# graphic-goose/ferreus_rbf_rs

Measured on AMD Instinct MI355X. Metric: BBFMM matvecs/s, higher is better.
Workload: dtype f64; 1 GPU; 10000000 uniform 3D points, LinearRbf, order 7, 1 rhs, adaptive sparse tree, ACA eps=1e-7, set_weights + evaluate at the sources; points=10000000, kernel=LinearRbf, order=7, nrhs=1, parallelism=single GPU

## Files before the change

### ferreus_rbf_rs_amd/_lib.py

```python
from __future__ import annotations

import ctypes
import os

HERE = os.path.dirname(os.path.abspath(__file__))
LIB_PATH = os.environ.get("FERREUS_BBFMM_HIP_LIB") or os.path.join(HERE, "libferreus_bbfmm_hip.so")

OK, POINT_OUTSIDE_TREE, KERNEL_NO_GRADIENTS, BAD_ARGUMENT, DEVICE_ERROR, UNSUPPORTED, CALLBACK_FAILED = range(7)
FLAG_HOST_ONLY = 1
FLAG_M2L_SHARED_BASIS = 2
FLAG_DIRECT_SMALL_W_LEAVES = 4
FLAG_DETERMINISTIC = 8
N_PHASES = 11
PHASE_NAMES = ["gather", "P2M", "M2M", "M2L_stage1", "M2L_stage2", "P2L", "L2L", "P2P", "M2P",
               "L2P", "scatter"]

c_i32, c_i64, c_f64, c_u32 = ctypes.c_int32, ctypes.c_int64, ctypes.c_double, ctypes.c_uint32
c_p = ctypes.c_void_p


class Params(ctypes.Structure):
    _fields_ = [("max_points_per_cell", c_i64), ("compression_type", c_i32),
                ("epsilon", c_f64), ("eval_chunk_size", c_i64)]

# ... 36 lines not shown
    "bbfmm_isosurface_tables": (ctypes.c_int, [c_p, c_p, c_p, c_p, c_p]),
    "bbfmm_isosurface_lattice": (ctypes.c_int, [c_p, c_p, c_f64, c_p]),
    "bbfmm_build_isosurfaces": (ctypes.c_int, [c_p, c_p, c_f64, c_p, c_i32, c_p, c_p, c_i64, c_p]),
    "bbfmm_isosurfaces_from_values": (ctypes.c_int, [c_p, c_p, c_p, c_f64, c_p, c_i32, c_i64, c_p]),
    "bbfmm_build_isosurfaces_ex": (ctypes.c_int, [c_p, c_p, c_f64, c_p, c_i32, c_p, c_p, c_i64, c_i32, c_p]),
    "bbfmm_isosurfaces_from_values_ex": (ctypes.c_int, [c_p, c_p, c_p, c_f64, c_p, c_i32, c_i64, c_i32, c_p]),
    "bbfmm_isosurface_stats": (ctypes.c_int, [c_p, c_i32, c_p]),
    "bbfmm_build_isosurfaces_opts": (ctypes.c_int, [c_p, c_p, c_f64, c_p, c_i32, c_p, c_p, c_p, c_p]),
    "bbfmm_isosurfaces_from_values_opts": (ctypes.c_int, [c_p, c_p, c_p, c_f64, c_p, c_i32, c_p, c_p]),
    "bbfmm_isosurfaces_from_fields_opts": (ctypes.c_int, [c_p, c_i32, c_p, c_i32, c_p, c_f64, c_p, c_i32, c_p, c_p, c_p]),
    "bbfmm_isosurfaces_from_function_opts": (ctypes.c_int, [c_p, c_p, c_p, c_p, c_f64, c_p, c_i32, c_p, c_p]),
    "bbfmm_debug_evaluate_fields": (ctypes.c_int, [c_p, c_i32, c_p, c_i32, c_p, c_i64, c_i64, c_p, c_p, c_i64]),
    "bbfmm_debug_field_program": (ctypes.c_int, [c_i32, c_i32, c_p, c_p, c_p, c_i32, c_p, c_p, c_i64, c_p, c_p]),
    "bbfmm_isosurface_finish_mesh": (ctypes.c_int, [c_p, c_p, c_i64, c_p, c_i64, c_p, c_p]),
    "bbfmm_isosurface_finish_stats": (ctypes.c_int, [c_p, c_i32, c_p]),
    "bbfmm_isosurface_close_mesh": (ctypes.c_int, [c_p, c_p, c_i64, c_p, c_i64, c_p, ctypes.c_double, c_i32, c_p]),
    "bbfmm_isosurface_closure_stats": (ctypes.c_int, [c_p, c_i32, c_p]),
    "bbfmm_debug_closure_triangulate": (ctypes.c_int, [c_i32, c_i32, c_p, c_p, c_p, c_i64, c_p, c_i64, c_p, c_i64, ctypes.c_double,
                                                       ctypes.c_double, c_i64, c_p, c_p, c_i64, c_p, c_p, c_p, c_i64]),
    "bbfmm_debug_orient2d": (ctypes.c_int, [c_p, c_i64, c_p]),
    "bbfmm_isosurface_follow_stats": (ctypes.c_int, [c_p, c_i32, c_p]),
    "bbfmm_isosurface_follow_times": (ctypes.c_int, [c_p, c_i32, c_p]),
    "bbfmm_isosurface_follow_bricks": (ctypes.c_int, [c_p, c_i32, c_p, c_p]),
    "bbfmm_isosurface_intersection_stats": (ctypes.c_int, [c_p, c_i32, c_p]),
    "bbfmm_isosurface_self_intersections": (ctypes.c_int, [c_p, c_p, c_i64, c_p, c_i64, c_p, c_p]),
    "bbfmm_isosurface_intersection_ids": (ctypes.c_int, [c_p, c_i32, c_p, c_p]),
    "bbfmm_isosurface_triangle_pair": (ctypes.c_int, [c_p, c_p, c_p, c_p, c_p, c_p]),
    "bbfmm_isosurface_clip_triangle": (ctypes.c_int, [c_p, c_p, c_p, c_p, c_p]),
    "bbfmm_isosurface_topology": (ctypes.c_int, [ctypes.c_uint32, c_p, c_p, c_p]),
    "bbfmm_isosurface_cluster_tables": (ctypes.c_int, [c_p, c_p, c_p]),
    "bbfmm_isosurface_curvature_tables": (ctypes.c_int, [c_p, c_p, c_p]),
    "bbfmm_isosurface_curvature_weight": (ctypes.c_int, [c_p, c_p, c_i32, c_p, c_p, c_p, c_p]),
    "bbfmm_isosurface_curvature_stats": (ctypes.c_int, [c_p, c_i32, c_p]),
    "bbfmm_isosurface_count": (c_i32, [c_p]),
    "bbfmm_isosurface_size": (ctypes.c_int, [c_p, c_i32, c_p, c_p]),
    "bbfmm_isosurface_copy": (ctypes.c_int, [c_p, c_i32, c_p, c_p]),
    "bbfmm_isosurface_error": (ctypes.c_char_p, [c_p]),
    "bbfmm_isosurface_destroy": (None, [c_p]),
    "bbfmm_prepare_target_subset": (ctypes.c_int, [c_p, c_p, c_i64]),
    "bbfmm_fast_matrix_vector_product": (ctypes.c_int, [c_p, c_p, c_i64, c_i64, c_p, c_i64, c_p,
                                                        c_i64, c_f64, c_p]),
    "bbfmm_matvec_device": (ctypes.c_int, [c_p, c_p, c_i64, c_i32, c_p, c_i64, c_i32]),
    "bbfmm_target_subset_create": (ctypes.c_int, [c_p, c_p, c_i64, c_p]),
    "bbfmm_matvec_subset_device": (ctypes.c_int, [c_p, c_i32, c_p, c_p, c_i32]),
    "bbfmm_stream": (c_p, [c_p]),
    "bbfmm_set_partition": (ctypes.c_int, [c_p, c_i32, c_i32]),
    "bbfmm_partition_row_count": (c_i64, [c_p]),
    "bbfmm_partition_rows": (ctypes.c_int, [c_p, c_p]),
    "bbfmm_partition_coarse_count": (c_i64, [c_p]),
    "bbfmm_matvec_partition_upward": (ctypes.c_int, [c_p, c_p, c_i64, c_i32, c_p, c_p]),
    "bbfmm_matvec_partition_finish": (ctypes.c_int, [c_p, c_p, c_p, c_i64, c_i32, c_p]),
    "bbfmm_partition_world": (c_i32, [c_p]),
    "bbfmm_partition_rank": (c_i32, [c_p]),
    "bbfmm_partition_bounds": (ctypes.c_int, [c_p, c_i32, c_p]),
    "bbfmm_matvec_partition_finish_sorted": (ctypes.c_int, [c_p, c_p, c_p, c_i64, c_p]),
    "bbfmm_partition_scatter": (ctypes.c_int, [c_p, c_p, c_i32, c_i32, c_i64, c_i32, c_p, c_i64]),
    "bbfmm_debug_partition_upward_counts": (ctypes.c_int, [c_p, c_p, c_p, c_p]),
    "bbfmm_debug_host_copy_rates": (ctypes.c_int, [c_i64, c_p]),
    "bbfmm_get_tree_stats": (ctypes.c_int, [c_p, c_p]),
    "bbfmm_tree_built_on_device": (ctypes.c_int, [c_p]),
    "bbfmm_last_evaluate_at_sources": (ctypes.c_int, [c_p]),
    "bbfmm_debug_targets_are_sources": (ctypes.c_int, [c_p, c_p, c_i64, c_i64]),
    "bbfmm_debug_rows_of_sources": (ctypes.c_int, [c_p, c_p, c_i64, c_i64, c_p]),
    "bbfmm_get_cells": (ctypes.c_int, [c_p, c_p, c_p]),
    "bbfmm_get_leaf_sources": (ctypes.c_int, [c_p, c_p, c_p]),
    "bbfmm_get_list": (ctypes.c_int, [c_p, ctypes.c_char, c_p, c_p, c_p]),
    "bbfmm_get_m2l_ranks": (ctypes.c_int, [c_p, c_p, c_p]),
    "bbfmm_get_m2l_operator": (ctypes.c_int, [c_p, c_i32, c_i32, c_p]),
    "bbfmm_get_m2l_factors": (ctypes.c_int, [c_p, c_i32, c_i32, c_p, c_p]),
    "bbfmm_get_permutation_tables": (ctypes.c_int, [c_p, c_p, c_p, c_p, c_p, c_p]),
    "bbfmm_points_to_leaves": (ctypes.c_int, [c_p, c_p, c_i64, c_i64, c_p, c_p]),
    "bbfmm_set_profiling": (ctypes.c_int, [c_p, c_i32]),
    "bbfmm_get_phase_ms": (ctypes.c_int, [c_p, c_p, c_p]),
    "bbfmm_reset_phase_ms": (ctypes.c_int, [c_p]),
    "bbfmm_mfma_f64_selftest": (ctypes.c_int, [c_p, c_p, c_p]),
    "bbfmm_fp64_valu_selftest": (ctypes.c_int, [c_p, c_p]),
    "bbfmm_debug_kernel_values": (ctypes.c_int, [c_i32, c_i32, ctypes.c_double, ctypes.c_double, c_p, c_i64, c_p, c_p, c_p]),
    "bbfmm_debug_math": (ctypes.c_int, [c_i32, c_i32, c_p, c_i64, c_p, c_p]),
    "bbfmm_debug_dense_m2m": (ctypes.c_int, [c_p, c_i32, c_p]),
    "bbfmm_debug_apply_m2l_tables_host": (ctypes.c_int, [c_p, c_p, c_p]),
    "bbfmm_debug_m2l_variants": (ctypes.c_int, [c_p, c_p, c_p]),
    "bbfmm_debug_m2l_pairs": (ctypes.c_int, [c_p, c_p, c_i64, c_p, c_p]),
    "bbfmm_debug_m2l_pairs_axes": (ctypes.c_int, [c_p, c_p, c_i64, c_p]),
    "bbfmm_debug_m2l_pairs_stage2": (ctypes.c_int, [c_p, c_p, c_i64, c_p, c_p]),
    "bbfmm_debug_m2l_pairs_axes_stage2": (ctypes.c_int, [c_p, c_p, c_i64, c_p]),
    "bbfmm_debug_m2l_table_digests": (ctypes.c_int, [c_p, c_p, c_i32, c_p, c_p, c_i32, c_p]),
    "bbfmm_debug_m2l_s2_last_ksplit": (ctypes.c_int, [c_p, c_p]),
    "bbfmm_debug_leaf_runs": (ctypes.c_int, [c_p, c_p]),
    "bbfmm_debug_group_state": (ctypes.c_int, [c_p, c_p, c_i64]),
    "bbfmm_debug_m2l_parity_len": (ctypes.c_int, [c_p, c_p]),
    "bbfmm_debug_get_coefficients": (ctypes.c_int, [c_p, ctypes.c_char, c_i32, c_p]),
    "bbfmm_debug_morton_encode": (ctypes.c_uint64, [c_i32, c_p, ctypes.c_uint64]),
    "bbfmm_debug_morton_decode": (None, [c_i32, ctypes.c_uint64, c_p, c_p]),
    "bbfmm_debug_morton_neighbours": (c_i32, [c_i32, ctypes.c_uint64, c_p]),
    "bbfmm_debug_direction_vectors": (c_i32, [c_i32, c_p]),
    "bbfmm_debug_reference_vectors": (ctypes.c_int, [c_p, c_p, c_p]),
    "bbfmm_givens_rotation": (None, [c_f64, c_f64, c_p, c_p, c_p]),
    "bbfmm_fgmres": (ctypes.c_int, [c_i64, c_p, c_p, c_p, c_p, c_p, c_p, c_i32, c_i32, c_i32, c_f64,
                                    c_p, c_p, c_p, c_p, c_p]),
    "bbfmm_schwarz_ddm_solver": (ctypes.c_int, [c_i64, c_p, c_p, c_p, c_p, c_p, c_i32, c_i32, c_f64,
                                                c_p, c_p, c_p, c_p, c_p]),
    "bbfmm_rbf_system_apply": (ctypes.c_int, [c_p, c_p, c_p, c_i64]),
    "bbfmm_rbf_system_device_create": (ctypes.c_int, [c_p, c_i64, c_p, c_i64, c_f64, c_p]),
    "bbfmm_rbf_system_device_destroy": (None, [c_p]),
    "bbfmm_rbf_system_apply_device": (ctypes.c_int, [c_p, c_p, c_p, c_i64, c_p]),
    "bbfmm_fgmres_device": (ctypes.c_int, [c_i64, c_p, c_p, c_p, c_p, c_p, c_p, c_i32, c_i32, c_i32, c_f64,
                                           c_p, c_p, c_p, c_p, c_p, c_p]),
    "bbfmm_schwarz_ddm_solver_device": (ctypes.c_int, [c_i64, c_p, c_p, c_p, c_p, c_p, c_i32, c_i32, c_f64,
                                                       c_p, c_p, c_p, c_p, c_p, c_p]),
    "bbfmm_debug_solver_vector_op": (ctypes.c_int, [c_i32, c_i32, c_i64, c_p, c_p, c_p, c_f64, c_i32, c_p, c_i32, c_p, c_p]),
    "bbfmm_ddm_params_defaults": (None, [c_p]),
    "bbfmm_ddm_params_for_points": (None, [c_i64, c_p]),
    "bbfmm_ddm_build": (ctypes.c_int, [c_p, c_i64, c_i32, c_i64, c_p, c_p]),
    "bbfmm_ddm_destroy": (None, [c_p]),
    "bbfmm_ddm_num_levels": (c_i32, [c_p]),
    "bbfmm_ddm_level_size": (c_i64, [c_p, c_i32]),
    "bbfmm_ddm_level_points": (ctypes.c_int, [c_p, c_i32, c_p]),
    "bbfmm_ddm_num_domains": (c_i64, [c_p, c_i32]),
    "bbfmm_ddm_domain_size": (c_i64, [c_p, c_i32, c_i64]),
    "bbfmm_ddm_domain": (ctypes.c_int, [c_p, c_i32, c_i64, c_p, c_p, c_p]),
    "bbfmm_schwarz_create": (ctypes.c_int, [c_p, c_p, c_i64, c_i32, c_i64, c_p, c_p, c_p]),
    "bbfmm_schwarz_create_sharded": (ctypes.c_int, [c_p, c_p, c_i64, c_i32, c_i64, c_p, c_p, c_i32, c_i32, c_p, c_i64, c_p, c_p, c_p]),
    "bbfmm_schwarz_factor_bytes": (c_i64, [c_p]),
    "bbfmm_schwarz_domains_owned": (c_i64, [c_p, c_i32, ctypes.POINTER(c_i64), ctypes.POINTER(c_i64)]),
    "bbfmm_schwarz_destroy": (None, [c_p]),
    "bbfmm_schwarz_basis_size": (c_i64, [c_p]),
    "bbfmm_schwarz_num_levels": (c_i32, [c_p]),
    "bbfmm_schwarz_monomial_matrix": (c_p, [c_p]),
    "bbfmm_debug_evaluate_monomials": (ctypes.c_int, [c_p, c_i64, c_i32, c_i64, c_i32, c_p, c_p, c_p]),
    "bbfmm_schwarz_apply": (ctypes.c_int, [c_p, c_p, c_p, c_i64]),
    "bbfmm_schwarz_apply_device": (ctypes.c_int, [c_p, c_p, c_p, c_i64, c_p]),
    "bbfmm_schwarz_debug_trace_steps": (c_i32, [c_p]),
    "bbfmm_schwarz_debug_apply_trace": (ctypes.c_int, [c_p, c_p, c_p, c_i64, c_i32, c_p, c_p, c_p, c_p, c_p]),
    "bbfmm_schwarz_debug_ortho_matrix": (c_p, [c_p]),
    "bbfmm_schwarz_level_size": (c_i64, [c_p, c_i32]),
    "bbfmm_schwarz_level_points": (ctypes.c_int, [c_p, c_i32, c_p]),
    "bbfmm_schwarz_debug_level_solve": (ctypes.c_int, [c_p, c_i32, c_p, c_p, c_i64, c_i32]),
    "bbfmm_ddm_debug_level_create": (ctypes.c_int, [c_p, c_i64, c_i32, c_i64, c_i64, c_p, c_p, c_p, c_p, c_i32, c_i32, c_p]),
    "bbfmm_ddm_debug_level_destroy": (None, [c_p]),
    "bbfmm_ddm_debug_level_info": (ctypes.c_int, [c_p, c_p]),
    "bbfmm_ddm_debug_level_layout": (ctypes.c_int, [c_p, c_p, c_p, c_p, c_p, c_p]),
    "bbfmm_ddm_debug_level_assembled": (ctypes.c_int, [c_p, c_p]),
    "bbfmm_ddm_debug_level_factor": (ctypes.c_int, [c_p, c_p]),
    "bbfmm_ddm_debug_level_solve": (ctypes.c_int, [c_p, c_p, c_p, c_i64, c_i32]),
    "bbfmm_schwarz_create_ex": (ctypes.c_int, [c_p, c_p, c_i64, c_i32, c_i64, c_p, c_i64, c_p, c_p, c_p]),
    "bbfmm_schwarz_create_sharded_ex": (ctypes.c_int, [c_p, c_p, c_i64, c_i32, c_i64, c_p, c_i64, c_p, c_p, c_i32, c_i32, c_p, c_i64,
                                                       c_p, c_p, c_p]),
    "bbfmm_ddm_debug_level_create_ex": (ctypes.c_int, [c_p, c_i64, c_i32, c_i64, c_p, c_i64, c_i64, c_p, c_p, c_p, c_p, c_i32, c_i32,
                                                       c_p]),
    "bbfmm_global_trend_transform": (ctypes.c_int, [c_i32, c_p, c_p, c_p, c_p]),
    "bbfmm_duplicate_cutoff_distance": (ctypes.c_int, [c_p, c_f64, c_p]),
    "bbfmm_remove_duplicates": (ctypes.c_int, [c_p, c_i64, c_i32, c_i64, c_f64, c_i32, c_p, c_p, c_p]),
    "bbfmm_debug_interpolant_terms": (ctypes.c_int, [c_i32, c_i32, c_p, c_p, c_i64, c_i64, c_p, c_i64, c_p, c_i64, c_p, c_i64]),
    "bbfmm_evaluate_interpolant": (ctypes.c_int, [c_p, c_i32, c_i32, c_p, c_i64, c_i32, c_i64, c_p, c_i64, c_i64, c_p, c_f64,
                                                  c_p, c_i64, c_p, c_i64, c_p]),
    "bbfmm_evaluate_device": (ctypes.c_int, [c_p, c_i32, c_p, c_i64, c_i64, c_p, c_p, c_i64, c_p, c_i64, c_p, c_p]),
    "bbfmm_evaluate_grid": (ctypes.c_int, [c_p, c_i32, c_p, c_p, c_p, c_i64, c_p, c_i64, c_p, c_p]),
    "bbfmm_evaluate_grid_stats": (ctypes.c_int, [c_p, c_p]),
    "bbfmm_debug_grid_coords": (ctypes.c_int, [c_i32, c_p, c_i64, c_i64, c_p, c_i64]),
    "bbfmm_debug_split_runs": (ctypes.c_int, [c_i32, c_p, c_p, c_p, c_i64, c_i32, c_p, c_p, c_p, c_i64, c_p]),
}


class Interpolant(ctypes.Structure):
    _fields_ = [("kernel_type", c_i32), ("polynomial_degree", c_i32), ("nugget", c_f64), ("base_range", c_f64),
                ("total_sill", c_f64), ("flags", c_u32)]
# ... 83 lines not shown
```

### ferreus_rbf_rs_amd/csrc/capi_debug.cpp

```cpp
#include <algorithm>
#include <chrono>
#include <cstring>
#include <vector>

#include "capi_handle.hpp"
#include "morton.hpp"

namespace {
template <int ID>
void debug_kernel_values_host(const bbfmm::KernelSpec &ks, const double *r2, int64_t n, double *value, double *value_g, double *factor) {
    for (int64_t i = 0; i < n; ++i) {
        value[i] = bbfmm::kernel_value_r2<ID>(ks, r2[i]);
        value_g[i] = bbfmm::kernel_value_grad_r2<ID>(ks, r2[i], &factor[i]);
    }
}
}

extern "C" {

int bbfmm_debug_targets_are_sources(const bbfmm_handle *h, const double *x, int64_t m, int64_t ldx) {
    return (h && h->tree.targets_are_sources(x, m, ldx)) ? 1 : 0;
}
int bbfmm_debug_rows_of_sources(bbfmm_handle *h, const double *x, int64_t m, int64_t ldx, int64_t *rows_out) {
    if (!h || !rows_out) return 0;
// ... 95 lines not shown
            case 1: bbfmm::bb_sqrt_rsqrt(x[i], &a, &b); break;
            case 2: a = bbfmm::bb_rcp(x[i]); break;
            default: a = bbfmm::bb_log(x[i]); break;
            }
            out[i] = a;
            if (out2) out2[i] = b;
        }
        return BBFMM_OK;
    }
    int ndev = 0;
    if (hipGetDeviceCount(&ndev) != hipSuccess || ndev == 0) return BBFMM_DEVICE_ERROR;
    return bbfmm::debug_math_device(which, x, n, out, out2) == 0 ? BBFMM_OK : BBFMM_DEVICE_ERROR;
}

int bbfmm_debug_dense_m2m(const bbfmm_handle *h, int32_t child_index, double *out) {
    if (!h || !out) return BBFMM_BAD_ARGUMENT;
    std::vector<double> m;
    bbfmm::dense_m2m_matrix(h->tree.ops(), child_index, &m);
    std::memcpy(out, m.data(), m.size() * sizeof(double));
    return BBFMM_OK;
}

int bbfmm_debug_apply_m2l_tables_host(const bbfmm_handle *h, const double *M, double *L) {
    if (!h || !M || !L) return BBFMM_BAD_ARGUMENT;
    return h->tree.debug_apply_m2l_tables_host(M, L);
}

uint64_t bbfmm_debug_morton_encode(int32_t d, const uint64_t *anchor, uint64_t level) {
    if (d < 1 || d > 3 || !anchor) return 0;
    return bbfmm::encode_morton_point(anchor, level, d);
}
void bbfmm_debug_morton_decode(int32_t d, uint64_t key, uint64_t *anchor_out, uint64_t *level_out) {
    if (d < 1 || d > 3 || !anchor_out || !level_out) return;
    bbfmm::decode_key(key, d, anchor_out, level_out);
}
int32_t bbfmm_debug_morton_neighbours(int32_t d, uint64_t key, uint64_t *keys_out) {
    if (d < 1 || d > 3 || !keys_out) return -1;
    return bbfmm::get_neighbours(key, d, keys_out);
}
int32_t bbfmm_debug_direction_vectors(int32_t d, int32_t *out) {
    if (d < 1 || d > 3 || !out) return -1;
    const int(*dirs)[3];
    const int n = bbfmm::direction_vectors(d, &dirs);
    for (int i = 0; i < n; ++i)
        for (int a = 0; a < d; ++a) out[i * d + a] = dirs[i][a];
    return n;
}
int bbfmm_debug_reference_vectors(const bbfmm_handle *h, int32_t *out, int32_t *n_ref_out) {
    if (!h) return BBFMM_BAD_ARGUMENT;
    const bbfmm::Operators &ops = h->tree.ops();
    if (n_ref_out) *n_ref_out = ops.n_ref;
    if (out) std::copy(ops.ref_vecs.begin(), ops.ref_vecs.end(), out);
    return BBFMM_OK;
}

int bbfmm_debug_m2l_variants(const bbfmm_handle *h, int64_t *n_variants, int64_t *n_cells) {
    if (!h) return BBFMM_BAD_ARGUMENT;
    int64_t nv = 0, nc = 0;
    h->tree.m2l_variant_stats(&nv, &nc);
    if (n_variants) *n_variants = nv;
    if (n_cells) *n_cells = nc;
    return BBFMM_OK;
}

int bbfmm_debug_m2l_pairs(const bbfmm_handle *h, int32_t *out, int64_t cap, int64_t *n_out, int32_t *pairs_on) {
    if (!h || !n_out) return BBFMM_BAD_ARGUMENT;
    std::vector<int32_t> v;
    h->tree.debug_m2l_pairs(&v);
    *n_out = static_cast<int64_t>(v.size());
    if (pairs_on) *pairs_on = h->tree.m2l_pairs() ? 1 : 0;
    if (out) std::copy(v.begin(), v.begin() + std::min<int64_t>(cap, *n_out), out);
    return BBFMM_OK;
}

int bbfmm_debug_m2l_pairs_axes(const bbfmm_handle *h, int32_t *out, int64_t cap, int64_t *n_out) {
    if (!h || !n_out) return BBFMM_BAD_ARGUMENT;
    std::vector<int32_t> v;
    h->tree.debug_m2l_pairs_axes(&v);
    *n_out = static_cast<int64_t>(v.size());
    if (out) std::copy(v.begin(), v.begin() + std::min<int64_t>(cap, *n_out), out);
    return BBFMM_OK;
}

int bbfmm_debug_m2l_pairs_stage2(const bbfmm_handle *h, int32_t *out, int64_t cap, int64_t *n_out, int32_t *pairs_on) {
    if (!h || !n_out) return BBFMM_BAD_ARGUMENT;
    std::vector<int32_t> v;
    h->tree.debug_m2l_pairs_stage2(&v);
    *n_out = static_cast<int64_t>(v.size());
    if (pairs_on) *pairs_on = h->tree.m2l_pairs_stage2() ? 1 : 0;
    if (out) std::copy(v.begin(), v.begin() + std::min<int64_t>(cap, *n_out), out);
    return BBFMM_OK;
}

int bbfmm_debug_m2l_pairs_axes_stage2(const bbfmm_handle *h, int32_t *out, int64_t cap, int64_t *n_out) {
    if (!h || !n_out) return BBFMM_BAD_ARGUMENT;
    std::vector<int32_t> v;
    h->tree.debug_m2l_pairs_axes_stage2(&v);
    *n_out = static_cast<int64_t>(v.size());
    if (out) std::copy(v.begin(), v.begin() + std::min<int64_t>(cap, *n_out), out);
    return BBFMM_OK;
}

int bbfmm_debug_m2l_table_digests(const bbfmm_handle *h, uint64_t *digests, int32_t cap, int32_t *n_out, double *flops_level,
                                  int32_t flops_cap, int32_t *n_levels_out) {
    if (!h || !n_out) return BBFMM_BAD_ARGUMENT;
    std::vector<uint64_t> v;
    h->tree.debug_m2l_table_digests(&v);
    *n_out = static_cast<int32_t>(v.size());
    if (digests) std::copy(v.begin(), v.begin() + std::min<int32_t>(cap, *n_out), digests);
    const std::vector<double> &fl = h->tree.m2l_flops_level();
    if (n_levels_out) *n_levels_out = static_cast<int32_t>(fl.size());
    if (flops_level) std::copy(fl.begin(), fl.begin() + std::min<int32_t>(flops_cap, static_cast<int32_t>(fl.size())), flops_level);
    return BBFMM_OK;
}

int bbfmm_debug_m2l_s2_last_ksplit(const bbfmm_handle *h, int32_t *ksplit) {
    if (!h || !ksplit) return BBFMM_BAD_ARGUMENT;
    *ksplit = h->tree.debug_m2l_s2_last_ksplit();
    return BBFMM_OK;
}

int bbfmm_debug_leaf_runs(const bbfmm_handle *h, int32_t *counts) {
    if (!h || !counts) return BBFMM_BAD_ARGUMENT;
    h->tree.debug_leaf_runs(counts);
    return BBFMM_OK;
}

int bbfmm_debug_group_state(const bbfmm_handle *h, int64_t *out, int64_t cap) {
    if (!h || !out) return BBFMM_BAD_ARGUMENT;
    const int64_t need = bbfmm::DeviceGroup::kStateHeader + (h->group ? h->group->n_parts() : 1);
    if (cap < need) return BBFMM_BAD_ARGUMENT;
    std::fill(out, out + need, int64_t(0));
    if (h->group)
        h->group->debug_state(out);
    else
        out[0] = 1;
    return BBFMM_OK;
}

int bbfmm_debug_m2l_parity_len(const bbfmm_handle *h, int32_t *len) {
    if (!h || !len) return BBFMM_BAD_ARGUMENT;
    *len = h->tree.debug_m2l_parity_len();
    return BBFMM_OK;
}

int bbfmm_debug_get_coefficients(bbfmm_handle *h, char which, int32_t k, double *out) {
    GUARD(h) return h->tree.debug_get_coefficients(which, k, out);
    END_GUARD(h)
}

}
```

### ferreus_rbf_rs_amd/csrc/device.hpp

```cpp
#pragma once
#include <hip/hip_runtime.h>

#include <cstdint>

#include "kernels.hpp"

namespace bbfmm {

constexpr int kMaxOrder = 16;
constexpr int kM2lTile = 128;
constexpr int kM2lS1Block = 176;
constexpr int kM2lS1BlockPairs = 160;
constexpr int kM2lSlotWindow = 128;
constexpr int kM2lBlkTwoDst = 1 << 30;

struct DevCheb {
    int p, d, n, n_pad;
    double polyn[kMaxOrder * kMaxOrder];
    double q[kMaxOrder * kMaxOrder];
    double nodes[kMaxOrder];
    double xfer[2 * kMaxOrder * kMaxOrder];
};

struct ChebRef {
    const DevCheb *dev;
    int p, d, n, n_pad;
};

struct M2lClass {
    const double *vt_all;
    const int32_t *row_dst;
    const int32_t *row_dst2;
    const int32_t *blk_t0;
    int32_t yb0;
    int32_t n_rows;
    int32_t r_pad16;
    int32_t n_t;
    const double *u_all;
    int32_t k_pad;
    int32_t kp;
    int32_t kpy;
    const int32_t *cells;
    int32_t n_cells;
    const int32_t *cslot;
    const int64_t *cbase;
};

struct M2lTileDesc {
    int32_t level_class;
    int32_t first;
    int32_t count;
    int32_t q_first;
    int32_t q_count;
    int32_t pad;
};

void launch_gather_weights(const double *w, int64_t ldw, int K, const int32_t *order, int64_t N,
                           double *w_sorted, hipStream_t s);
void launch_gather_weights_subset(const double *w, int64_t ldw, int K, const int32_t *order, const int32_t *pos, int64_t n_pos,
                                  int64_t N, double *w_sorted, hipStream_t s);
constexpr int kMaxScatterParts = 64;
struct ScatterParts {
    int n;
    int64_t bound[kMaxScatterParts + 1];
};
void launch_scatter_parts(const double *all, const ScatterParts &parts, int64_t m_max, int K, const int32_t *order, double *out,
                          int64_t ldo, hipStream_t s);
void launch_sum_slots(const double *slots, int n_slots, int64_t len, double *out, hipStream_t s);
void launch_scatter_output(const double *out_sorted, int64_t n, int K, const int32_t *perm,
                           double *out, int64_t ldo, int accumulate, hipStream_t s);
void launch_gather_rows(const double *src, int64_t ld_src, int ncols, const int32_t *idx, int64_t n,
                        double *dst, int64_t ld_dst, hipStream_t s);

void launch_p2m(const ChebRef &ch, const double *const *src_xyz, const double *w_sorted, int64_t N,
                int K, int64_t C, const int32_t *leaf_cells, int n_leaves, const int32_t *pt_begin,
                const int32_t *pt_end, const double *centers, const double *lengths, double *M,
                hipStream_t s);
struct M2lParityRowArgs;
struct M2lUnparityRowArgs;
int launch_m2m(const ChebRef &ch, int K, int64_t C, const int32_t *parents, int n_parents,
               const int64_t *child_ptr, const int32_t *child_idx, const int32_t *octant, double *M,
               hipStream_t s, const M2lParityRowArgs *par = nullptr, double *Mp = nullptr);
bool m2m_writes_parity(const ChebRef &ch);
int launch_l2l(const ChebRef &ch, int K, int64_t C, const int32_t *cells, int n_cells,
               const int32_t *parent, const int32_t *octant, const uint8_t *active, double *L,
               hipStream_t s, const M2lUnparityRowArgs *unp = nullptr, const double *Lp = nullptr,
               const uint8_t *has_m2l = nullptr, const uint8_t *has_x = nullptr);
bool l2l_reads_parity(const ChebRef &ch);
void launch_zero_rows(const int32_t *cells, int n_cells, int n_pad, int K, int64_t C, double *L, hipStream_t s);

void launch_m2l_stage1(const M2lClass *classes, const M2lTileDesc *tiles, const int32_t *tile_idx, int n_tiles,
                       int n_pad, int max_slot_t, int K, int64_t C, const double *M, double *cbuf,
                       int64_t cbuf_len, hipStream_t s, bool own_blocks = false, int max_blocks = 8, int ne16 = 0, int s_ee = 0,
                       int s_eo = 0);
void launch_m2l_parity(const double *M, int n_pad, double *Mp, int n_par, int ne16, int n_e, int n_o, int p, int64_t rows,
                       hipStream_t s);
struct M2lParityOffsets {
    int32_t v[4];
};
void launch_m2l_parity2(const double *M, int n_pad, double *Mp, int n_par, M2lParityOffsets off, int p, int p2, int64_t rows,
                        hipStream_t s);
void launch_m2l_stage2(const M2lClass *classes, const M2lTileDesc *tiles, const int32_t *tile_idx, int n_tiles,
                       int n_pad, int K, int64_t C, const double *cbuf, int64_t cbuf_len,
                       const uint16_t *qlist, double *L, hipStream_t s, bool allow_ksplit = true);
struct M2lS2PairsPlan {
    int ga, gb, ce, co;
    int ya = 0, yb = 0;
    int ne16() const { return 16 * ga * ce; }
    __host__ __device__ int n_par() const { return 16 * (ga * ce + gb * co); }
    __host__ __device__ int col(int part, int j) const {
        const int g = part < 2 ? ga : gb, y = part < 2 ? ya : yb, w = 16 * ((part & 1) ? g - y : y);
        const int jj = j % w, gl = ((part & 1) ? y : 0) + jj / 16, pp = jj % 16, paired = g / 2 * 2;
        const int local = gl < paired ? 32 * (gl / 2) + 2 * pp + (gl & 1) : 16 * paired + pp;
        return (part < 2 ? 0 : 16 * ga * ce) + (j / w) * 16 * g + local;
    }
};
M2lS2PairsPlan m2l_s2_pairs_plan(int groups_even, int groups_odd);
M2lS2PairsPlan m2l_s2_pairs_plan2(const int groups[4]);
struct M2lParityRowArgs {
    int axes = 0;
    int n_par = 0;
    int p = 0;
    int ne16 = 0, n_e = 0, n_o = 0, p1 = 0;
    M2lParityOffsets off{{0, 0, 0, 0}};
    int p2 = 0;
};

struct M2lUnparityRowArgs {
    int axes = 0;
    int n_par = 0;
    int p = 0;
    int ne16 = 0, n_e = 0, n_o = 0, p1 = 0;
    M2lS2PairsPlan plan{1, 1, 1, 1};
    int p2 = 0;
};
void launch_m2l_parity_cells(const double *M, int n_pad, double *Mp, const M2lParityRowArgs &par, const int32_t *cells, int n_cells,
                             int K, int64_t C, hipStream_t s);
int m2l_s2_pairs_ksplit(int n_tiles, const M2lS2PairsPlan &plan, int K, bool allow_ksplit);
bool launch_m2l_stage2_pairs(const M2lClass *classes, const M2lTileDesc *tiles, const int32_t *tile_idx, int n_tiles,
                             const M2lS2PairsPlan &plan, int K, int64_t C, const double *cbuf, int64_t cbuf_len,
                             const uint16_t *qlist, double *Lp, hipStream_t s, bool allow_ksplit = true, int *ksplit_out = nullptr);
void launch_m2l_unparity(const double *Lp, int n_par, int ne16, double *L, int n, int n_pad, int n_e, int n_o, int p, int64_t rows,
                         hipStream_t s);
void launch_m2l_unparity2(const double *Lp, const M2lS2PairsPlan &plan, double *L, int n, int n_pad, int p, int p2, int64_t rows,
                          hipStream_t s);
void launch_m2l_zero_segments(const int32_t *segs, int64_t n_segs, int K, double *cbuf, int64_t cbuf_len, hipStream_t s);
void launch_m2l_basis(const M2lClass *classes, const M2lTileDesc *tiles, int n_tiles, int in_ld, int out_ld, int K,
                      int64_t C, const double *in, double *out, hipStream_t s);
void launch_small_gemm(bool trans_a, int M, int N, int Kd, const double *A, int64_t lda, const double *B, int64_t ldb,
                       double *Cm, int64_t ldc, hipStream_t s);

struct M2lAssembleTv {
    int32_t perm;
    int32_t rank;
    int32_t row;
    int64_t vt_off;
    int64_t u_off;
};
struct M2lAssembleClass {
    const M2lAssembleTv *src, *tgt;
    int32_t n_src, n_tgt, r_pad16, k_pad, max_rank;
    int32_t n_e, n_o, ne16, n_par, p;
    int32_t u_npar, u_ne16, u_rows, u_ne, u_no;
    int32_t s1_axes;
    M2lParityOffsets s1_off;
    M2lS2PairsPlan u_plan;
};
void launch_m2l_assemble(const M2lAssembleClass &c, int n, int n_pad, bool compressed, const double *ops,
                         const int32_t *invperm, double *vt_all, double *u_all, hipStream_t s);

struct DirectJobs {
    int n_jobs;
    const int32_t *job_cell;
    const int32_t *tgt_begin, *tgt_end;
    const int64_t *run_ptr;
    const int32_t *runs;
};
// ... 53 lines not shown
```

### ferreus_rbf_rs_amd/csrc/device_m2l.hip

```cpp
#include "device_common.hpp"
#include "m2l_basis_rows.hpp"

#include <cmath>

namespace bbfmm {

typedef __attribute__((address_space(3))) void *lptr_t;

__device__ inline unsigned lds_offset(const double *p) {
    return static_cast<unsigned>(reinterpret_cast<uintptr_t>((lptr_t)p));
}
__device__ inline unsigned uniform_u32(unsigned v) { return __builtin_amdgcn_readfirstlane(v); }
__device__ inline const double *uniform_ptr(const double *p) {
    const uintptr_t v = reinterpret_cast<uintptr_t>(p);
    const unsigned lo = __builtin_amdgcn_readfirstlane(static_cast<unsigned>(v));
    const unsigned hi = __builtin_amdgcn_readfirstlane(static_cast<unsigned>(v >> 32));
    return reinterpret_cast<const double *>((static_cast<uintptr_t>(hi) << 32) | lo);
}
__device__ inline void dma16(const double *g, unsigned lds_wave_byte_offset) {
    asm volatile("s_mov_b32 m0, %1\n\ts_nop 0\n\tglobal_load_lds_dwordx4 %0, off" ::"v"(g),
                 "s"(uniform_u32(lds_wave_byte_offset))
                 : "memory");
}
__device__ inline void dma4(const int32_t *g, unsigned lds_wave_byte_offset) {
    asm volatile("s_mov_b32 m0, %1\n\ts_nop 0\n\tglobal_load_lds_dword %0, off" ::"v"(g),
                 "s"(uniform_u32(lds_wave_byte_offset))
                 : "memory");
}
__device__ inline void wait_dma_and_barrier() {
    asm volatile("s_waitcnt vmcnt(0)" ::: "memory");
    __syncthreads();
}
template <int N> __device__ inline void wait_dma_keep_stores_and_barrier() {
    asm volatile("s_waitcnt vmcnt(%0)" ::"n"(N < 63 ? N : 63) : "memory");
    __syncthreads();
}
template <int N> __device__ inline double add_row_ror(double v) {
    const int lo = __double2loint(v), hi = __double2hiint(v);
    const int rlo = __builtin_amdgcn_update_dpp(0, lo, 0x120 + N, 0xf, 0xf, false);
    const int rhi = __builtin_amdgcn_update_dpp(0, hi, 0x120 + N, 0xf, 0xf, false);
    return v + __hiloint2double(rhi, rlo);
}

__device__ inline void dma16s(const double *sbase, unsigned voff_bytes, unsigned lds_wave_byte_offset) {
    asm volatile("s_mov_b32 m0, %2\n\ts_nop 0\n\tglobal_load_lds_dwordx4 %0, %1" ::"v"(voff_bytes),
                 "s"(uniform_ptr(sbase)), "s"(uniform_u32(lds_wave_byte_offset))
                 : "memory");
}

template <int NG16, int STAGE, int MINW, bool PAIRS = false>
__global__ __launch_bounds__(512, MINW) void m2l_gemm_k4(const M2lClass *__restrict__ classes,
                                                  const M2lTileDesc *__restrict__ tiles, int n_pad, int g16_0,
                                                  int64_t C, const double *__restrict__ in, int64_t in_len,
                                                  double *__restrict__ out, int64_t out_len,
                                                  const uint16_t *__restrict__ qlist, int slot_t,
                                                  const int32_t *__restrict__ tile_idx) {
    extern __shared__ double lds[];
    const M2lTileDesc tile = tiles[blockIdx.x];
    const M2lClass cls = classes[tile.level_class];
    const int kr = blockIdx.y;
    const int tid = threadIdx.x, wave = tid >> 6, lane = tid & 63;
    constexpr int BLK = PAIRS ? kM2lS1BlockPairs : kM2lS1Block;
    const int n_zb = STAGE == 1 ? cls.r_pad16 / BLK : 1;
    const bool own_blocks = STAGE == 1 && tile.pad == 2;
    const int zb0 = STAGE == 1 ? (own_blocks ? tile.q_first : (int)((int64_t)n_zb * blockIdx.z / gridDim.z)) : 0;
    const int zb1 = STAGE == 1 ? (own_blocks ? tile.q_first + tile.q_count : (int)((int64_t)n_zb * (blockIdx.z + 1) / gridDim.z)) : 1;
    const int ld = STAGE == 1 ? cls.r_pad16 : n_pad;
    const int ksplit = STAGE == 2 && slot_t > 1 ? slot_t : 1;
    const int zcols = STAGE == 2 ? (int)gridDim.z / ksplit : 1;
    const int zk = STAGE == 2 ? (int)blockIdx.z / zcols : 0, zc = STAGE == 2 ? (int)blockIdx.z - zk * zcols : (int)blockIdx.z;
    const int q_lo = STAGE == 2 ? tile.q_count * zk / ksplit : 0;
    const int nq = STAGE == 1 ? n_pad / 16 : STAGE == 2 ? tile.q_count * (zk + 1) / ksplit - q_lo : (int)(in_len / 16);
    const uint16_t *ql = qlist + tile.q_first + q_lo;
    const int nq_e = PAIRS ? (int)(in_len & 0xffffffff) / 16 : 0;
    const int s_ee = PAIRS ? (int)(in_len >> 32) & 0xffff : 0, s_eo = PAIRS ? (int)(in_len >> 48) : 0;
    if (zb0 >= zb1) return;
    const int g16 = g16_0 + (STAGE >= 2 ? zc * NG16 : 0);
    const double *opbase = (STAGE == 1 ? cls.vt_all : cls.u_all) + 16 * g16;

    constexpr int OP_CHUNKS = 2 * NG16;
    constexpr int NCH = (OP_CHUNKS + 7) / 8;
    constexpr int OP_DOUBLES = OP_CHUNKS * 128;
    constexpr int BUF = OP_DOUBLES + 2048;

    constexpr int NP = NG16 / 2, NS = NG16 & 1;
    unsigned voff[NCH];
#pragma unroll
    for (int i = 0; i < NCH; ++i) {
        const int c = wave + 8 * i;
        if (c < 4 * NP) {
            const int e = c / NP, pr = c - e * NP, k = lane >> 4, p = lane & 15;
            voff[i] = (unsigned)(((4 * k + e) * ld + 32 * pr + 2 * p) * 8);
        } else {
            const int e = 2 * (c - 4 * NP) + (lane >> 5), r = lane & 31, k = r >> 3, pair = r & 7;
            voff[i] = (unsigned)(((4 * k + e) * ld + 32 * NP + 2 * pair) * 8);
        }
    }
    auto cell_p = [&](int pos) {
        const int q = pos < tile.count ? pos : 0;
        return tile.pad ? tile_idx[tile.first + q] : tile.first + q;
    };
    const double *cptr[2];
#pragma unroll
    for (int h = 0; h < 2; ++h) {
        const int tg = 2 * h + (lane >> 5), eh = (lane >> 4) & 1, k = (lane >> 2) & 3, j = lane & 3;
        const int pos = wave * 16 + 4 * tg + j;
        const int p = cell_p(pos);
        const int64_t base = STAGE == 2 ? (int64_t)kr * in_len + cls.cbase[p]
                                        : ((int64_t)kr * C + cls.cells[p]) * (STAGE == 1 ? (int64_t)n_pad : in_len);
        cptr[h] = in + base + 4 * k + 2 * eh;
    }
    const unsigned lds0 = lds_offset(lds);
    const int64_t qstride = (int64_t)16 * ld;
    auto stage = [&](int sidx, int buf) {
        const int zb = zb0 + sidx / nq, qi = sidx - (sidx / nq) * nq;
        int q = STAGE == 2 ? (int)ql[qi] : qi;
        if constexpr (PAIRS) {
            if (zb >= cls.yb0) {
                if (qi >= s_ee && qi < s_ee + s_eo) q = qi + s_eo;
                else if (qi >= s_ee + s_eo && qi < s_ee + 2 * s_eo) q = qi - s_eo;
            }
        }
#pragma unroll
        for (int i = 0; i < NCH; ++i)
            if (wave + 8 * i < OP_CHUNKS)
                dma16s(opbase + (int64_t)zb * BLK + q * qstride, voff[i],
                       lds0 + (unsigned)(buf * BUF + (wave + 8 * i) * 128) * 8u);
#pragma unroll
        for (int h = 0; h < 2; ++h)
            dma16(cptr[h] + 16 * q, lds0 + (unsigned)(buf * BUF + OP_DOUBLES + (2 * wave + h) * 128) * 8u);
    };

    double acc[4][NG16];
    double acc_e[4][PAIRS ? NG16 : 1];
#pragma unroll
    for (int tg = 0; tg < 4; ++tg)
#pragma unroll
        for (int g = 0; g < NG16; ++g) {
            acc[tg][g] = 0.0;
            if constexpr (PAIRS) acc_e[tg][g] = 0.0;
        }

    const int bk = lane >> 4, bj = lane & 3;
    const bool wave_live = wave * 16 < tile.count;
    const int n_steps = (zb1 - zb0) * nq;
    const int di = lane >> 4, db = (lane >> 2) & 3, dj = lane & 3;
    constexpr int AUX = PAIRS ? 384 : 192;
    const int32_t *aux = reinterpret_cast<const int32_t *>(lds + 2 * BUF);
    int32_t *ptab = reinterpret_cast<int32_t *>(lds + 2 * BUF) + 2 * AUX;
    const int32_t *slds = aux + 2 * AUX + 128 + wave * 16 * slot_t;
    if (STAGE == 1 && lane < 16) ptab[wave * 16 + lane] = cell_p(wave * 16 + lane);
    const unsigned aux0 = lds0 + (unsigned)(2 * BUF) * 8u;
    auto stage_cols = [&](int zb_, int par) {
        if (STAGE == 1 && 64 * wave <= 16 * NG16) {
            const int e = 64 * wave + lane;
            const int32_t *src = e < 16 * NG16 ? cls.row_dst + zb_ * BLK + 16 * g16 + e : cls.blk_t0 + zb_;
            dma4(src, aux0 + (unsigned)(par * AUX + 64 * wave) * 4u);
        } else if (PAIRS && 64 * wave < 192 + 16 * NG16) {
            const int e = 64 * wave + lane - 192;
            const int32_t *src = e < 16 * NG16 ? cls.row_dst2 + zb_ * BLK + 16 * g16 + e : cls.blk_t0 + zb_;
            dma4(src, aux0 + (unsigned)(par * AUX + 64 * wave) * 4u);
        }
    };
    const int slot_sh = 31 - __builtin_clz(slot_t | 1);
    auto stage_slots = [&](int par) {
        const int t0 = __builtin_amdgcn_readfirstlane(aux[par * AUX + 16 * NG16]) & (kM2lBlkTwoDst - 1);
        const unsigned dst0 = aux0 + (unsigned)(2 * AUX + 128 + wave * 16 * slot_t) * 4u;
        for (int i = 0; i < slot_t / 4; ++i) {
            const int e = i * 64 + lane, cl = e >> slot_sh, tl = e & (slot_t - 1);
            const int32_t *src = cls.cslot + (int64_t)ptab[wave * 16 + cl] * cls.n_t + min(t0 + tl, cls.n_t - 1);
            dma4(src, dst0 + (unsigned)i * 256u);
        }
    };
    if (n_steps > 0) {
        stage(0, 0);
        stage_cols(zb0, 0);
    }
    wait_dma_and_barrier();
    int qcnt = 0, zb = zb0;
    for (int sidx = 0; sidx < n_steps; ++sidx) {
        const double *op = lds + (sidx & 1) * BUF + lane;
        const double2 *op2 = reinterpret_cast<const double2 *>(lds + (sidx & 1) * BUF) + lane;
        const double *ct = lds + (sidx & 1) * BUF + OP_DOUBLES + wave * 256 + (bk * 4 + bj) * 2;
        if (sidx + 1 < n_steps) stage(sidx + 1, (sidx + 1) & 1);
        if (STAGE == 1) {
            if (qcnt == 0 && zb + 1 < zb1) stage_cols(zb + 1, (zb + 1 - zb0) & 1);
            if (qcnt == nq - 2) stage_slots((zb - zb0) & 1);
        }
        if (wave_live) {
            if constexpr (PAIRS) {
                if (qcnt == nq_e) {
#pragma unroll
                    for (int tg = 0; tg < 4; ++tg)
#pragma unroll
                        for (int g = 0; g < NG16; ++g) {
                            acc_e[tg][g] = acc[tg][g];
                            acc[tg][g] = 0.0;
                        }
                }
            }
            constexpr int EH = PAIRS ? 1 : 2;
#pragma unroll
            for (int eh0 = 0; eh0 < 2; eh0 += EH) {
                double bq[4][2 * EH];
#pragma unroll
                for (int tg = 0; tg < 4; ++tg)
#pragma unroll
                    for (int eh = 0; eh < EH; ++eh) {
                        const double2 v = *reinterpret_cast<const double2 *>(ct + ((tg * 2 + eh0 + eh) * 16) * 2);
                        bq[tg][2 * eh] = v.x;
                        bq[tg][2 * eh + 1] = v.y;
                    }
#pragma unroll
                for (int el = 0; el < 2 * EH; ++el) {
                    const int e = 2 * eh0 + el;
#pragma unroll
                    for (int pr = 0; pr < NP; ++pr) {
                        const double2 a = op2[(e * NP + pr) * 64];
#pragma unroll
                        for (int tg = 0; tg < 4; ++tg) {
                            acc[tg][2 * pr] = __builtin_amdgcn_mfma_f64_4x4x4f64(a.x, bq[tg][el], acc[tg][2 * pr], 0, 0, 0);
                            acc[tg][2 * pr + 1] =
                                __builtin_amdgcn_mfma_f64_4x4x4f64(a.y, bq[tg][el], acc[tg][2 * pr + 1], 0, 0, 0);
                        }
                    }
                    if (NS) {
                        const double a = op[4 * NP * 128 + e * 64];
#pragma unroll
                        for (int tg = 0; tg < 4; ++tg)
                            acc[tg][NG16 - 1] = __builtin_amdgcn_mfma_f64_4x4x4f64(a, bq[tg][el], acc[tg][NG16 - 1], 0, 0, 0);
                    }
                }
            }
        }
        if (++qcnt == nq) {
            qcnt = 0;
            const int col0 = zb * BLK + 16 * g16;
            ++zb;
            bool two_dst = false;
            if constexpr (PAIRS) {
              if (wave_live) {
                double *cb = out + (int64_t)kr * out_len;
                double *dump = cb + (out_len - 128) + 2 * lane;
                const int32_t *auxb = aux + ((zb - 1 - zb0) & 1) * AUX;
                two_dst = (__builtin_amdgcn_readfirstlane(auxb[16 * NG16]) & kM2lBlkTwoDst) != 0;
                int pk[NP + NS], pk2[NP + NS];
#pragma unroll
                for (int pr = 0; pr < NP + NS; ++pr) {
                    pk[pr] = auxb[pr < NP ? 32 * pr + 2 * (4 * db + di) : 32 * NP + 4 * db + di];
                    pk2[pr] = two_dst ? auxb[192 + (pr < NP ? 32 * pr + 2 * (4 * db + di) : 32 * NP + 4 * db + di)] : -1;
                }
#pragma unroll
                for (int tg = 0; tg < 4; ++tg) {
                    const bool spv = wave * 16 + 4 * tg + dj < tile.count;
                    const int32_t *srow = slds + (4 * tg + dj) * slot_t;
#pragma unroll
                    for (int pr = 0; pr < NP + NS; ++pr) {
                        const bool single = NS && pr == NP;
                        const int g0 = single ? NG16 - 1 : 2 * pr, g1 = single ? NG16 - 1 : 2 * pr + 1;
                        const int sl = srow[max(pk[pr] >> 24, 0)];
                        const int okm = (spv ? -1 : 0) & ~(pk[pr] | sl);
                        double *dst = okm < 0 ? cb + (int64_t)sl * 2 + (pk[pr] & 0xffffff) : dump;
                        if (single) *dst = acc_e[tg][g0] + acc[tg][g0];
                        else *reinterpret_cast<double2 *>(dst) = make_double2(acc_e[tg][g0] + acc[tg][g0], acc_e[tg][g1] + acc[tg][g1]);
                        if (two_dst) {
                            const int sl2 = srow[max(pk2[pr] >> 24, 0)];
                            const int okm2 = (spv ? -1 : 0) & ~(pk2[pr] | sl2);
                            double *dst2 = okm2 < 0 ? cb + (int64_t)sl2 * 2 + (pk2[pr] & 0xffffff) : dump;
                            if (single) *dst2 = acc_e[tg][g0] - acc[tg][g0];
                            else *reinterpret_cast<double2 *>(dst2) = make_double2(acc_e[tg][g0] - acc[tg][g0], acc_e[tg][g1] - acc[tg][g1]);
                        }
                    }
                    __builtin_amdgcn_sched_barrier(0);
                }
              }
            } else if (STAGE == 1 && wave_live) {
                double *cb = out + (int64_t)kr * out_len;
                double *dump = cb + (out_len - 128) + 2 * lane;
                const int32_t *auxb = aux + ((zb - 1 - zb0) & 1) * AUX;
                int pk[NP + NS];
#pragma unroll
                for (int pr = 0; pr < NP; ++pr) pk[pr] = auxb[32 * pr + 2 * (4 * db + di)];
                if (NS) pk[NP] = auxb[32 * NP + 4 * db + di];
#pragma unroll
                for (int tg = 0; tg < 4; ++tg) {
                    const bool spv = wave * 16 + 4 * tg + dj < tile.count;
                    const int32_t *srow = slds + (4 * tg + dj) * slot_t;
#pragma unroll
                    for (int pr = 0; pr < NP; ++pr) {
                        const int sl = srow[max(pk[pr] >> 24, 0)];
                        const int okm = (spv ? -1 : 0) & ~(pk[pr] | sl);
                        double *dst = okm < 0 ? cb + (int64_t)sl * 2 + (pk[pr] & 0xffffff) : dump;
                        *reinterpret_cast<double2 *>(dst) = make_double2(acc[tg][2 * pr], acc[tg][2 * pr + 1]);
                    }
                    if (NS) {
                        const int sl = srow[max(pk[NP] >> 24, 0)];
                        const int okm = (spv ? -1 : 0) & ~(pk[NP] | sl);
                        double *dst = okm < 0 ? cb + (int64_t)sl * 2 + (pk[NP] & 0xffffff) : dump;
                        *dst = acc[tg][NG16 - 1];
                    }
                }
            } else if (STAGE >= 2) {
#pragma unroll
                for (int tg = 0; tg < 4; ++tg) {
                    const int tp = wave * 16 + 4 * tg + dj;
                    if (tp < tile.count) {
                        const int cell = cls.cells[cell_p(tp)];
                        double *Lc = out + ((int64_t)kr * C + cell) * n_pad + col0;
                        if (ksplit > 1) {
#pragma unroll
                            for (int pr = 0; pr < NP; ++pr) {
                                unsafeAtomicAdd(Lc + 32 * pr + 2 * (4 * db + di), acc[tg][2 * pr]);
                                unsafeAtomicAdd(Lc + 32 * pr + 2 * (4 * db + di) + 1, acc[tg][2 * pr + 1]);
                            }
                            if (NS) unsafeAtomicAdd(Lc + 32 * NP + 4 * db + di, acc[tg][NG16 - 1]);
                        } else {
#pragma unroll
                            for (int pr = 0; pr < NP; ++pr)
                                *reinterpret_cast<double2 *>(Lc + 32 * pr + 2 * (4 * db + di)) =
                                    make_double2(acc[tg][2 * pr], acc[tg][2 * pr + 1]);
                            if (NS) Lc[32 * NP + 4 * db + di] = acc[tg][NG16 - 1];
                        }
                    }
                }
            }
#pragma unroll
            for (int tg = 0; tg < 4; ++tg)
#pragma unroll
                for (int g = 0; g < NG16; ++g) acc[tg][g] = 0.0;
            if (STAGE == 1) {
                if (wave_live && two_dst) asm volatile("s_waitcnt vmcnt(%0)" ::"n"(8 * (NP + NS) < 63 ? 8 * (NP + NS) : 63) : "memory");
                else if (wave_live) asm volatile("s_waitcnt vmcnt(%0)" ::"n"(4 * (NP + NS) < 63 ? 4 * (NP + NS) : 63) : "memory");
                else asm volatile("s_waitcnt vmcnt(0)" ::: "memory");
                __syncthreads();
                continue;
            }
        }
        wait_dma_and_barrier();
    }
}

template <int NG16, int STAGE, int MINW, bool PAIRS = false>
static void m2l_gemm_launch(const M2lClass *classes, const M2lTileDesc *tiles, int n_tiles, int n_pad, int g16_0,
                            int n_colblocks, int K, int64_t C, const double *in, int64_t in_len, double *out,
                            int64_t out_len, const uint16_t *qlist, int slot_t, const int32_t *tile_idx, hipStream_t s) {
    const size_t lds = 2 * sizeof(double) * (size_t)(2 * NG16 * 128 + 2048) + (STAGE == 1 ? (size_t)(2 * (PAIRS ? 384 : 192) + 128 + 8 * 16 * (slot_t & 0xffff)) * 4 : 0);
    static std::atomic<uint64_t> attr_set[4] = {{0}, {0}, {0}, {0}};
    (void)allow_large_dynamic_lds(reinterpret_cast<const void *>(&m2l_gemm_k4<NG16, STAGE, MINW, PAIRS>), lds, attr_set);
    const int zdim = STAGE == 2 && slot_t > 1 ? n_colblocks * slot_t : n_colblocks;
    hipLaunchKernelGGL((m2l_gemm_k4<NG16, STAGE, MINW, PAIRS>), dim3(n_tiles, K, zdim), dim3(512), lds, s, classes,
                       tiles, n_pad, g16_0, C, in, in_len, out, out_len, qlist, slot_t, tile_idx);
}


template <int STAGE> constexpr int m2l_chunk_pref() { return STAGE == 1 ? kM2lS1Block / 16 : 22; }
constexpr int kM2lS2KsplitFill = 4;

template <int STAGE>
static void m2l_dispatch_chunks(int total_groups, const M2lClass *classes, const M2lTileDesc *tiles, int n_tiles,
                                int n_pad, int n_colblocks, int K, int64_t C, const double *in, int64_t in_len,
                                double *out, int64_t out_len, const uint16_t *qlist, int slot_t,
                                const int32_t *tile_idx, hipStream_t s) {
    int done = 0;
    const int pref = m2l_chunk_pref<STAGE>();
    while (done < total_groups) {
        const int left = total_groups - done;
        int take;
#define M2L_GO(NG, MW)                                                                                              \
    {                                                                                                               \
        take = NG;                                                                                                  \
        m2l_gemm_launch<NG, STAGE, MW>(classes, tiles, n_tiles, n_pad, done,                                        \
                                       STAGE >= 2 ? 1 : n_colblocks, K, C, in, in_len,                            \
                                       out, out_len, qlist, slot_t, tile_idx, s);                                   \
    }
        if (STAGE >= 2 && !(n_colblocks == 1 && left >= 16)) {
            int best_ng = 2, best_z = 1;
            for (int ng : {11, 8, 7, 6, 4, 2})
                for (int zc = 1; zc <= (n_colblocks == 1 ? 1 : ng == 11 ? 2 : 3); ++zc)
                    if (ng * zc <= left && ((left - ng * zc) % 2 == 0 || left - ng * zc == 7) &&
                        (ng * zc > best_ng * best_z || (ng * zc == best_ng * best_z && ng > best_ng))) {
                        best_ng = ng;
                        best_z = zc;
                    }
            take = best_ng * best_z;
#define M2L_ZGO(NG, MW)                                                                                             \
    m2l_gemm_launch<NG, STAGE, MW>(classes, tiles, n_tiles, n_pad, done, best_z, K, C, in, in_len, out, out_len,    \
                                   qlist, slot_t, tile_idx, s);
            if constexpr (STAGE >= 2) {
                switch (best_ng) {
                case 11: M2L_ZGO(11, 1) break;
                case 8: M2L_ZGO(8, 4) break;
                case 7: M2L_ZGO(7, 2) break;
                case 6: M2L_ZGO(6, 4) break;
                case 4: M2L_ZGO(4, 4) break;
                default: M2L_ZGO(2, 4) break;
                }
            }
#undef M2L_ZGO
        } else if (pref == 22 && left >= 22) M2L_GO(22, 1)
        else if (pref == 22 && left >= 16) M2L_GO(16, 1)
        else if (pref == 11 && left >= 11) M2L_GO(11, 1)
        else if (left >= 8) M2L_GO(8, 4)
        else if (left >= 6) M2L_GO(6, 4)
        else if (left >= 4) M2L_GO(4, 4)
        else M2L_GO(2, 4)
#undef M2L_GO
        done += take;
    }
}

void launch_m2l_stage1(const M2lClass *classes, const M2lTileDesc *tiles, const int32_t *tile_idx, int n_tiles,
                       int n_pad, int max_slot_t, int K, int64_t C, const double *M, double *cbuf, int64_t cbuf_len,
                       hipStream_t s, bool own_blocks, int max_blocks, int ne16, int s_ee, int s_eo) {
    if (n_tiles == 0) return;
    int slot_t = 16;
    while (slot_t < max_slot_t) slot_t *= 2;
    const int n_cu = device_cu_count();
    const int zmax = n_tiles * 8 < n_cu ? std::max(8, std::min(max_blocks, 32)) : 8;
    int zsplit = 1;
    double best = 1e300;
    for (int z = 1; z <= zmax; ++z) {
        const double rounds = std::ceil(static_cast<double>(n_tiles) * z / n_cu);
        const double cost = rounds / z * (1.0 + 0.005 * z);
        if (cost < best - 1e-12) {
            best = cost;
            zsplit = z;
        }
    }
    const int n_colblocks = own_blocks ? 1 : zsplit;
    if (ne16 > 0) {
        const int64_t packed = static_cast<int64_t>(ne16) | (static_cast<int64_t>(s_ee & 0xffff) << 32) | (static_cast<int64_t>(s_eo & 0x7fff) << 48);
        m2l_gemm_launch<kM2lS1BlockPairs / 16, 1, 1, true>(classes, tiles, n_tiles, n_pad, 0, n_colblocks, K, C, M, packed, cbuf, cbuf_len,
                                                      nullptr, slot_t, tile_idx, s);
        return;
    }
    m2l_dispatch_chunks<1>(kM2lS1Block / 16, classes, tiles, n_tiles, n_pad, n_colblocks, K, C, M, 0, cbuf, cbuf_len, nullptr,
                           slot_t, tile_idx, s);
}

static int m2l_s2_ksplit(int64_t wgs, bool allow_ksplit) {
    static const int ks_env = [] {
        const int v = env_int("BBFMM_M2L_S2_KSPLIT", 0);
        return v >= 1 && v <= 32 ? v : 0;
    }();
    if (!allow_ksplit) return 1;
    if (ks_env > 0) return ks_env;
    const int n_cu = device_cu_count();
    int ksplit = 1;
    if (wgs * 2 <= static_cast<int64_t>(kM2lS2KsplitFill) * n_cu) {
        double best = 1e300;
        for (int ks = 1; ks <= 16; ++ks) {
            const double cost = std::ceil(static_cast<double>(wgs * ks) / n_cu) * (0.05 + 1.0 / ks);
            if (cost < best - 1e-12) {
                best = cost;
                ksplit = ks;
            }
        }
    }
    return ksplit;
}

void launch_m2l_stage2(const M2lClass *classes, const M2lTileDesc *tiles, const int32_t *tile_idx, int n_tiles,
                       int n_pad, int K, int64_t C, const double *cbuf, int64_t cbuf_len, const uint16_t *qlist,
                       double *L, hipStream_t s, bool allow_ksplit) {
    if (n_tiles == 0) return;
    static const int z = env_int("BBFMM_M2L_S2_ZSPLIT", 2) == 1 ? 1 : 2;
    const int ksplit = m2l_s2_ksplit(static_cast<int64_t>(n_tiles) * z * K, allow_ksplit);
    m2l_dispatch_chunks<2>(n_pad / 16, classes, tiles, n_tiles, n_pad, z, K, C, cbuf, cbuf_len, L, 0, qlist, ksplit > 1 ? ksplit : 0, tile_idx, s);
}

template <int NG16, int Y = NG16>
__device__ __forceinline__ void m2l_s2_pairs_body(const M2lClass &cls, const M2lTileDesc &tile, int n_par, int g16, bool odd,
                                                  int zk, int ksplit, int64_t C, const double *__restrict__ in, int64_t in_len,
                                                  double *__restrict__ out, const uint16_t *__restrict__ qlist,
                                                  const int32_t *__restrict__ tile_idx, double *lds) {
    const int kr = blockIdx.y;
    const int tid = threadIdx.x, wave = tid >> 6, lane = tid & 63;
    const int ld = n_par;
    const int q_lo = tile.q_count * zk / ksplit;
    const int nq = tile.q_count * (zk + 1) / ksplit - q_lo;
    const uint16_t *ql = qlist + tile.q_first + q_lo;
    const int kp = cls.kp, kp16 = kp >> 4;
    const int kpy16 = Y < NG16 ? cls.kpy >> 4 : kp16;
    const double *opbase = cls.u_all + 16 * g16;

    constexpr int OP_CHUNKS = 2 * NG16;
    constexpr int NCH = (OP_CHUNKS + 7) / 8;
    constexpr int OP_DOUBLES = OP_CHUNKS * 128;
    constexpr int BUF = OP_DOUBLES + 4096;
    constexpr int NP = NG16 / 2, NS = NG16 & 1;
    unsigned voff[NCH];
#pragma unroll
    for (int i = 0; i < NCH; ++i) {
        const int c = wave + 8 * i;
        if (c < 4 * NP) {
            const int e = c / (NP > 0 ? NP : 1), pr = c - e * NP, k = lane >> 4, p = lane & 15;
            voff[i] = (unsigned)(((4 * k + e) * ld + 32 * pr + 2 * p) * 8);
        } else {
            const int e = 2 * (c - 4 * NP) + (lane >> 5), r = lane & 31, k = r >> 3, pair = r & 7;
            voff[i] = (unsigned)(((4 * k + e) * ld + 32 * NP + 2 * pair) * 8);
        }
    }
    auto cell_p = [&](int pos) {
        const int q = pos < tile.count ? pos : 0;
        return tile.pad ? tile_idx[tile.first + q] : tile.first + q;
    };
    const double *cptr[2];
#pragma unroll
    for (int h = 0; h < 2; ++h) {
        const int tg = 2 * h + (lane >> 5), eh = (lane >> 4) & 1, k = (lane >> 2) & 3, j = lane & 3;
        const int p = cell_p(wave * 16 + 4 * tg + j);
        cptr[h] = in + (int64_t)kr * in_len + cls.cbase[p] + 4 * k + 2 * eh;
    }
    const unsigned lds0 = lds_offset(lds);
    const int64_t qstride = (int64_t)16 * ld;
    auto stage = [&](int qi, int buf) {
// ... 558 lines not shown
```

### ferreus_rbf_rs_amd/csrc/fmm_m2l_debug.cpp

```cpp
#include "fmm_tree_impl.hpp"

#include <type_traits>

namespace bbfmm {

namespace {
struct Fnv {
    uint64_t h = 1469598103934665603ull;
    template <class T> void put(T v) {
        static_assert(std::is_integral<T>::value, "integer tables only");
        unsigned char b[sizeof(T)];
        std::memcpy(b, &v, sizeof(T));
        for (unsigned char c : b) h = (h ^ c) * 1099511628211ull;
    }
    template <class V> void vec(const V &v) {
        put(static_cast<uint64_t>(v.size()));
        for (auto x : v) put(x);
    }
    void tiles(const std::vector<M2lTileDesc> &v) {
        put(static_cast<uint64_t>(v.size()));
        for (const M2lTileDesc &t : v) {
            put(t.level_class);
            put(t.first);
            put(t.count);
// ... 40 lines not shown
        f[2].vec(h.tgt_pair);
        f[2].vec(h.tgt_kind);
        for (int v : {h.level, h.octant, h.n_rows, h.r_pad16, h.n_t, h.k_pad, h.yb0, h.pad_cols, h.kp, h.kpy, h.tgt_pad}) f[2].put<int32_t>(v);
        f[3].vec(h.row_dst);
        f[3].vec(h.row_dst2);
        f[3].vec(h.blk_t0);
        f[3].vec(h.row_tpos);
        f[3].vec(h.row_off);
        f[3].vec(h.row_tpos2);
        f[3].vec(h.row_off2);
        f[4].vec(h.cells);
        f[4].vec(h.cbase);
        f[4].vec(h.cslot);
    }
    f[5].tiles(m2l_tiles1_h_);
    f[5].vec(m2l_tile_idx1_h_);
    f[6].tiles(m2l_tiles_h_);
    f[6].tiles(m2l_tiles2_h_);
    f[6].vec(m2l_qlist_h_);
    f[7].put(static_cast<uint64_t>(m2l_batches_.size()));
    for (const M2lBatch &b : m2l_batches_) {
        for (int v : {b.level_lo, b.level_hi, b.groups, b.group}) f[7].put<int32_t>(v);
        f[7].put(b.len);
        for (int32_t v : {b.t1_first, b.t1_count, b.t2_first, b.t2_count}) f[7].put(v);
    }
    f[7].vec(m2l_batch_of_class_);
    f[7].put(static_cast<uint64_t>(m2l_group_ops_.size()));
    for (const std::vector<int32_t> &g : m2l_group_ops_) f[7].vec(g);
    f[7].vec(m2l_zero_h_);
    f[7].vec(m2l_zero_ptr_);
    out->clear();
    for (const Fnv &x : f) out->push_back(x.h);
}

int FmmTree::debug_apply_m2l_tables_host(const double *M, double *L) const {
    const int n = ops_.n, n_pad = round_up(n, 32);
    std::vector<double> Mp;
    if (m2l_pairs_) {
        Mp.assign(static_cast<size_t>(tree_.n_cells()) * m2l_npar_, 0.0);
        for (int64_t c = 0; c < tree_.n_cells(); ++c) {
            const double *Mv = M + static_cast<size_t>(c) * n;
            double *mp = &Mp[static_cast<size_t>(c) * m2l_npar_];
            for (int k = 0; m2l_axes_ == 2 && k < m2l_npar_; ++k)
                for (int g = 0; g < 4; ++g)
                    if (m2l_par_node_[static_cast<size_t>(4 * k + g)] >= 0)
                        mp[k] += m2l_par_sign_[static_cast<size_t>(4 * k + g)] * Mv[m2l_par_node_[static_cast<size_t>(4 * k + g)]];
            for (int j = 0; m2l_axes_ == 1 && j < m2l_ne_; ++j) {
                if (j < m2l_no_) {
                    mp[j] = Mv[j] + Mv[m2l_rho(j)];
                    mp[m2l_ne16_ + j] = Mv[j] - Mv[m2l_rho(j)];
                } else {
                    mp[j] = Mv[j];
                }
            }
        }
    }
    std::vector<double> cbuf(static_cast<size_t>(std::max<int64_t>(cbuf_batch_len_, 1)), 0.0);
    std::vector<int32_t> seen(static_cast<size_t>(tree_.n_cells()), 0);
    const bool have_zero_lists = m2l_batches_.size() > 1 && !m2l_zero_h_.empty();
    for (size_t b = 0; b < m2l_batches_.size(); ++b) {
        const M2lBatch &mb = m2l_batches_[b];
        if (have_zero_lists)
            for (int64_t z = m2l_zero_ptr_[b]; z < m2l_zero_ptr_[b + 1]; ++z)
                std::fill(cbuf.begin() + 2 * static_cast<int64_t>(m2l_zero_h_[static_cast<size_t>(2 * z)]),
                          cbuf.begin() + 2 * (static_cast<int64_t>(m2l_zero_h_[static_cast<size_t>(2 * z)]) + m2l_zero_h_[static_cast<size_t>(2 * z + 1)]), 0.0);
        for (int32_t ti = mb.t1_first; ti < mb.t1_first + mb.t1_count; ++ti) {
            const M2lTileDesc &td = m2l_tiles1_h_[static_cast<size_t>(ti)];
            const bool variant = static_cast<size_t>(td.level_class) >= m2l_host_.size();
            const HostM2lClass &hc = variant ? m2l_variants_[static_cast<size_t>(td.level_class) - m2l_host_.size()]
                                             : m2l_host_[static_cast<size_t>(td.level_class)];
            if (hc.vt_all.empty()) return BBFMM_UNSUPPORTED;
            if (m2l_batch_of_class_[static_cast<size_t>(td.level_class)] != static_cast<int32_t>(b)) return BBFMM_BAD_ARGUMENT;
            for (int32_t q = 0; q < td.count; ++q) {
                const size_t pos = static_cast<size_t>(td.pad ? m2l_tile_idx1_h_[static_cast<size_t>(td.first + q)] : td.first + q);
                ++seen[hc.cells[pos]];
                const double *Mv = M + static_cast<size_t>(hc.cells[pos]) * n;
                for (int row = 0; row < hc.n_rows; ++row) {
                    if (hc.row_tpos[row] < 0) continue;
                    const int32_t slot = hc.cslot[pos * hc.n_t + hc.row_tpos[row]];
                    if (m2l_pairs_) {
                        const int32_t slot2 = hc.row_tpos2[row] >= 0 ? hc.cslot[pos * hc.n_t + hc.row_tpos2[row]] : -1;
                        if (slot < 0 && slot2 < 0) continue;
                        const double *mp = &Mp[static_cast<size_t>(hc.cells[pos]) * m2l_npar_];
                        double a = 0.0, bsum = 0.0;
                        if (row / m2l_s1_block_ >= hc.yb0) {
                            for (int j = 0; j < m2l_npar_; ++j) {
                                const bool y_odd = (j >= m2l_s1_off_.v[1] && j < m2l_s1_off_.v[2]) || j >= m2l_s1_off_.v[3];
                                (y_odd ? bsum : a) += hc.vt_all[static_cast<size_t>(j) * hc.r_pad16 + row] * mp[j];
                            }
                        } else {
                            for (int j = 0; j < m2l_ne16_; ++j) a += hc.vt_all[static_cast<size_t>(j) * hc.r_pad16 + row] * mp[j];
                            for (int j = m2l_ne16_; j < m2l_npar_; ++j) bsum += hc.vt_all[static_cast<size_t>(j) * hc.r_pad16 + row] * mp[j];
                        }
                        if (slot >= 0) cbuf[static_cast<size_t>(slot) * 2 + hc.row_off[row]] = a + bsum;
                        if (slot2 >= 0) cbuf[static_cast<size_t>(slot2) * 2 + hc.row_off2[row]] = a - bsum;
                        continue;
                    }
                    if (slot < 0) continue;
                    double s = 0.0;
                    for (int m = 0; m < n; ++m) s += hc.vt_all[static_cast<size_t>(m) * hc.r_pad16 + row] * Mv[m];
                    cbuf[static_cast<size_t>(slot) * 2 + hc.row_off[row]] = s;
                }
            }
        }
        for (size_t lc = 0; lc < m2l_host_.size(); ++lc) {
            if (m2l_batch_of_class_[lc] != static_cast<int32_t>(b)) continue;
            const HostM2lClass &hc = m2l_host_[lc];
            for (size_t pos = 0; pos < hc.cells.size(); ++pos) {
                double *Lb = L + static_cast<size_t>(hc.cells[pos]) * n;
                const double *cc = &cbuf[static_cast<size_t>(hc.cbase[pos])];
                if (m2l_pairs2_) {
                    const int n_par = m2l_s2_plan_.n_par(), ne16 = m2l_s2_plan_.ne16(), rows = hc.k_pad - hc.kp;
                    std::vector<double> sm(static_cast<size_t>(rows)), df(static_cast<size_t>(rows));
                    for (int r = 0; r < rows; ++r) {
                        sm[static_cast<size_t>(r)] = r < hc.kp ? cc[r] + cc[hc.kp + r] : cc[hc.kp + r];
                        df[static_cast<size_t>(r)] = r < hc.kp ? cc[r] - cc[hc.kp + r] : cc[hc.kp + r];
                    }
                    if (m2l_s2_axes_ == 2) {
                        for (int k = 0; k < n_par; ++k) {
                            const int part = m2l_s2_part_[static_cast<size_t>(k)];
                            if (part < 0) continue;
                            double acc = 0.0;
                            for (int r = 0; r < rows; ++r) {
                                const bool odd = r < hc.kpy ? part >= 2 : (part & 1);
                                acc += hc.u_all[static_cast<size_t>(r) * n_par + k] * (odd ? df : sm)[static_cast<size_t>(r)];
                            }
                            for (int g = 0; g < 4; ++g)
                                if (m2l_s2_node_[static_cast<size_t>(4 * k + g)] >= 0)
                                    Lb[m2l_s2_node_[static_cast<size_t>(4 * k + g)]] += m2l_s2_sign_[static_cast<size_t>(4 * k + g)] * acc;
                        }
                        continue;
                    }
                    for (int i = 0; i < m2l_ne_; ++i) {
                        double le = 0.0, lo = 0.0;
                        for (int r = 0; r < rows; ++r) {
                            le += hc.u_all[static_cast<size_t>(r) * n_par + i] * sm[static_cast<size_t>(r)];
                            if (i < m2l_no_) lo += hc.u_all[static_cast<size_t>(r) * n_par + ne16 + i] * df[static_cast<size_t>(r)];
                        }
                        if (i >= m2l_no_) {
                            Lb[i] += le;
                        } else {
                            Lb[i] += le + lo;
                            Lb[m2l_rho(i)] += le - lo;
                        }
                    }
                    continue;
                }
                for (int i = 0; i < n; ++i) {
                    double s = 0.0;
                    for (int k = 0; k < hc.k_pad; ++k) s += hc.u_all[static_cast<size_t>(k) * n_pad + i] * cc[k];
                    Lb[i] += s;
                }
            }
        }
    }
    for (const HostM2lClass &hc : m2l_host_)
        for (int32_t c : hc.cells) {
            const size_t lc = static_cast<size_t>(&hc - m2l_host_.data());
            const M2lBatch &mb = m2l_batches_[static_cast<size_t>(m2l_batch_of_class_[lc])];
            const int want = mb.groups == 1 || m2l_group_ops_[lc].empty() ? mb.groups : static_cast<int>(m2l_group_ops_[lc].size());
            if (seen[c] != want) return BBFMM_BAD_ARGUMENT;
        }
    return BBFMM_OK;
}

void FmmTree::debug_m2l_pairs(std::vector<int32_t> *out) const {
    out->clear();
    const int d = d_;
    for (size_t i = 0; i < m2l_host_.size() + m2l_variants_.size(); ++i) {
        const HostM2lClass &h = i < m2l_host_.size() ? m2l_host_[i] : m2l_variants_[i - m2l_host_.size()];
        if (h.cells.empty()) continue;
        out->push_back(h.level);
        out->push_back(h.octant);
        out->push_back(i < m2l_host_.size() ? 0 : 1);
        const size_t n_at = out->size();
        out->push_back(0);
        int32_t n_entries = 0;
        for (size_t pos = 0; pos < h.src_tv.size(); ++pos) {
            const bool x_pair = h.src_pair[pos] >= 0 && h.src_kind[pos] == 1;
            if (h.src_pair[pos] == -2 && h.src_kind[pos] == 1) continue;
            out->push_back(x_pair ? 1 : 0);
            for (int a = 0; a < d; ++a) out->push_back(ops_.all_vecs[static_cast<size_t>(h.src_tv[pos]) * d + a]);
            ++n_entries;
        }
        (*out)[n_at] = n_entries;
    }
}

void FmmTree::debug_m2l_pairs_axes(std::vector<int32_t> *out) const {
    out->clear();
    const int d = d_;
    out->push_back(m2l_pairs_ ? m2l_axes_ : 0);
    out->push_back(static_cast<int32_t>(m2l_work_[0]));
    out->push_back(static_cast<int32_t>(m2l_work_[1]));
    for (size_t i = 0; i < m2l_host_.size() + m2l_variants_.size(); ++i) {
        const HostM2lClass &h = i < m2l_host_.size() ? m2l_host_[i] : m2l_variants_[i - m2l_host_.size()];
        if (h.cells.empty()) continue;
        const int n_blk = h.r_pad16 / m2l_s1_block_;
        out->push_back(h.level);
        out->push_back(h.octant);
        out->push_back(i < m2l_host_.size() ? 0 : 1);
        out->push_back(h.pad_cols);
        out->push_back(h.yb0);
        out->push_back(n_blk);
        const size_t n_at = out->size();
        out->push_back(0);
        for (int b = 0; b < n_blk; ++b) out->push_back(b >= h.yb0 ? 1 : 0);
        int32_t n_entries = 0;
        for (size_t pos = 0; pos < h.src_tv.size(); ++pos) {
            if (h.src_pair[pos] == -2) continue;
            out->push_back(h.src_pair[pos] >= 0 ? h.src_kind[pos] : 0);
            const bool rows = h.src_row1[pos] > h.src_row0[pos];
            out->push_back(rows ? h.src_row0[pos] / m2l_s1_block_ : -1);
            out->push_back(rows ? (h.src_row1[pos] - 1) / m2l_s1_block_ : -1);
            for (int a = 0; a < d; ++a) out->push_back(ops_.all_vecs[static_cast<size_t>(h.src_tv[pos]) * d + a]);
            ++n_entries;
        }
        (*out)[n_at] = n_entries;
    }
}

void FmmTree::debug_m2l_pairs_stage2(std::vector<int32_t> *out) const {
    out->clear();
    const int d = d_;
    for (const HostM2lClass &h : m2l_host_) {
        if (h.cells.empty()) continue;
        out->push_back(h.level);
        out->push_back(h.octant);
        out->push_back(0);
        const size_t n_at = out->size();
        out->push_back(0);
        int32_t n_entries = 0;
        for (size_t pos = 0; pos < h.tgt_tv.size(); ++pos) {
            const bool x_member = h.tgt_kind[pos] == 1;
            if (h.tgt_pair[pos] == -2 && x_member) continue;
            out->push_back(h.tgt_pair[pos] >= 0 && x_member ? 1 : 0);
            for (int a = 0; a < d; ++a) out->push_back(ops_.all_vecs[static_cast<size_t>(h.tgt_tv[pos]) * d + a]);
            ++n_entries;
        }
        (*out)[n_at] = n_entries;
    }
}

void FmmTree::debug_m2l_pairs_axes_stage2(std::vector<int32_t> *out) const {
    out->clear();
    const int d = d_;
    out->push_back(m2l_pairs2_ ? m2l_s2_axes_ : 0);
    out->push_back(static_cast<int32_t>(m2l_s2_work_[0]));
    out->push_back(static_cast<int32_t>(m2l_s2_work_[1]));
    for (const HostM2lClass &h : m2l_host_) {
        if (h.cells.empty()) continue;
        const auto &lops = ops_.m2l[h.level];
        out->push_back(h.level);
        out->push_back(h.octant);
        out->push_back(h.kp);
        out->push_back(h.kpy);
        out->push_back(h.k_pad);
        out->push_back(h.tgt_pad);
        const size_t n_at = out->size();
        out->push_back(0);
        int32_t n_entries = 0;
        for (size_t pos = 0; pos < h.tgt_tv.size(); ++pos) {
            if (h.tgt_pair[pos] == -2) continue;
            out->push_back(h.tgt_pair[pos] >= 0 ? h.tgt_kind[pos] : 0);
            out->push_back(h.tgt_off[pos]);
            out->push_back(h.tgt_pair[pos] >= 0 ? h.tgt_off[static_cast<size_t>(h.tgt_pair[pos])] : -1);
            out->push_back(lops[ops_.ref_lookup[h.tgt_tv[pos]]].rank);
            for (int a = 0; a < d; ++a) out->push_back(ops_.all_vecs[static_cast<size_t>(h.tgt_tv[pos]) * d + a]);
            ++n_entries;
        }
        (*out)[n_at] = n_entries;
    }
}

}
```

### ferreus_rbf_rs_amd/csrc/fmm_m2l_tables.cpp

```cpp
#include "fmm_tree_impl.hpp"

namespace bbfmm {

void FmmTree::fill_m2l_operator_arrays(const HostM2lClass &hc, std::vector<double> *vt_all,
                                       std::vector<double> *u_all) const {
    const int n_pad = round_up(ops_.n, 32);
    vt_all->resize(static_cast<size_t>(m2l_pairs_ ? m2l_npar_ : n_pad) * hc.r_pad16);
    u_all->resize(m2l_pairs2_ ? static_cast<size_t>(hc.k_pad - hc.kp) * m2l_s2_plan_.n_par() : static_cast<size_t>(hc.k_pad) * n_pad);
    fill_m2l_operator_arrays(hc, vt_all->data(), u_all->data());
}

void FmmTree::fill_m2l_operator_arrays(const HostM2lClass &hc, double *vt_all, double *u_all) const {
    const int n = ops_.n, n_pad = round_up(n, 32);
    const bool compressed = ops_.compression != kCompressionNone;
    const auto &lops = ops_.m2l[hc.level];
    auto zero = [](double *p, size_t len) {
        parallel_for_chunks(static_cast<int64_t>(len), int64_t(1) << 18, [&](int64_t b, int64_t e) {
            std::memset(p + b, 0, static_cast<size_t>(e - b) * sizeof(double));
        });
    };
    zero(vt_all, static_cast<size_t>(m2l_pairs_ ? m2l_npar_ : n_pad) * hc.r_pad16);
    zero(u_all, m2l_pairs2_ ? static_cast<size_t>(hc.k_pad - hc.kp) * m2l_s2_plan_.n_par() : static_cast<size_t>(hc.k_pad) * n_pad);
    struct RowSrc {
        const M2lOperator *op;
// ... 35 lines not shown
            for (const RowSrc &rs : row_src) {
                const int r = rs.op->rank;
                const double *s0 = &rs.op->vt[static_cast<size_t>(rs.inv[j]) * r], *s1 = &rs.op->vt[static_cast<size_t>(rs.inv[rj]) * r];
                for (int kk = 0; kk < r; ++kk) {
                    if (centre) {
                        de[rs.first_row + kk] = s0[kk];
                    } else {
                        de[rs.first_row + kk] = 0.5 * (s0[kk] + s1[kk]);
                        dod[rs.first_row + kk] = 0.5 * (s0[kk] - s1[kk]);
                    }
                }
            }
        });
    } else {
        parallel_for(n, 8, [&](int64_t m) {
            double *dst = vt_all + static_cast<size_t>(m) * hc.r_pad16;
            for (const RowSrc &rs : row_src) {
                const int r = rs.op->rank;
                const int im = rs.inv[m];
                if (compressed) {
                    const double *src = &rs.op->vt[static_cast<size_t>(im) * r];
                    for (int kk = 0; kk < r; ++kk) dst[rs.first_row + kk] = src[kk];
                } else {
                    dst[rs.first_row + im] = 1.0;
                }
            }
        });
    }
    if (m2l_pairs2_) {
        const int n_par = m2l_s2_plan_.n_par(), ne16 = m2l_s2_plan_.ne16();
        parallel_for(static_cast<int64_t>(hc.tgt_tv.size()), 1, [&](int64_t pos) {
            if (hc.tgt_pair[pos] == -2) return;
            const int tv = hc.tgt_tv[pos];
            const M2lOperator &op = lops[ops_.ref_lookup[tv]];
            const int32_t *inv = &ops_.invperm[static_cast<size_t>(ops_.perm_lookup[tv]) * n];
            const int row0 = hc.tgt_off[pos] - (hc.tgt_pair[pos] >= 0 ? 0 : hc.kp);
            for (int kk = 0; kk < op.rank; ++kk) {
                double *dst = u_all + static_cast<size_t>(row0 + kk) * n_par;
                const double *ucol = &op.u[static_cast<size_t>(kk) * n];
                for (int k = 0; m2l_s2_axes_ == 2 && k < n_par; ++k) {
                    const int32_t *nd = &m2l_s2_node_[static_cast<size_t>(4 * k)];
                    const int8_t *sg = &m2l_s2_sign_[static_cast<size_t>(4 * k)];
                    if (nd[0] < 0) continue;
                    int cnt = 0;
                    double half[2] = {0.0, 0.0};
                    for (int g = 0; g < 4; ++g)
                        if (nd[g] >= 0) {
                            half[g >> 1] += sg[g] * ucol[inv[nd[g]]];
                            ++cnt;
                        }
                    dst[k] = (half[0] + half[1]) / cnt;
                }
                if (m2l_s2_axes_ == 2) continue;
                for (int i = 0; i < m2l_ne_; ++i) {
                    const double a = ucol[inv[i]], b = ucol[inv[m2l_rho(i)]];
                    if (i >= m2l_no_) {
                        dst[i] = a;
                    } else {
                        dst[i] = 0.5 * (a + b);
                        dst[ne16 + i] = 0.5 * (a - b);
                    }
                }
            }
        });
        return;
    }
    parallel_for(static_cast<int64_t>(hc.tgt_tv.size()), 1, [&](int64_t pos) {
        const int tv = hc.tgt_tv[pos];
        const M2lOperator &op = lops[ops_.ref_lookup[tv]];
        const int32_t *inv = &ops_.invperm[static_cast<size_t>(ops_.perm_lookup[tv]) * n];
        for (int kk = 0; kk < op.rank; ++kk) {
            double *dst = u_all + static_cast<size_t>(hc.tgt_off[pos] + kk) * n_pad;
            const double *ucol = &op.u[static_cast<size_t>(kk) * n];
            for (int i = 0; i < n; ++i) dst[i] = ucol[inv[i]];
        }
    });
}


struct FmmTree::M2lSwitches {
    double cbuf_mb = 0.0;
    bool s1_pairs = true, s2_pairs = true;
    int s1_axes = 0, s2_axes = 0;
    int variant_min_tiles = 4;
    bool verbose = false;
    static M2lSwitches read() {
        M2lSwitches sw;
        auto number = [](const char *name, int unset) {
            const char *e = std::getenv(name);
            return e ? std::atoi(e) : unset;
        };
        if (const char *e = std::getenv("BBFMM_M2L_CBUF_MB")) sw.cbuf_mb = std::atof(e);
        sw.s1_pairs = number("BBFMM_M2L_S1_PAIRS", 1) != 0;
        sw.s2_pairs = number("BBFMM_M2L_S2_PAIRS", 1) != 0;
        sw.s1_axes = number("BBFMM_M2L_S1_AXES", 0);
        sw.s2_axes = number("BBFMM_M2L_S2_AXES", 0);
        sw.variant_min_tiles = number("BBFMM_M2L_VARIANTS", 4);
        sw.verbose = std::getenv("BBFMM_VERBOSE") != nullptr;
        return sw;
    }
};

struct FmmTree::M2lLists {
    std::vector<std::vector<int>> src, tgt;
    std::vector<std::vector<int>> tpos_src, tpos_tgt;
    std::vector<std::vector<int32_t>> tgt_pair;
    std::vector<std::vector<int8_t>> tgt_kind;
    std::vector<int> level_groups;
    std::vector<std::vector<int>> batch_of;
    void index(int nvec) {
        for (auto *p : {&tpos_src, &tpos_tgt}) {
            const std::vector<std::vector<int>> &lists = p == &tpos_src ? src : tgt;
            p->assign(lists.size(), std::vector<int>(static_cast<size_t>(nvec), -1));
            for (size_t o = 0; o < lists.size(); ++o)
                for (size_t i = 0; i < lists[o].size(); ++i) (*p)[o][static_cast<size_t>(lists[o][i])] = static_cast<int>(i);
        }
    }
};

struct FmmTree::M2lSlotLayout {
    std::vector<std::vector<int>> off_tgt;
    std::vector<int> k_pad, kp, kpy, pad;
};

struct FmmTree::M2lPairSplit {
    std::vector<size_t> x, y, singles;
};

struct FmmTree::M2lStage1Marks {
    std::vector<int32_t> pair;
    std::vector<int8_t> kind;
    std::vector<int32_t> row0;
    int rows = 0;
    int y_blk = -1;
    int pad_rows = 0;
};

struct FmmTree::M2lTargetOrder {
    std::vector<std::vector<int>> tgt;
    std::vector<std::vector<int32_t>> pair;
    std::vector<std::vector<int8_t>> kind;
    std::vector<M2lSlotLayout> layout;
    int64_t work = 0;
};

struct FmmTree::M2lLevel {
    int level;
    size_t first_class;
    const M2lLists &lists;
    const M2lSlotLayout &lay;
};

struct FmmTree::M2lBuildState {
    std::vector<int32_t> pos_in_class;
    std::vector<std::vector<M2lTileDesc>> tiles1_of_batch;
    std::vector<int32_t> variant_batch;
    std::vector<std::vector<int32_t>> zero_of_batch;
    int64_t bad_pairs = 0;
};

namespace {
inline int tv_comp(const Operators &ops, int tv, int a) { return ops.all_vecs[static_cast<size_t>(tv) * ops.d + a]; }

int target_class(const Operators &ops, int o, int tv) {
    int oc = 0;
    for (int a = 0; a < ops.d; ++a) {
        const int v = ((o >> a) & 1) + tv_comp(ops, tv, a);
        oc |= (((v % 2) + 2) % 2) << a;
    }
    return oc;
}

M2lTileDesc m2l_tile(int32_t level_class, int32_t first, int32_t count, int32_t pad, int32_t q_first = 0, int32_t q_count = 0) {
    M2lTileDesc td;
    std::memset(&td, 0, sizeof td);
    td.level_class = level_class;
    td.first = first;
    td.count = count;
    td.pad = pad;
// ... 137 lines not shown
    mk.kind.assign(tvs.size(), 0);
    mk.row0.assign(tvs.size(), 0);
    for (size_t pos = 0; m2l_pairs_ && pos + 1 < tvs.size(); ++pos) {
        const size_t a = static_cast<size_t>(tvs[pos]), b = static_cast<size_t>(tvs[pos + 1]);
        const bool px = m2l_partner_[a] == tvs[pos + 1] && m2l_partner_[b] == tvs[pos];
        const bool py = !px && axes == 2 && m2l_partner_y_[a] == tvs[pos + 1] && m2l_partner_y_[b] == tvs[pos];
        if (px || py) {
            mk.pair[pos] = static_cast<int32_t>(pos + 1);
            mk.pair[pos + 1] = -2;
            mk.kind[pos] = mk.kind[pos + 1] = px ? 1 : 2;
            ++pos;
        }
    }
    int rows = 0, blk = -1, blk_first = 0;
    int last_x_blk = -1;
    for (size_t pos = 0; pos < tvs.size(); ++pos) {
        if (mk.pair[pos] == -2) continue;
        const int r = lops[ops_.ref_lookup[tvs[pos]]].rank;
        if (r == 0) continue;
        if (mk.kind[pos] == 2 && mk.y_blk < 0) {
            if (rows / m2l_s1_block_ <= last_x_blk) {
                mk.pad_rows = round_up(rows, m2l_s1_block_) - rows;
                rows += mk.pad_rows;
            }
            mk.y_blk = rows / m2l_s1_block_;
        }
        const int last = mk.pair[pos] >= 0 ? static_cast<int>(pos) + 1 : static_cast<int>(pos);
        if (rows / m2l_s1_block_ == blk && last - blk_first + 1 > kM2lSlotWindow) rows = round_up(rows, m2l_s1_block_);
        mk.row0[pos] = rows;
        const int b1 = (rows + r - 1) / m2l_s1_block_;
        if (rows / m2l_s1_block_ != blk || b1 != blk) {
            blk = b1;
            blk_first = static_cast<int>(pos);
        }
        if (mk.kind[pos] == 1) last_x_blk = b1;
        rows = round_up(rows + r, 2);
    }
    mk.rows = rows;
    return mk;
}

std::vector<uint8_t> FmmTree::m2l_classes_present(int level) const {
    std::vector<uint8_t> has(size_t(1) << d_, 0);
    for (int64_t c = tree_.level_ptr[level]; c < tree_.level_ptr[level + 1]; ++c) has[tree_.octant[c]] = 1;
    return has;
}

void FmmTree::choose_m2l_stage1_axes(const M2lSwitches &sw, M2lLists *lists) {
    m2l_axes_ = 1;
    m2l_s_ee_ = m2l_s_eo_ = 0;
    m2l_s1_off_ = M2lParityOffsets{{0, m2l_ne16_, m2l_ne16_, m2l_npar_}};
    m2l_work_[0] = m2l_work_[1] = 0;
    m2l_par_node_.clear();
    m2l_par_sign_.clear();
    if (!m2l_pairs_) return;
    const M2lParts q(ops_);
    M2lParityOffsets off2{{0, 0, 0, 0}};
    for (int i = 1; i < 4; ++i) off2.v[i] = off2.v[i - 1] + round_up(q.len[i - 1], 16);
    const int npar2 = off2.v[3] + round_up(q.len[3], 16);
    std::vector<std::vector<int>> src_x = lists->src, src_xy = lists->src;
    for (size_t o = 0; o < src_x.size(); ++o) {
        m2l_order_stage1(false, &src_x[o], nullptr);
        m2l_order_stage1(true, &src_xy[o], nullptr);
    }
    auto blocks = [&](int rows) { return static_cast<int64_t>(round_up(std::max(rows, 1), m2l_s1_block_) / m2l_s1_block_); };
    for (int level = 2; level <= tree_.depth; ++level) {
        const std::vector<uint8_t> has = m2l_classes_present(level);
        for (size_t o = 0; o < has.size(); ++o) {
            if (!has[o]) continue;
            m2l_work_[0] += blocks(m2l_mark_stage1(level, 1, src_x[o]).rows) * (m2l_npar_ / 16);
            m2l_work_[1] += blocks(m2l_mark_stage1(level, 2, src_xy[o]).rows) * (npar2 / 16);
        }
    }
    const bool two = sw.s1_axes == 2 || (sw.s1_axes != 1 && m2l_work_[1] < m2l_work_[0]);
    lists->src = std::move(two ? src_xy : src_x);
    if (!two) return;
    m2l_axes_ = 2;
    m2l_s1_off_ = off2;
    m2l_ne16_ = off2.v[2];
    m2l_npar_ = npar2;
    m2l_s_ee_ = off2.v[1] / 16;
    m2l_s_eo_ = (off2.v[2] - off2.v[1]) / 16;
    m2l_orbit_tables(q, npar2, [&](int part, int j) { return off2.v[part] + j; }, &m2l_par_node_, &m2l_par_sign_, nullptr);
}

FmmTree::M2lTargetOrder FmmTree::m2l_target_order(const std::vector<std::vector<int>> &tgt, int axes) const {
    M2lTargetOrder to;
    const size_t ncls = tgt.size();
    to.tgt.resize(ncls);
    to.pair.resize(ncls);
    to.kind.resize(ncls);
    for (size_t o = 0; o < ncls; ++o) {
        if (axes == 0) {
            to.tgt[o] = tgt[o];
            to.pair[o].assign(tgt[o].size(), -1);
            to.kind[o].assign(tgt[o].size(), 0);
            continue;
        }
        const M2lPairSplit ps = m2l_split_pairs(tgt[o], axes == 2);
        for (int part = 0; part < 3; ++part) {
            const std::vector<size_t> &src = part == 0 ? ps.x : part == 1 ? ps.y : ps.singles;
            for (size_t i = 0; i < src.size(); ++i) {
                const int32_t pos = static_cast<int32_t>(to.tgt[o].size());
                to.tgt[o].push_back(tgt[o][src[i]]);
                to.pair[o].push_back(part == 2 ? -1 : (i & 1) ? -2 : pos + 1);
                to.kind[o].push_back(static_cast<int8_t>(part == 2 ? 0 : part + 1));
            }
        }
    }
    to.layout.resize(static_cast<size_t>(tree_.depth) + 1);
    for (int level = 2; level <= tree_.depth; ++level) to.layout[static_cast<size_t>(level)] = m2l_slot_layout(level, to);
    return to;
}

FmmTree::M2lSlotLayout FmmTree::m2l_slot_layout(int level, const M2lTargetOrder &to) const {
    const auto &lops = ops_.m2l[level];
    const size_t ncls = to.tgt.size();
    M2lSlotLayout lay;
    lay.off_tgt.assign(ncls, {});
    for (auto *v : {&lay.k_pad, &lay.kp, &lay.kpy, &lay.pad}) v->assign(ncls, 0);
    for (size_t o = 0; o < ncls; ++o) {
        const std::vector<int> &tl = to.tgt[o];
        auto seg = [&](size_t pos) { return round_up(lops[ops_.ref_lookup[tl[pos]]].rank, 2); };
        int lead = 0, lead_y = 0;
        bool has_y = false;
        for (size_t pos = 0; pos < tl.size(); ++pos)
            if (to.pair[o][pos] >= 0) {
                (to.kind[o][pos] == 2 ? lead_y : lead) += seg(pos);
                has_y = has_y || to.kind[o][pos] == 2;
            }
        const int kp = has_y ? round_up(round_up(lead, 16) + lead_y, 16) : round_up(lead, 16);
        const int kpy = has_y ? round_up(lead, 16) : kp;
        int off = 0, off_s = 2 * kp;
        bool in_y = false;
        for (size_t pos = 0; pos < tl.size(); ++pos) {
            if (to.pair[o][pos] >= 0) {
                if (to.kind[o][pos] == 2 && !in_y) {
                    off = kpy;
                    in_y = true;
                }
                lay.off_tgt[o].push_back(off);
            } else if (to.pair[o][pos] == -2) {
                lay.off_tgt[o].push_back(kp + off);
                off += seg(pos);
            } else {
                lay.off_tgt[o].push_back(off_s);
                off_s += seg(pos);
            }
        }
        lay.k_pad[o] = round_up(std::max(off_s, 16), 16);
        lay.kp[o] = kp;
        lay.kpy[o] = kpy;
        lay.pad[o] = has_y ? kpy - lead : 0;
    }
    return lay;
}

void FmmTree::choose_m2l_stage2_axes(const M2lSwitches &sw, M2lLists *lists, std::vector<M2lSlotLayout> *layouts) {
    m2l_s2_axes_ = 1;
    m2l_s2_work_[0] = m2l_s2_work_[1] = 0;
    m2l_s2_node_.clear();
    m2l_s2_sign_.clear();
    m2l_s2_part_.clear();
    M2lTargetOrder one = m2l_target_order(lists->tgt, m2l_pairs2_ ? 1 : 0), two;
    bool pick_two = false;
    if (m2l_pairs2_) {
// ... 94 lines not shown
            if (tv >= 0 && tv < 384) bits[tv >> 6] |= 1ull << (tv & 63);
        }
        for (uint64_t b : bits) hsh = (hsh ^ b) * 1099511628211ull;
        key[static_cast<size_t>(c - c_lo)] = (static_cast<uint64_t>(1023 - std::min<int64_t>(nv, 1023)) << 54) | (hsh >> 10);
    }
    std::vector<int32_t> &pos_in_class = st->pos_in_class;
    parallel_for(int64_t(1) << d_, 1, [&](int64_t o) {
        auto &cells = m2l_host_[lv.first_class + static_cast<size_t>(o)].cells;
        std::stable_sort(cells.begin(), cells.end(), [&](int32_t a, int32_t b) {
            return key[static_cast<size_t>(a - c_lo)] < key[static_cast<size_t>(b - c_lo)];
        });
        for (size_t i = 0; i < cells.size(); ++i) pos_in_class[cells[i]] = static_cast<int32_t>(i);
    });
}

bool FmmTree::m2l_stage1_rows(const M2lLevel &lv, int o, const std::vector<int> &tvs, HostM2lClass *hcp) {
    HostM2lClass &hc = *hcp;
    const auto &lops = ops_.m2l[lv.level];
    auto rank_of = [&](int tv) { return lops[ops_.ref_lookup[tv]].rank; };
    auto slot_off = [&](int tv) {
        const int oc = target_class(ops_, o, tv);
        return lv.lay.off_tgt[oc][lv.lists.tpos_tgt[oc][tv]];
    };
    M2lStage1Marks mk = m2l_mark_stage1(lv.level, m2l_axes_, tvs);
    hc.n_t = static_cast<int>(tvs.size());
    hc.n_rows = mk.rows;
    hc.src_pair = std::move(mk.pair);
    hc.src_kind = std::move(mk.kind);
    hc.pad_cols = mk.pad_rows;
    hc.r_pad16 = round_up(std::max(hc.n_rows, 1), m2l_s1_block_);
    hc.yb0 = mk.y_blk >= 0 ? mk.y_blk : hc.r_pad16 / m2l_s1_block_;
    hc.row_tpos.assign(hc.r_pad16, -1);
    hc.row_off.assign(hc.r_pad16, 0);
    hc.row_tpos2.assign(hc.r_pad16, -1);
    hc.row_off2.assign(hc.r_pad16, 0);
    hc.src_tv = tvs;
    int row = 0;
    hc.src_row0.assign(tvs.size(), 0);
    hc.src_row1.assign(tvs.size(), 0);
    for (size_t pos = 0; pos < tvs.size(); ++pos) {
        if (hc.src_pair[pos] == -2) {
            hc.src_row0[pos] = hc.src_row0[pos - 1];
            hc.src_row1[pos] = hc.src_row1[pos - 1];
            continue;
        }
        const int tv = tvs[pos];
        const int base_off = slot_off(tv), base_off2 = hc.src_pair[pos] >= 0 ? slot_off(tvs[pos + 1]) : 0;
        if (rank_of(tv) > 0) row = mk.row0[pos];
        hc.src_row0[pos] = row;
        for (int kk = 0; kk < rank_of(tv); ++kk, ++row) {
            hc.row_tpos[row] = static_cast<int32_t>(pos);
            hc.row_off[row] = base_off + kk;
            if (hc.src_pair[pos] >= 0) {
                hc.row_tpos2[row] = static_cast<int32_t>(pos + 1);
                hc.row_off2[row] = base_off2 + kk;
            }
        }
        hc.src_row1[pos] = row;
        row = round_up(row, 2);
    }
    const int n_blk = hc.r_pad16 / m2l_s1_block_;
    m2l_max_blocks_ = std::max(m2l_max_blocks_, n_blk);
    hc.blk_t0.assign(n_blk, 0);
    hc.row_dst.assign(hc.r_pad16, -1);
    hc.row_dst2.assign(hc.r_pad16, -1);
    for (int b = 0; b < n_blk; ++b) {
        int t0 = -1, t1 = -1;
        bool two = false;
        for (int r = b * m2l_s1_block_; r < (b + 1) * m2l_s1_block_; ++r) {
            if (hc.row_tpos[r] < 0) continue;
            if (t0 < 0) t0 = hc.row_tpos[r];
            t1 = std::max(hc.row_tpos[r], hc.row_tpos2[r]);
            two = two || hc.row_tpos2[r] >= 0;
        }
        if (t0 < 0) continue;
        hc.blk_t0[b] = t0 | (two ? kM2lBlkTwoDst : 0);
        m2l_slot_t_ = std::max(m2l_slot_t_, t1 - t0 + 1);
        for (int r = b * m2l_s1_block_; r < (b + 1) * m2l_s1_block_; ++r) {
            if (hc.row_tpos[r] < 0) continue;
            if (hc.row_off[r] >= (1 << 24) || hc.row_off2[r] >= (1 << 24)) return false;
            hc.row_dst[r] = ((hc.row_tpos[r] - t0) << 24) | hc.row_off[r];
            if (hc.row_tpos2[r] >= 0) hc.row_dst2[r] = ((hc.row_tpos2[r] - t0) << 24) | hc.row_off2[r];
        }
    }
    return true;
}

int FmmTree::fill_m2l_classes(const M2lLevel &lv) {
    const M2lLists &ls = lv.lists;
    for (int o = 0; o < (1 << d_); ++o) {
        HostM2lClass &hc = m2l_host_[lv.first_class + o];
        hc.level = lv.level;
        hc.octant = o;
        hc.k_pad = lv.lay.k_pad[o];
        hc.kp = lv.lay.kp[o];
        hc.kpy = lv.lay.kpy[o];
        hc.tgt_pad = lv.lay.pad[o];
        hc.tgt_pair = ls.tgt_pair[o];
        hc.tgt_kind = ls.tgt_kind[o];
        if (!m2l_stage1_rows(lv, o, ls.src[o], &hc)) return fail(BBFMM_BAD_ARGUMENT, "M2L slot too long for the packed row table");
        if (hc.cells.empty()) continue;
        hc.tgt_tv = ls.tgt[o];
        hc.tgt_off = lv.lay.off_tgt[o];
        if (host_only_) fill_m2l_operator_arrays(hc, &hc.vt_all, &hc.u_all);
        hc.cbase.resize(hc.cells.size());
        int64_t &cursor = m2l_batches_[static_cast<size_t>(ls.batch_of[lv.level][o])].len;
        for (size_t i = 0; i < hc.cells.size(); ++i) {
            hc.cbase[i] = cursor;
            cursor += hc.k_pad;
        }
        hc.cslot.resize(hc.cells.size() * static_cast<size_t>(hc.n_t));
        int32_t *cs = hc.cslot.data();
        parallel_for_chunks(static_cast<int64_t>(hc.cslot.size()), int64_t(1) << 18, [&](int64_t b, int64_t e) {
            std::fill(cs + b, cs + e, int32_t(-1));
        });
    }
    return BBFMM_OK;
}

void FmmTree::fill_m2l_cslot(const M2lLevel &lv, M2lBuildState *st) {
    const HostTree &t = tree_;
    const int n = ops_.n, nvec = ops_.n_vec, level = lv.level;
    const bool compressed = ops_.compression != kCompressionNone;
    const auto &lops = ops_.m2l[level];
    const M2lLists &ls = lv.lists;
    const std::vector<int32_t> &pos_in_class = st->pos_in_class;
    const int64_t b0 = t.level_ptr[level], nb_cells = t.level_ptr[level + 1] - b0;
    constexpr int64_t kChunkB = 2048;
    const int64_t nch = (nb_cells + kChunkB - 1) / kChunkB;
    std::vector<double> flops_part(static_cast<size_t>(std::max<int64_t>(nch, 1)), 0.0);
    std::vector<int64_t> bad_part(static_cast<size_t>(std::max<int64_t>(nch, 1)), 0);
    parallel_for_chunks(nb_cells, kChunkB, [&](int64_t lo, int64_t hi) {
        double fl = 0.0;
        int64_t bad = 0;
        for (int64_t B = b0 + lo; B < b0 + hi; ++B) {
            const HostM2lClass &hb = m2l_host_[lv.first_class + t.octant[B]];
            const int64_t base = hb.cbase[pos_in_class[B]];
            for (int64_t q = t.v.ptr[B]; q < t.v.ptr[B + 1]; ++q) {
                const int32_t V = t.v.idx[q];
                const int tv = t.v_tidx[q];
                HostM2lClass &hv = m2l_host_[lv.first_class + t.octant[V]];
                const int ps = (tv >= 0 && tv < nvec) ? ls.tpos_src[t.octant[V]][tv] : -1;
                if (ps < 0 || t.level[V] != level || ls.tpos_tgt[t.octant[B]][tv] < 0) {
                    ++bad;
                    continue;
                }
                hv.cslot[static_cast<size_t>(pos_in_class[V]) * hv.n_t + ps] = static_cast<int32_t>(base / 2);
                fl += compressed ? 4.0 * n * lops[ops_.ref_lookup[tv]].rank : 2.0 * n * static_cast<double>(n);
            }
        }
        flops_part[static_cast<size_t>(lo / kChunkB)] = fl;
        bad_part[static_cast<size_t>(lo / kChunkB)] = bad;
    });
    double level_flops = 0.0;
    for (double f : flops_part) level_flops += f;
    m2l_flops_k1_ += level_flops;
    if (m2l_flops_level_.size() <= static_cast<size_t>(level)) m2l_flops_level_.resize(static_cast<size_t>(level) + 1, 0.0);
    m2l_flops_level_[static_cast<size_t>(level)] = level_flops;
    for (int64_t b : bad_part) st->bad_pairs += b;
}

void FmmTree::m2l_zero_segments(const M2lLevel &lv, M2lBuildState *st) const {
    const HostTree &t = tree_;
    const auto &lops = ops_.m2l[lv.level];
    for (int o = 0; o < (1 << d_); ++o) {
        const HostM2lClass &hc = m2l_host_[lv.first_class + o];
// ... 166 lines not shown
    return BBFMM_OK;
}

int FmmTree::build_m2l_level(const M2lLevel &lv, const M2lSwitches &sw, M2lBuildState *st) {
    m2l_host_.resize(lv.first_class + (size_t(1) << d_));
    m2l_group_ops_.resize(m2l_host_.size());
    sort_m2l_class_cells(lv, st);
    CHK(fill_m2l_classes(lv));
    fill_m2l_cslot(lv, st);
    if (m2l_batches_.size() > 1) m2l_zero_segments(lv, st);
    m2l_stage2_tiles(lv);
    return lv.lists.level_groups[lv.level] > 1 ? m2l_group_operators(lv, st) : m2l_boundary_variants(lv, sw, st);
}

int FmmTree::finish_m2l_launch_lists(const M2lLists &lists, const M2lBuildState &st) {
    if (st.bad_pairs > 0)
        return fail(BBFMM_UNSUPPORTED,
                    "V-list pairs outside the admissible transfer-vector set (source points outside the root box?)");
    m2l_batch_of_class_.assign(m2l_host_.size() + m2l_variants_.size(), 0);
    for (size_t lc = 0; lc < m2l_host_.size(); ++lc)
        m2l_batch_of_class_[lc] = lists.batch_of[static_cast<size_t>(m2l_host_[lc].level)][static_cast<size_t>(m2l_host_[lc].octant)];
    for (size_t v = 0; v < m2l_variants_.size(); ++v) m2l_batch_of_class_[m2l_host_.size() + v] = st.variant_batch[v];
    size_t next = 0;
    for (size_t b = 0; b < m2l_batches_.size(); ++b) {
        M2lBatch &mb = m2l_batches_[b];
        mb.t1_first = static_cast<int32_t>(m2l_tiles1_h_.size());
        for (M2lTileDesc td : st.tiles1_of_batch[b]) {
            if (td.level_class < 0) td.level_class = static_cast<int32_t>(m2l_host_.size()) + (-1 - td.level_class);
            m2l_tiles1_h_.push_back(td);
        }
        mb.t1_count = static_cast<int32_t>(m2l_tiles1_h_.size()) - mb.t1_first;
        std::vector<M2lTileDesc> part;
        while (next < m2l_tiles_h_.size() && m2l_batch_of_class_[static_cast<size_t>(m2l_tiles_h_[next].level_class)] == static_cast<int32_t>(b))
            part.push_back(m2l_tiles_h_[next++]);
        split_tile_tail(&part, n_cu_);
        mb.t2_first = static_cast<int32_t>(m2l_tiles2_h_.size());
        mb.t2_count = static_cast<int32_t>(part.size());
        m2l_tiles2_h_.insert(m2l_tiles2_h_.end(), part.begin(), part.end());
        cbuf_batch_len_ = std::max(cbuf_batch_len_, mb.len);
    }
    if (next != m2l_tiles_h_.size()) return fail(BBFMM_DEVICE_ERROR, "internal: M2L tiles out of batch order");
    m2l_zero_h_.clear();
    m2l_zero_ptr_.assign(m2l_batches_.size() + 1, 0);
    for (size_t b = 0; b < m2l_batches_.size(); ++b) {
        m2l_zero_h_.insert(m2l_zero_h_.end(), st.zero_of_batch[b].begin(), st.zero_of_batch[b].end());
        m2l_zero_ptr_[b + 1] = static_cast<int64_t>(m2l_zero_h_.size() / 2);
    }
    cbuf_batch_len_ += 128;
    if (cbuf_batch_len_ / 2 >= (int64_t(1) << 31))
        return fail(BBFMM_UNSUPPORTED, "M2L intermediate buffer of one batch too large (raise the number of groups: lower BBFMM_M2L_CBUF_MB)");
    return BBFMM_OK;
}

int FmmTree::build_m2l_tables() {
    clear_m2l_tables();
    if (tree_.depth < 2) return BBFMM_OK;
    const M2lSwitches sw = M2lSwitches::read();
    if (!host_only_) {
        size_t free_b = 0, total_b = 0;
        if (hipMemGetInfo(&free_b, &total_b) == hipSuccess && total_b > 0)
            m2l_budget_bytes_ = std::max<int64_t>(int64_t(4) << 30, static_cast<int64_t>(total_b / 16));
    }
    if (sw.cbuf_mb > 0) m2l_budget_bytes_ = static_cast<int64_t>(sw.cbuf_mb * 1048576.0);
    init_m2l_parity_basis(sw);
    const int ncls = 1 << d_;
    M2lLists lists;
    lists.src.resize(ncls);
    lists.tgt.resize(ncls);
    for (int o = 0; o < ncls; ++o)
        for (int tv = 0; tv < ops_.n_vec; ++tv) {
            int mx = 0;
            bool okt = true, oks = true;
            for (int a = 0; a < d_; ++a) {
                const int oa = (o >> a) & 1, ta = tv_comp(ops_, tv, a);
                mx = std::max(mx, std::abs(ta));
                okt = okt && ta >= oa - 3 && ta <= oa + 2;
                oks = oks && ta >= -2 - oa && ta <= 3 - oa;
            }
            if (mx >= 2 && okt) lists.tgt[o].push_back(tv);
            if (mx >= 2 && oks) lists.src[o].push_back(tv);
        }
    std::vector<M2lSlotLayout> layouts;
    choose_m2l_stage1_axes(sw, &lists);
    choose_m2l_stage2_axes(sw, &lists, &layouts);
    lists.index(ops_.n_vec);
    plan_m2l_batches(sw, layouts, &lists);
    M2lBuildState st;
    st.pos_in_class.assign(static_cast<size_t>(tree_.n_cells()), -1);
    st.tiles1_of_batch.resize(m2l_batches_.size());
    st.zero_of_batch.resize(m2l_batches_.size());
    for (int level = 2; level <= tree_.depth; ++level)
        CHK(build_m2l_level(M2lLevel{level, m2l_host_.size(), lists, layouts[static_cast<size_t>(level)]}, sw, &st));
    return finish_m2l_launch_lists(lists, st);
}

}
```

### ferreus_rbf_rs_amd/csrc/fmm_tree.cpp

```cpp
#include "fmm_tree_impl.hpp"
#include "interpolant_terms.hpp"

namespace bbfmm {

int FmmTree::fail(int code, const std::string &msg) {
    err_ = msg;
    return code;
}
int FmmTree::hip_fail(hipError_t e, const char *what) {
    err_ = std::string("HIP error: ") + hipGetErrorString(e) + " in " + what;
    return BBFMM_DEVICE_ERROR;
}

void FmmTree::arena_begin() {
    arena_active_ = true;
    arena_used_ = 0;
    arena_need_ = 0;
}
int FmmTree::arena_end() {
    arena_active_ = false;
    if (arena_need_ > arena_.n) {
        dfree(&arena_);
        CHK(dalloc(&arena_, arena_need_ + arena_need_ / 4));
    }
// ... 377 lines not shown
        std::vector<double> c3(static_cast<size_t>(C) * 3, 0.0);
        for (int64_t c = 0; c < C; ++c)
            for (int a = 0; a < d; ++a) c3[c * 3 + a] = t.centers[c * d + a];
        CHK(dupload(&d_centers_, c3));
        CHK(dupload(&d_lengths_, t.lengths));
        std::vector<int32_t> b(C), e(C);
        for (int64_t c = 0; c < C; ++c) {
            b[c] = static_cast<int32_t>(t.pt_begin[c]);
            e[c] = static_cast<int32_t>(t.pt_end[c]);
        }
        CHK(dupload(&d_pt_begin_, b));
        CHK(dupload(&d_pt_end_, e));
        CHK(dupload(&d_parent_, t.parent));
        CHK(dupload(&d_octant_, t.octant));
        CHK(dupload(&d_child_ptr_, t.children.ptr));
        CHK(dupload(&d_child_idx_, t.children.idx));
        CHK(dupload(&d_src_leaves_, src_leaves_));
    }
    d_m2m_parents_.resize(level_cells_.size());
    d_level_cells_.resize(level_cells_.size());
    for (size_t l = 0; l < level_cells_.size(); ++l) {
        CHK(dupload(&d_m2m_parents_[l], m2m_parents_[l]));
        CHK(dupload(&d_level_cells_[l], level_cells_[l]));
    }
    CHK(dupload(&d_u_run_ptr_, u_runs_.ptr));
    CHK(dupload(&d_u_runs_, u_runs_.idx));
    CHK(dupload(&d_w_ptr_, t.w.ptr));
    CHK(dupload(&d_w_idx_, t.w.idx));
    {
        std::vector<int64_t> job_ptr(x_cells_.size() + 1, 0);
        std::vector<int32_t> job_runs;
        for (size_t j = 0; j < x_cells_.size(); ++j) {
            const int32_t c = x_cells_[j];
            for (int64_t r = x_runs_.ptr[c]; r < x_runs_.ptr[c + 1]; ++r) {
                job_runs.push_back(x_runs_.idx[2 * r]);
                job_runs.push_back(x_runs_.idx[2 * r + 1]);
            }
            job_ptr[j + 1] = static_cast<int64_t>(job_runs.size() / 2);
        }
        CHK(dupload(&d_x_cells_, x_cells_));
        CHK(dupload(&d_x_job_run_ptr_, job_ptr));
        CHK(dupload(&d_x_runs_, job_runs));
    }
    StageTimer ut;
    HIPCHK(hipStreamSynchronize(stream_));
    ut.lap("  upload: tree, run lists");
    m2l_classes_h_.resize(m2l_host_.size() + m2l_variants_.size());
    const bool compressed = ops_.compression != kCompressionNone;
    DevBuf<int32_t> d_invperm;
    CHK(dupload(&d_invperm, ops_.invperm));
    std::vector<DevBuf<double>> d_level_ops(ops_.m2l.size());
    std::vector<std::vector<int64_t>> u_off(ops_.m2l.size()), vt_off(ops_.m2l.size());
    for (size_t lv = 0; lv < ops_.m2l.size(); ++lv) {
        std::vector<double> buf;
        for (const M2lOperator &op : ops_.m2l[lv]) {
            u_off[lv].push_back(static_cast<int64_t>(buf.size()));
            buf.insert(buf.end(), op.u.begin(), op.u.end());
            vt_off[lv].push_back(static_cast<int64_t>(buf.size()));
            buf.insert(buf.end(), op.vt.begin(), op.vt.end());
        }
        if (!buf.empty()) CHK(dupload(&d_level_ops[lv], buf));
    }
    if (shared_basis_) {
        if (!compressed) return fail(BBFMM_BAD_ARGUMENT, "BBFMM_FLAG_M2L_SHARED_BASIS needs compressed M2L operators (ACA or SVD)");
        CHK(build_shared_basis(&d_level_ops));
    }
    const int m2l_len = shared_basis_ ? basis_pad_ : cheb_.n_pad;
    std::vector<DevBuf<double>> natural_tmp;
    std::vector<DevBuf<M2lAssembleTv>> assemble_tmp;
    for (size_t i = 0; i < m2l_host_.size() + m2l_variants_.size(); ++i) {
        HostM2lClass &h = i < m2l_host_.size() ? m2l_host_[i] : m2l_variants_[i - m2l_host_.size()];
        M2lClass &c = m2l_classes_h_[i];
        std::memset(&c, 0, sizeof c);
        c.n_rows = h.n_rows;
        c.r_pad16 = h.r_pad16;
        c.n_t = h.n_t;
        c.k_pad = h.k_pad;
        c.kp = h.kp;
        c.kpy = h.kpy;
        c.yb0 = h.yb0;
        c.n_cells = static_cast<int32_t>(h.cells.size());
        if (h.cells.empty()) continue;
        DevBuf<double> vt, ua;
        DevBuf<int32_t> rt, rt2, ro, ce, cs;
        DevBuf<int64_t> cb;
        {
            const size_t nvt = static_cast<size_t>(m2l_pairs_ ? m2l_npar_ : cheb_.n_pad) * h.r_pad16, nu = m2l_pairs2_ ? static_cast<size_t>(h.k_pad - h.kp) * m2l_s2_plan_.n_par() : static_cast<size_t>(h.k_pad) * cheb_.n_pad;
            CHK(dalloc(&vt, nvt));
            CHK(dalloc(&ua, nu));
            const auto &lops = ops_.m2l[h.level];
            std::vector<M2lAssembleTv> src_tv, tgt_tv;
            int max_rank = 0;
            for (size_t pos = 0; pos < h.src_tv.size(); ++pos) {
                if (m2l_pairs_ && h.src_pair[pos] == -2) continue;
                const int tv = h.src_tv[pos];
                const int ref = ops_.ref_lookup[tv];
                const int rank = lops[ref].rank;
                src_tv.push_back(M2lAssembleTv{ops_.perm_lookup[tv], rank, h.src_row0[pos], vt_off[h.level][ref], u_off[h.level][ref]});
            }
            for (size_t pos = 0; pos < h.tgt_tv.size(); ++pos) {
                if (m2l_pairs2_ && h.tgt_pair[pos] == -2) continue;
                const int tv = h.tgt_tv[pos];
                const int ref = ops_.ref_lookup[tv];
                const int rank = lops[ref].rank;
                max_rank = std::max(max_rank, rank);
                const int row = m2l_pairs2_ && h.tgt_pair[pos] < 0 ? h.tgt_off[pos] - h.kp : h.tgt_off[pos];
                tgt_tv.push_back(M2lAssembleTv{ops_.perm_lookup[tv], rank, row, vt_off[h.level][ref], u_off[h.level][ref]});
            }
            DevBuf<M2lAssembleTv> d_src, d_tgt;
            CHK(dupload(&d_src, src_tv));
            CHK(dupload(&d_tgt, tgt_tv));
            const M2lAssembleClass ac{d_src.p, d_tgt.p, static_cast<int32_t>(src_tv.size()), static_cast<int32_t>(tgt_tv.size()),
                                      h.r_pad16, h.k_pad, max_rank,
                                      m2l_pairs_ ? m2l_ne_ : 0, m2l_no_, m2l_ne16_, m2l_npar_, ops_.p,
                                      m2l_pairs2_ ? m2l_s2_plan_.n_par() : 0, m2l_s2_plan_.ne16(), h.k_pad - h.kp, m2l_ne_, m2l_no_,
                                      m2l_axes_, m2l_s1_off_, m2l_pairs2_ && m2l_s2_axes_ == 2 ? m2l_s2_plan_ : M2lS2PairsPlan{1, 1, 1, 1}};
            static const bool host_fill = std::getenv("BBFMM_M2L_ASSEMBLE_HOST") != nullptr;
            if (host_fill) {
                std::vector<double> hv, hu;
                fill_m2l_operator_arrays(h, &hv, &hu);
                HIPCHK(hipMemcpy(vt.p, hv.data(), hv.size() * sizeof(double), hipMemcpyHostToDevice));
                HIPCHK(hipMemcpy(ua.p, hu.data(), hu.size() * sizeof(double), hipMemcpyHostToDevice));
            } else {
                launch_m2l_assemble(ac, ops_.n, cheb_.n_pad, compressed, d_level_ops[h.level].p, d_invperm.p, vt.p, ua.p, stream_);
            }
            assemble_tmp.push_back(d_src);
            assemble_tmp.push_back(d_tgt);
            if (shared_basis_) {
                DevBuf<double> vt2, ua2;
                CHK(dalloc(&vt2, static_cast<size_t>(m2l_len) * h.r_pad16));
                CHK(dalloc(&ua2, static_cast<size_t>(h.k_pad) * m2l_len));
                const double *W = d_basis_c_[static_cast<size_t>(h.level)].p;
                launch_small_gemm(true, m2l_len, h.r_pad16, cheb_.n_pad, W, m2l_len, vt.p, h.r_pad16, vt2.p, h.r_pad16, stream_);
                launch_small_gemm(false, h.k_pad, m2l_len, cheb_.n_pad, ua.p, cheb_.n_pad, W, m2l_len, ua2.p, m2l_len, stream_);
                natural_tmp.push_back(vt);
                natural_tmp.push_back(ua);
                vt = vt2;
                ua = ua2;
            }
        }
        CHK(dupload(&rt, h.row_dst));
        CHK(dupload(&rt2, h.row_dst2));
        CHK(dupload(&ro, h.blk_t0));
        CHK(dupload(&ce, h.cells));
        CHK(dalloc(&cs, h.cslot.size()));
        if (!h.cslot.empty()) HIPCHK(hipMemcpy(cs.p, h.cslot.data(), h.cslot.size() * sizeof(int32_t), hipMemcpyHostToDevice));
        CHK(dupload(&cb, h.cbase));
        c.vt_all = vt.p;
        c.u_all = ua.p;
        c.row_dst = rt.p;
        c.row_dst2 = rt2.p;
        c.blk_t0 = ro.p;
        c.cells = ce.p;
        c.cslot = cs.p;
        c.cbase = cb.p;
        decltype(h.cslot)().swap(h.cslot);
    }
    HIPCHK(hipStreamSynchronize(stream_));
    HIPCHK(hipGetLastError());
    for (auto &b : assemble_tmp) dfree(&b);
    for (auto &b : natural_tmp) dfree(&b);
    for (auto &b : d_level_ops) dfree(&b);
    dfree(&d_invperm);
    ut.lap("  upload: M2L operators, tables");
    CHK(dupload(&d_m2l_classes_, m2l_classes_h_));
    CHK(dupload(&d_m2l_tiles_, m2l_tiles_h_));
    CHK(dupload(&d_m2l_tiles1_, m2l_tiles1_h_));
    CHK(dupload(&d_tile_idx1_, m2l_tile_idx1_h_));
    CHK(dupload(&d_m2l_tiles2_, m2l_tiles2_h_));
    CHK(dupload(&d_m2l_zero_, m2l_zero_h_));
    decltype(m2l_zero_h_)().swap(m2l_zero_h_);
    CHK(dupload(&d_m2l_qlist_, m2l_qlist_h_));
    std::vector<uint8_t> act(static_cast<size_t>(C), 1);
    CHK(dupload(&d_active_, act));
    {
        const char *e = std::getenv("BBFMM_FUSED_PASSES");
        fused_mask_ = e ? static_cast<unsigned>(std::atoi(e)) & 15u : 15u;
        if (!(fused_mask_ & 2u)) fused_mask_ &= ~4u;
        const char *lp = std::getenv("BBFMM_LEAF_PASSES");
        leaf_mask_ = lp ? static_cast<unsigned>(std::atoi(lp)) & 1u : 1u;
        int n_cu = 256, dev = 0;
        if (hipGetDevice(&dev) != hipSuccess || hipDeviceGetAttribute(&n_cu, hipDeviceAttributeMultiprocessorCount, dev) != hipSuccess || n_cu <= 0)
            n_cu = 256;
        const char *rm = std::getenv("BBFMM_L2P_RUNS_MIN");
        l2p_runs_min_ = rm ? std::max(0, std::atoi(rm)) : 4 * n_cu;
        std::vector<uint8_t> has_m2l(static_cast<size_t>(C), 0), has_x(static_cast<size_t>(C), 0);
        fused_flags_ok_ = true;
        for (const M2lTileDesc &td : m2l_tiles2_h_) {
            const size_t lc = static_cast<size_t>(td.level_class);
            const HostM2lClass &h = lc < m2l_host_.size() ? m2l_host_[lc] : m2l_variants_[lc - m2l_host_.size()];
            if (td.pad != 0 || td.first < 0 || static_cast<size_t>(td.first) + td.count > h.cells.size()) {
                fused_flags_ok_ = false;
                break;
            }
            for (int32_t q = 0; q < td.count; ++q) has_m2l[static_cast<size_t>(h.cells[static_cast<size_t>(td.first + q)])] = 1;
        }
        for (int32_t c : x_cells_) has_x[static_cast<size_t>(c)] = 1;
        CHK(dupload(&d_has_m2l_, has_m2l));
        CHK(dupload(&d_has_x_, has_x));
        std::vector<int32_t> top;
        for (size_t l = 0; l < level_cells_.size() && l < 2; ++l) top.insert(top.end(), level_cells_[l].begin(), level_cells_[l].end());
        n_top_cells_ = static_cast<int>(top.size());
        CHK(dupload(&d_top_cells_, top));
    }
    return BBFMM_OK;
}

M2lParityRowArgs FmmTree::mp_row_args() const {
    M2lParityRowArgs a;
    a.axes = m2l_axes_;
    a.n_par = m2l_npar_;
    a.p = ops_.p;
    a.ne16 = m2l_ne16_;
    a.n_e = m2l_ne_;
    a.n_o = m2l_no_;
    a.p1 = m2l_ne_ / ((ops_.p + 1) / 2);
    a.off = m2l_s1_off_;
    a.p2 = ops_.n / (ops_.p * ops_.p);
    return a;
}

M2lUnparityRowArgs FmmTree::lp_row_args() const {
    M2lUnparityRowArgs a;
    a.axes = m2l_s2_axes_;
    a.n_par = m2l_s2_plan_.n_par();
    a.p = ops_.p;
    a.ne16 = m2l_s2_plan_.ne16();
    a.n_e = m2l_ne_;
    a.n_o = m2l_no_;
    a.p1 = m2l_ne_ / ((ops_.p + 1) / 2);
    a.plan = m2l_s2_plan_;
    a.p2 = ops_.n / (ops_.p * ops_.p);
    return a;
}

// ... 279 lines not shown
            HIPCHK(hipMemsetAsync(d_M_.p + static_cast<size_t>(j) * C * cheb_.n_pad, 0,
                                  static_cast<size_t>(dp->coarse_cells) * cheb_.n_pad * sizeof(double), stream_));
        launch_p2m(cheb_, src_ptr_, d_w_sorted_.p, t.n_points, k, C, dp->d_up_leaves.p, static_cast<int>(dp->up_leaves_h.size()),
                   d_pt_begin_.p, d_pt_end_.p, d_centers_.p, d_lengths_.p, d_M_.p, stream_);
    } else {
        launch_p2m(cheb_, src_ptr_, d_w_sorted_.p, t.n_points, k, C, d_src_leaves_.p, static_cast<int>(src_leaves_.size()),
                   d_pt_begin_.p, d_pt_end_.p, d_centers_.p, d_lengths_.p, d_M_.p, stream_);
    }
    phase_end(kPhP2M);
    phase_begin();
    for (int level = t.depth - 1; level >= 1; --level) {
        const int rc = part ? launch_m2m(cheb_, k, C, dp->d_up_parents[level].p, static_cast<int>(dp->up_parents_h[level].size()),
                                         dp->d_part_child_ptr.p, dp->d_part_child_idx.p, d_octant_.p, d_M_.p, stream_)
                            : launch_m2m(cheb_, k, C, d_m2m_parents_[level].p, static_cast<int>(m2m_parents_[level].size()),
                                         d_child_ptr_.p, d_child_idx_.p, d_octant_.p, d_M_.p, stream_, fuse_mp ? &mp_args : nullptr,
                                         fuse_mp ? d_Mp_.p : nullptr);
        if (rc != 0) return hip_fail(static_cast<hipError_t>(rc), "M2M: dynamic LDS attribute");
    }
    if (fuse_mp) {
        launch_m2l_parity_cells(d_M_.p, cheb_.n_pad, d_Mp_.p, mp_args, d_top_cells_.p, n_top_cells_, k, C, stream_);
        mp_current_k_ = k;
    }
    phase_end(kPhM2M);
    HIPCHK(hipGetLastError());
    return BBFMM_OK;
}

int FmmTree::downward(int k, const DownwardPlan *dp, const TargetSet *wx) {
    CHK(downward_m2l(k, dp));
    return downward_tail(k, dp, wx);
}

int FmmTree::downward_m2l(int k, const DownwardPlan *dp) {
    const HostTree &t = tree_;
    const int64_t C = t.n_cells();
    have_locals_ = false;
    lp_pending_ = false;
    const bool s2_pairs = m2l_pairs2_ && !m2l_batches_.empty();
    const int lp_len = m2l_s2_plan_.n_par();
    if (!s2_pairs) HIPCHK(hipMemsetAsync(d_L_.p, 0, static_cast<size_t>(k) * C * cheb_.n_pad * sizeof(double), stream_));
    const int m2l_len = shared_basis_ ? basis_pad_ : cheb_.n_pad;
    const double *m_in = shared_basis_ ? d_Mc_.p : m2l_pairs_ ? d_Mp_.p : d_M_.p;
    const int s1_len = m2l_pairs_ ? m2l_npar_ : m2l_len, s1_ne16 = m2l_pairs_ ? m2l_ne16_ : 0;
    if (m2l_pairs_ && !m2l_batches_.empty() && mp_current_k_ < k) {
        phase_begin();
        if (m2l_axes_ == 2)
            launch_m2l_parity2(d_M_.p, cheb_.n_pad, d_Mp_.p, m2l_npar_, m2l_s1_off_, ops_.p, ops_.n / (ops_.p * ops_.p), static_cast<int64_t>(k) * C, stream_);
        else
            launch_m2l_parity(d_M_.p, cheb_.n_pad, d_Mp_.p, m2l_npar_, m2l_ne16_, m2l_ne_, m2l_no_, ops_.p, static_cast<int64_t>(k) * C, stream_);
        phase_end(kPhM2L1);
    }
    double *l_out = shared_basis_ ? d_Lc_.p : s2_pairs ? d_Lp_.p : d_L_.p;
    if (shared_basis_) {
        phase_begin();
        launch_m2l_basis(d_basis_classes_.p, d_basis_tiles_c_.p, n_basis_tiles_, cheb_.n_pad, basis_pad_, k, C, d_M_.p, d_Mc_.p, stream_);
        HIPCHK(hipMemsetAsync(d_Lc_.p, 0, static_cast<size_t>(k) * C * basis_pad_ * sizeof(double), stream_));
        phase_end(kPhM2L1);
    }
    const int nb = static_cast<int>(m2l_batches_.size());
    const bool fuse_lp = s2_pairs && !dp && l2l_fusable(k);
    bool clear_lp = true;
    if (fuse_lp && (fused_mask_ & 4u)) {
        clear_lp = false;
        for (const M2lBatch &mb : m2l_batches_)
            if (mb.t2_count > 0 && m2l_s2_pairs_ksplit(mb.t2_count, m2l_s2_plan_, k, !deterministic_) > 1) clear_lp = true;
    }
    for (int k0 = 0; k0 < k; k0 += m2l_rhs_chunk_) {
        const int kb = std::min(m2l_rhs_chunk_, k - k0);
        const double *m_chunk = m_in + static_cast<size_t>(k0) * C * s1_len;
        double *l_chunk = s2_pairs ? d_Lp_.p : l_out + static_cast<size_t>(k0) * C * m2l_len;
        if (s2_pairs && clear_lp) HIPCHK(hipMemsetAsync(d_Lp_.p, 0, static_cast<size_t>(kb) * C * lp_len * sizeof(double), stream_));
        for (int b = 0; b < nb; ++b) {
            const M2lBatch &mb = m2l_batches_[static_cast<size_t>(b)];
            const int t1_first = dp ? dp->batch_t1[4 * b] : mb.t1_first, t1_count = dp ? dp->batch_t1[4 * b + 1] : mb.t1_count;
            const int t2_first = dp ? dp->batch_t2[2 * b] : mb.t2_first, t2_count = dp ? dp->batch_t2[2 * b + 1] : mb.t2_count;
            if (t2_count == 0) continue;
            phase_begin();
            if (nb > 1)
                launch_m2l_zero_segments(d_m2l_zero_.p + 2 * m2l_zero_ptr_[static_cast<size_t>(b)],
                                         m2l_zero_ptr_[static_cast<size_t>(b) + 1] - m2l_zero_ptr_[static_cast<size_t>(b)], kb, d_cbuf_.p,
                                         cbuf_batch_len_, stream_);
            if (dp) {
                launch_m2l_stage1(d_m2l_classes_.p, dp->d_tiles1.p + t1_first, dp->d_tile_idx.p, t1_count, s1_len, m2l_slot_t_, kb,
                                  C, m_chunk, d_cbuf_.p, cbuf_batch_len_, stream_, false, m2l_max_blocks_, s1_ne16, m2l_s_ee_, m2l_s_eo_);
                launch_m2l_stage1(d_m2l_classes_.p, dp->d_tiles1.p + dp->batch_t1[4 * b + 2], dp->d_tile_idx.p, dp->batch_t1[4 * b + 3],
                                  s1_len, m2l_slot_t_, kb, C, m_chunk, d_cbuf_.p, cbuf_batch_len_, stream_, true, m2l_max_blocks_, s1_ne16, m2l_s_ee_, m2l_s_eo_);
            } else
                launch_m2l_stage1(d_m2l_classes_.p, d_m2l_tiles1_.p + t1_first, d_tile_idx1_.p, t1_count, s1_len, m2l_slot_t_, kb, C,
                                  m_chunk, d_cbuf_.p, cbuf_batch_len_, stream_, false, m2l_max_blocks_, s1_ne16, m2l_s_ee_, m2l_s_eo_);
            phase_end(kPhM2L1);
            phase_begin();
            if (s2_pairs) {
                if (!launch_m2l_stage2_pairs(d_m2l_classes_.p, dp ? dp->d_tiles2.p + t2_first : d_m2l_tiles2_.p + t2_first,
                                             dp ? dp->d_tile_idx.p : nullptr, t2_count, m2l_s2_plan_, kb, C, d_cbuf_.p, cbuf_batch_len_,
                                             dp ? dp->d_qlist.p : d_m2l_qlist_.p, l_chunk, stream_, !deterministic_, &m2l_s2_last_ksplit_))
                    return fail(BBFMM_DEVICE_ERROR, "internal: no stage-2 kernel instance for the parity-basis column plan");
            } else if (dp)
                launch_m2l_stage2(d_m2l_classes_.p, dp->d_tiles2.p + t2_first, dp->d_tile_idx.p, t2_count, m2l_len, kb, C, d_cbuf_.p,
                                  cbuf_batch_len_, dp->d_qlist.p, l_chunk, stream_, !deterministic_);
            else
                launch_m2l_stage2(d_m2l_classes_.p, d_m2l_tiles2_.p + t2_first, nullptr, t2_count, m2l_len, kb, C, d_cbuf_.p,
                                  cbuf_batch_len_, d_m2l_qlist_.p, l_chunk, stream_, !deterministic_);
            phase_end(kPhM2L2);
        }
        if (fuse_lp) {
            lp_pending_ = true;
        } else if (s2_pairs) {
            phase_begin();
            if (m2l_s2_axes_ == 2)
                launch_m2l_unparity2(d_Lp_.p, m2l_s2_plan_, d_L_.p + static_cast<size_t>(k0) * C * cheb_.n_pad, ops_.n, cheb_.n_pad, ops_.p,
                                     ops_.n / (ops_.p * ops_.p), static_cast<int64_t>(kb) * C, stream_);
            else
                launch_m2l_unparity(d_Lp_.p, lp_len, m2l_s2_plan_.ne16(), d_L_.p + static_cast<size_t>(k0) * C * cheb_.n_pad, ops_.n, cheb_.n_pad,
                                    m2l_ne_, m2l_no_, ops_.p, static_cast<int64_t>(kb) * C, stream_);
            phase_end(kPhM2L2);
        }
    }
    if (shared_basis_) {
        phase_begin();
        launch_m2l_basis(d_basis_classes_.p, d_basis_tiles_e_.p, n_basis_tiles_, basis_pad_, cheb_.n_pad, k, C, d_Lc_.p, d_L_.p, stream_);
        phase_end(kPhM2L2);
    }
    HIPCHK(hipGetLastError());
    (void)t;
    return BBFMM_OK;
}

int FmmTree::downward_tail(int k, const DownwardPlan *dp, const TargetSet *wx) {
    const HostTree &t = tree_;
    const int64_t C = t.n_cells();
    const bool fuse_lp = lp_pending_ && !dp;
    lp_pending_ = false;
    const M2lUnparityRowArgs lp_args = lp_row_args();
    phase_begin();
    if (fuse_lp && t.adaptive) launch_zero_rows(d_x_cells_.p, static_cast<int>(x_cells_.size()), cheb_.n_pad, k, C, d_L_.p, stream_);
    if (t.adaptive && wx) {
        launch_wx_sym(kernel_, cheb_, wx->n_wx_jobs, wx->wx_tb.p, wx->wx_te.p, wx->wx_range.p, wx->n_wxl_jobs, wx->wxl_tb.p, wx->wxl_te.p,
                      wx->wxl_range.p, d_w_idx_.p, d_centers_.p,
                      d_lengths_.p, src_ptr_, d_w_sorted_.p, t.n_points, k, d_M_.p, d_L_.p, C * cheb_.n_pad, wx->out.p,
                      static_cast<int64_t>(wx->m), wx->sym_off, static_cast<int>(wx->m), stream_);
    } else if (t.adaptive) {
        if (dp)
            launch_p2l(kernel_, cheb_, dp->n_x_jobs, dp->d_x_cells.p, dp->d_x_ptr.p, dp->d_x_runs.p, d_centers_.p,
                       d_lengths_.p, src_ptr_, d_w_sorted_.p, t.n_points, k, C, d_L_.p, stream_);
        else
            launch_p2l(kernel_, cheb_, static_cast<int>(x_cells_.size()), d_x_cells_.p, d_x_job_run_ptr_.p,
                       d_x_runs_.p, d_centers_.p, d_lengths_.p, src_ptr_, d_w_sorted_.p, t.n_points, k, C, d_L_.p,
                       stream_);
    }
    phase_end(kPhP2L);
    phase_begin();
    for (int level = 2; level <= t.depth; ++level) {
        const int rc = launch_l2l(cheb_, k, C, d_level_cells_[level].p, static_cast<int>(level_cells_[level].size()), d_parent_.p,
                                  d_octant_.p, dp ? dp->d_active.p : d_active_.p, d_L_.p, stream_, fuse_lp ? &lp_args : nullptr,
                                  fuse_lp ? d_Lp_.p : nullptr, fuse_lp ? d_has_m2l_.p : nullptr, fuse_lp ? d_has_x_.p : nullptr);
        if (rc != 0) return hip_fail(static_cast<hipError_t>(rc), "L2L: dynamic LDS attribute");
    }
    phase_end(kPhL2L);
    HIPCHK(hipGetLastError());
    have_locals_ = dp == nullptr;
    return BBFMM_OK;
}

hipError_t FmmTree::columns_to_host(double *dst, int64_t ld, const double *d_src, int64_t m, int ncols) {
    if (m <= 0 || ncols <= 0) return hipSuccess;
    if (ld == m) return hipMemcpyAsync(dst, d_src, static_cast<size_t>(m) * ncols * sizeof(double), hipMemcpyDeviceToHost, stream_);
    for (int j = 0; j < ncols; ++j) {
        const hipError_t e = hipMemcpyAsync(dst + static_cast<size_t>(j) * ld, d_src + static_cast<size_t>(j) * m,
                                            static_cast<size_t>(m) * sizeof(double), hipMemcpyDeviceToHost, stream_);
        if (e != hipSuccess) return e;
    }
    return hipSuccess;
// ... 769 lines not shown
```

### ferreus_rbf_rs_amd/csrc/fmm_tree.hpp

```cpp
#pragma once
#include <hip/hip_runtime.h>

#include <cstdint>
#include <string>
#include <memory>
#include <vector>

#include "device.hpp"
#include "targets.hpp"
#include "ferreus_bbfmm_hip.h"
#include "kernels.hpp"
#include "operators.hpp"
#include "parallel.hpp"
#include "tree.hpp"
#include "tree_device.hpp"

namespace bbfmm {

enum Phase {
    kPhGather = 0, kPhP2M, kPhM2M, kPhM2L1, kPhM2L2, kPhP2L, kPhL2L, kPhP2P, kPhM2P, kPhL2P, kPhScatter,
    kNumPhases
};
static_assert(kNumPhases == BBFMM_N_PHASES, "phase table");

template <class T> struct DevBuf {
    T *p = nullptr;
    size_t n = 0;
    bool borrowed = false;
};

struct HostM2lClass {
    int level = 0, octant = 0;
    int n_rows = 0, r_pad16 = 16, n_t = 0, k_pad = 16;
    std::vector<double> vt_all, u_all;
    std::vector<int> src_tv, tgt_tv, tgt_off;
    std::vector<int32_t> row_tpos, row_off, row_dst, blk_t0, cells;
    std::vector<int32_t, DefaultInitAllocator<int32_t>> cslot;
    std::vector<int32_t> src_row0, src_row1;
    std::vector<int32_t> row_tpos2, row_off2, row_dst2;
    std::vector<int32_t> src_pair;
    std::vector<int8_t> src_kind;
    int yb0 = 0;
    int pad_cols = 0;
    int kp = 0;
    std::vector<int32_t> tgt_pair;
    std::vector<int8_t> tgt_kind;
    int kpy = 0;
    int tgt_pad = 0;
    std::vector<int64_t> cbase;
};

struct M2lBatch {
    int level_lo = 0, level_hi = 0;
    int groups = 1, group = 0;
    int64_t len = 0;
    int32_t t1_first = 0, t1_count = 0;
    int32_t t2_first = 0, t2_count = 0;
};

struct TargetSet {
    int64_t m = 0;
    DevBuf<double> xyz[3];
    const double *xyz_ptr[3] = {nullptr, nullptr, nullptr};
    DevBuf<int32_t> perm;
    DevBuf<int32_t> job_cell, tgt_begin, tgt_end;
    int n_jobs = 0;
    int n_l2p_runs = 0, n_l2p_rest = 0;
    DevBuf<int32_t> l2p_runs, l2p_rest_cell, l2p_rest_begin, l2p_rest_end;
    DevBuf<int32_t> w_tgt_begin, w_tgt_end;
    DevBuf<int64_t> w_begin, w_end;
    int n_w_jobs = 0;
    DevBuf<double> out, grad;
    bool sym = false;
    int32_t sym_off = 0;
    int n_sym_jobs = 0;
    DevBuf<int32_t> sym_tb, sym_te;
    DevBuf<int64_t> sym_ptr;
    DevBuf<int32_t> sym_runs;
    int n_syml_jobs = 0;
    DevBuf<int32_t> syml_tb, syml_te;
    DevBuf<int64_t> syml_ptr;
    int n_symw_jobs = 0;
    DevBuf<int32_t> symw_tb, symw_te;
    DevBuf<int64_t> symw_ptr;
    int n_wx_jobs = 0;
    DevBuf<int32_t> wx_tb, wx_te;
    DevBuf<int64_t> wx_range;
    int n_wxl_jobs = 0;
    DevBuf<int32_t> wxl_tb, wxl_te;
    DevBuf<int64_t> wxl_range;
};

struct DownwardPlan {
    std::vector<uint8_t> active;
    std::vector<M2lTileDesc> tiles2_h;
    std::vector<M2lTileDesc> tiles1_h;
    std::vector<int32_t> batch_t1, batch_t2;
    int64_t n_tiles1_blocks = 0;
    std::vector<int32_t> tile_idx_h;
    std::vector<uint16_t> qlist_h;
    int n_x_jobs = 0;
    bool restrict_upward = false;
    int coarse_level = 0;
    int64_t coarse_cells = 0;
    std::vector<int32_t> up_leaves_h;
    std::vector<std::vector<int32_t>> up_parents_h;
    std::vector<int64_t> part_child_ptr_h;
    std::vector<int32_t> part_child_idx_h;
    std::vector<uint8_t> reads_h;
    std::vector<int32_t> gather_pos_h;
    DevBuf<int32_t> d_gather_pos;
    DevBuf<int32_t> d_up_leaves;
    std::vector<DevBuf<int32_t>> d_up_parents;
    DevBuf<int64_t> d_part_child_ptr;
    DevBuf<int32_t> d_part_child_idx;
    DevBuf<uint8_t> d_active;
    DevBuf<M2lTileDesc> d_tiles2, d_tiles1;
    DevBuf<int32_t> d_tile_idx, d_x_cells, d_x_runs;
    DevBuf<int64_t> d_x_ptr;
    DevBuf<uint16_t> d_qlist;
};

struct TargetSetStats {
    int64_t runs = 0, jobs = 0, largest = 0, w_jobs = 0;
};

// ... 9 lines not shown
class DeviceGroup;
struct InterpolantTerms;

class FmmTree {
    friend class DeviceGroup;
  public:
    FmmTree() = default;
    ~FmmTree();
    FmmTree(const FmmTree &) = delete;
    FmmTree &operator=(const FmmTree &) = delete;

    int create(const double *pts, int64_t n, int d, int64_t ld, int order, int kernel_type, double base_range,
               double total_sill, bool adaptive, bool sparse, const double *extents, const bbfmm_params *params,
               uint32_t flags);
    int set_weights(const double *w, int64_t rows, int k, int64_t ldw);
    int set_local_coefficients(const double *w, int64_t rows, int k, int64_t ldw);
    int evaluate_leaves_device(const double *d_x0, const double *d_x1, const double *d_x2, int64_t m, double *d_out,
                               int64_t *bad_point_index, double *d_grad = nullptr, bool batch_independent = false);
    int evaluate_device(const double *d_x, int64_t m, int64_t ldx, const InterpolantTerms *terms, double *d_values, int64_t ldo,
                        double *d_grad, int64_t ldg, bool batch_independent, int32_t max_job_targets, int64_t *bad_point_index,
                        TargetSetStats *stats = nullptr);
    int nrhs() const { return nrhs_; }
    bool supports_gradients() const;
    int evaluate(const double *w, int64_t rows, int k, int64_t ldw, const double *x, int64_t m, int64_t ldx,
                 double *out, int64_t ldo, double *grad, int64_t ldg, bool with_grads, bool leaves_only,
                 int64_t *bad_point_index);
    int prepare_target_subset(const int64_t *target_indices, int64_t n_target_indices);
    bool is_identity_subset(const int64_t *idx, int64_t n_idx) const;
    int fast_matrix_vector_product(const double *w, int64_t rows, int64_t basis_size, const int64_t *target_indices,
                                   int64_t n_target_indices, const double *poly, int64_t ldp, double nugget,
                                   double *result);
    int matvec_device(const double *d_w, int64_t ldw, int k, double *d_out, int64_t ldo, bool sync);
    int64_t partition_coarse_count() const;
    int matvec_partition_upward(const double *d_w, int64_t ldw, int k, double *d_coarse, hipStream_t comm_stream, bool near_field = true);
    int partition_subset_finish(const double *d_coarse, const int64_t *idx, int64_t n_idx, double *h_out, hipStream_t comm_stream);
    int matvec_partition_finish(const double *d_coarse, double *d_out, int64_t ldo, bool sync, hipStream_t comm_stream);
    int matvec_partition_finish_sorted(const double *d_coarse, double *d_seg, int64_t ld, hipStream_t comm_stream);
    int partition_scatter(const double *d_all, int first_part, int n_parts, int64_t m_max, int k, double *d_out, int64_t ldo);
    int matvec_partition_finish_host(const double *d_coarse, double *h_seg, int64_t ld, hipStream_t comm_stream);
    const std::vector<int64_t> &partition_bounds() const { return part_bounds_; }
    int register_subset(const int64_t *idx, int64_t n_idx, int *id_out);
    int matvec_subset_device(int id, const double *d_w, double *d_y, bool sync);
    int set_partition(int rank, int world);

    const HostTree &tree() const { return tree_; }
    const Operators &ops() const { return ops_; }
    const PodDoubles &source_points() const { return pts_; }
    int order() const { return order_; }
    const char *last_error() const { return err_.c_str(); }
    hipStream_t stream() const { return stream_; }
    bool host_only() const { return host_only_; }
    bool deterministic() const { return deterministic_; }
    bool leaves_ready() const { return nrhs_ == 1 && have_locals_; }
    void bind_device() const {
        if (device_ >= 0) (void)hipSetDevice(device_);
    }
    int device() const { return device_; }
    bool tree_built_on_device() const { return tree_built_on_device_; }
    bool last_evaluate_at_sources() const { return last_eval_at_sources_; }
    int last_evaluate_path() const { return last_eval_at_sources_ ? 1 : (last_eval_rows_of_sources_ ? 2 : 0); }
    bool targets_are_rows_of_sources(const double *x, int64_t m, int64_t ldx, std::vector<int64_t> *rows);
    bool targets_are_sources(const double *x, int64_t m, int64_t ldx) const;
    void stats(bbfmm_tree_stats *out) const;
    void set_profiling(bool on) { profiling_ = on; }
    const double *phase_ms() { collect_phase_times(); return phase_ms_; }
    const int64_t *phase_count() { collect_phase_times(); return phase_count_; }
    void reset_phase_ms() {
        collect_phase_times();
        for (double &v : phase_ms_) v = 0.0;
        for (int64_t &v : phase_count_) v = 0;
    }
    const std::vector<int64_t> &partition_rows() const { return part_rows_; }
    bool partitioned() const { return part_world_ > 1; }
    int partition_rank() const { return part_rank_; }
    const std::vector<HostM2lClass> &m2l_host() const { return m2l_host_; }
    void m2l_variant_stats(int64_t *n_variants, int64_t *n_cells) const {
        *n_variants = static_cast<int64_t>(m2l_variants_.size());
        *n_cells = 0;
        for (const HostM2lClass &v : m2l_variants_) *n_cells += static_cast<int64_t>(v.cells.size());
    }
    void debug_m2l_pairs(std::vector<int32_t> *out) const;
    bool m2l_pairs() const { return m2l_pairs_; }
    void debug_m2l_pairs_axes(std::vector<int32_t> *out) const;
    void debug_m2l_pairs_stage2(std::vector<int32_t> *out) const;
    bool m2l_pairs_stage2() const { return m2l_pairs2_; }
    void debug_m2l_pairs_axes_stage2(std::vector<int32_t> *out) const;
    static constexpr int kM2lDigestFamilies = 8;
    void debug_m2l_table_digests(std::vector<uint64_t> *out) const;
    const std::vector<double> &m2l_flops_level() const { return m2l_flops_level_; }
    int debug_m2l_s2_last_ksplit() const { return m2l_s2_last_ksplit_; }
    void debug_leaf_runs(int32_t *counts) const {
        counts[0] = static_cast<int32_t>(leaf_mask_);
        counts[1] = src_targets_.n_l2p_runs;
        counts[2] = src_targets_.n_l2p_rest;
        counts[3] = src_targets_.n_jobs;
    }
    int debug_apply_m2l_tables_host(const double *M, double *L) const;
    int debug_get_coefficients(char which, int k, double *out);
    int debug_m2l_parity_len() const { return m2l_pairs_ ? m2l_npar_ : 0; }
    int debug_partition_upward_counts(int64_t *counts_out, uint8_t *reads_out, int64_t *info_out) const;

  private:
    int fail(int code, const std::string &msg);
    int hip_fail(hipError_t e, const char *what);
    int upload();
    int build_m2l_tables();
    struct M2lSwitches;
    struct M2lLists;
    struct M2lSlotLayout;
    struct M2lPairSplit;
    struct M2lStage1Marks;
    struct M2lTargetOrder;
    struct M2lLevel;
    struct M2lBuildState;
    void clear_m2l_tables();
    void init_m2l_parity_basis(const M2lSwitches &sw);
    std::vector<int32_t> m2l_reflection_partners(int axis) const;
    M2lPairSplit m2l_split_pairs(const std::vector<int> &list, bool with_y) const;
    void m2l_order_stage1(bool with_y, std::vector<int> *list, std::vector<int> *carry) const;
    M2lStage1Marks m2l_mark_stage1(int level, int axes, const std::vector<int> &tvs) const;
    M2lTargetOrder m2l_target_order(const std::vector<std::vector<int>> &tgt, int axes) const;
    M2lSlotLayout m2l_slot_layout(int level, const M2lTargetOrder &order) const;
    std::vector<uint8_t> m2l_classes_present(int level) const;
    void choose_m2l_stage1_axes(const M2lSwitches &sw, M2lLists *lists);
    void choose_m2l_stage2_axes(const M2lSwitches &sw, M2lLists *lists, std::vector<M2lSlotLayout> *layouts);
    void plan_m2l_batches(const M2lSwitches &sw, const std::vector<M2lSlotLayout> &layouts, M2lLists *lists);
    int build_m2l_level(const M2lLevel &lv, const M2lSwitches &sw, M2lBuildState *st);
    void sort_m2l_class_cells(const M2lLevel &lv, M2lBuildState *st);
    bool m2l_stage1_rows(const M2lLevel &lv, int o, const std::vector<int> &tvs, HostM2lClass *hc);
    int fill_m2l_classes(const M2lLevel &lv);
    void fill_m2l_cslot(const M2lLevel &lv, M2lBuildState *st);
    void m2l_zero_segments(const M2lLevel &lv, M2lBuildState *st) const;
    void m2l_stage2_tiles(const M2lLevel &lv);
    bool m2l_restricted_operator(const M2lLevel &lv, const HostM2lClass &hc, const std::vector<int> &tvs, const std::vector<int> &keep,
                                 size_t first, size_t count, HostM2lClass *v);
    int m2l_group_operators(const M2lLevel &lv, M2lBuildState *st);
    int m2l_boundary_variants(const M2lLevel &lv, const M2lSwitches &sw, M2lBuildState *st);
    int finish_m2l_launch_lists(const M2lLists &lists, const M2lBuildState &st);
    void fill_m2l_operator_arrays(const HostM2lClass &hc, std::vector<double> *vt_all,
                                  std::vector<double> *u_all) const;
    void fill_m2l_operator_arrays(const HostM2lClass &hc, double *vt_all, double *u_all) const;
    int ensure_rhs_capacity(int k);
    int upward(int k, const DownwardPlan *dp = nullptr);
    int downward(int k, const DownwardPlan *dp = nullptr, const TargetSet *wx = nullptr);
    int downward_m2l(int k, const DownwardPlan *dp);
    int downward_tail(int k, const DownwardPlan *dp, const TargetSet *wx);
    int leaf_pass(const TargetSet &ts, int k, bool with_grads, bool fixed_plan = false);
    int leaf_pass_near(const TargetSet &ts, int k, bool with_grads, hipStream_t st, int parts, bool wx_done = false,
                       bool fixed_plan = false);
    int leaf_pass_far(const TargetSet &ts, int k, bool with_grads, double *user_out = nullptr, int64_t ldo = 0);
    int build_target_set(const double *x, int64_t m, int64_t ldx, TargetSet *ts, int64_t *bad_point_index,
                         std::vector<int32_t> *leaves_out = nullptr);
    int build_target_set_device(const double *x, int64_t m, int64_t ldx, TargetSet *ts, int64_t *bad_point_index,
                                std::vector<int32_t> *leaves_out, const double *const *d_x = nullptr, int32_t cap = 0,
                                TargetSetStats *stats = nullptr);
    int ensure_leaf_lookup();
    int build_target_set_host(const double *x, int64_t m, int64_t ldx, TargetSet *ts, int64_t *bad_point_index,
                              std::vector<int32_t> *leaves_out);
    int build_source_target_set();
    int build_l2p_runs(TargetSet *ts, const std::vector<int32_t> &jc, const std::vector<int32_t> &tb, const std::vector<int32_t> &te);
    int build_sym_runs(TargetSet *ts, const std::vector<int32_t> &job_cells, int64_t pb, int64_t pe, const std::vector<uint8_t> *part_active = nullptr);
    void free_target_set(TargetSet *ts);
    hipError_t columns_to_host(double *dst, int64_t ld, const double *d_src, int64_t m, int ncols);
    int upload_weights(const double *w, int64_t rows, int k, int64_t ldw);
    void phase_begin();
    void phase_end(int ph);
    void collect_phase_times();
    hipEvent_t get_event();

    std::string err_;
    bool host_only_ = false;
    bool deterministic_ = false;
    bool tree_built_on_device_ = false;
    DevTreePoints dev_points_;
    int order_ = 0, d_ = 0;
    KernelSpec kernel_{};
    bbfmm_params params_{};
    PodDoubles pts_;
    HostTree tree_;
    Operators ops_;
    int nrhs_ = 0;
    bool have_locals_ = false;
    bool locals_requested_ = false;
    Csr u_runs_;
    Csr x_runs_;
    std::vector<int32_t> src_leaves_;
    std::vector<std::vector<int32_t>> m2m_parents_;
    std::vector<std::vector<int32_t>> level_cells_;
    std::vector<int32_t> x_cells_;
    std::vector<HostM2lClass> m2l_host_;
    std::vector<HostM2lClass> m2l_variants_;
    std::vector<M2lTileDesc> m2l_tiles1_h_;
    std::vector<int32_t> m2l_tile_idx1_h_;
    std::vector<M2lClass> m2l_classes_h_;
    std::vector<M2lTileDesc> m2l_tiles_h_;
    std::vector<uint16_t> m2l_qlist_h_;
    std::vector<M2lBatch> m2l_batches_;
    std::vector<int32_t> m2l_batch_of_class_;
    std::vector<std::vector<int32_t>> m2l_group_ops_;
    std::vector<int32_t> m2l_zero_h_;
    std::vector<int64_t> m2l_zero_ptr_;
    int64_t cbuf_batch_len_ = 0;
    int64_t cbuf_total_len_ = 0;
    int64_t m2l_budget_bytes_ = int64_t(16384) << 20;
    int m2l_rhs_chunk_ = 1;
    double m2l_flops_k1_ = 0;
    int n_cu_ = 256;
    int device_ = -1;
    std::vector<M2lTileDesc> m2l_tiles2_h_;
    int m2l_slot_t_ = 1;
    int m2l_max_blocks_ = 1;
    int m2l_s1_block_ = kM2lS1Block;
    bool m2l_pairs_ = false;
    int m2l_ne_ = 0, m2l_no_ = 0;
    int m2l_ne16_ = 0, m2l_npar_ = 0;
    std::vector<int32_t> m2l_partner_;
    int m2l_axes_ = 1;
    M2lParityOffsets m2l_s1_off_{{0, 0, 0, 0}};
    int m2l_s_ee_ = 0, m2l_s_eo_ = 0;
    int64_t m2l_work_[2] = {0, 0};
    std::vector<int32_t> m2l_partner_y_;
    std::vector<int32_t> m2l_par_node_;
    std::vector<int8_t> m2l_par_sign_;
    int m2l_rho_y(int m) const {
        const int p2 = ops_.n / (ops_.p * ops_.p);
        return m + (ops_.p - 1 - 2 * ((m / p2) % ops_.p)) * p2;
    }
    int m2l_rho(int m) const {
        const int p1 = ops_.n / ops_.p;
        return m + (ops_.p - 1 - 2 * (m / p1)) * p1;
    }
    DevBuf<double> d_Mp_;
    bool m2l_pairs2_ = false;
    M2lS2PairsPlan m2l_s2_plan_{1, 1, 1, 1};
    DevBuf<double> d_Lp_;
    int m2l_s2_last_ksplit_ = 0;
    int m2l_s2_axes_ = 1;
    int64_t m2l_s2_work_[2] = {0, 0};
    std::vector<int32_t> m2l_s2_node_;
    std::vector<int8_t> m2l_s2_sign_;
    std::vector<int8_t> m2l_s2_part_;
    unsigned fused_mask_ = 15;
    unsigned leaf_mask_ = 1;
    int l2p_runs_min_ = 1024;
    int mp_current_k_ = 0;
    bool lp_pending_ = false;
    bool fused_flags_ok_ = false;
    M2lParityRowArgs mp_row_args() const;
    M2lUnparityRowArgs lp_row_args() const;
    bool m2m_fusable() const;
    bool l2l_fusable(int k) const;
    DevBuf<uint8_t> d_has_m2l_, d_has_x_;
    DevBuf<int32_t> d_top_cells_;
    int n_top_cells_ = 0;
    int part_rank_ = 0, part_world_ = 1;
    std::vector<int64_t> part_rows_, part_bounds_;
    int partition_finish_core(const double *d_coarse, hipStream_t comm_stream, int *k_out);
    bool part_empty_ = false;
    DownwardPlan part_plan_;
    std::vector<std::unique_ptr<SubsetPlan>> subset_plans_;
    uint64_t subset_clock_ = 0;
    int build_downward_plan(const std::vector<int32_t> &target_leaves, DownwardPlan *dp, bool restrict_upward = false,
                            int64_t own_b = 0, int64_t own_e = 0);
    int part_pending_k_ = 0;
    bool multipoles_partial_ = false;
    void free_downward_plan(DownwardPlan *dp);
    int subset_plan(const int64_t *idx, int64_t n_idx, SubsetPlan **out);
    uint64_t subset_key(const int64_t *idx, int64_t n_idx) const;
    bool subset_plan_cached(const int64_t *idx, int64_t n_idx, uint64_t key) const;
    uint64_t last_subset_miss_ = 0;
    int fill_subset_plan(const int64_t *idx, int64_t n_idx, SubsetPlan *sp);
    std::vector<std::unique_ptr<SubsetPlan>> registered_plans_;

    hipStream_t stream_ = nullptr;
    hipEvent_t ev_pack_ = nullptr, ev_comm_ = nullptr;
    struct PendingPhase {
        int phase;
        hipEvent_t e0, e1;
    };
    std::vector<PendingPhase> pending_;
    std::vector<hipEvent_t> event_pool_;
    hipEvent_t pending_begin_ = nullptr;
    bool profiling_ = false;
    double phase_ms_[kNumPhases] = {0};
    int64_t phase_count_[kNumPhases] = {0};
    std::vector<void *> owned_;
    template <class T> int dalloc(DevBuf<T> *b, size_t n, bool zero = false);
    template <class T> int dupload(DevBuf<T> *b, const std::vector<T> &v);
    template <class T> int talloc(DevBuf<T> *b, size_t n, bool zero = false);
    template <class T> int tupload(DevBuf<T> *b, const std::vector<T> &v);
    void arena_begin();
    int arena_end();
    template <class T> void dfree(DevBuf<T> *b);

    ChebRef cheb_{};
    DevBuf<DevCheb> d_cheb_;
    DevBuf<double> d_src_[3];
    const double *src_ptr_[3] = {nullptr, nullptr, nullptr};
    DevBuf<double> d_zero_axis_;
    DevBuf<uint8_t> arena_;
    size_t arena_used_ = 0, arena_need_ = 0;
    bool arena_active_ = false;
    DevBuf<uint64_t> d_tab_keys_;
// ... 71 lines not shown
```

### ferreus_rbf_rs_amd/fmm_tree.py

```python
from __future__ import annotations

import ctypes
import enum
from typing import Optional

import numpy as np

from . import _lib as L


class KernelType(enum.IntEnum):
    LinearRbf = 0
    ThinPlateSplineRbf = 1
    CubicRbf = 2
    Spheroidal3Rbf = 3
    Spheroidal5Rbf = 4
    Spheroidal7Rbf = 5
    Spheroidal9Rbf = 6
    Laplacian = 7
    OneOverR2 = 8
    OneOverR4 = 9
    GaussianExt = 100
    MultiquadricExt = 101

# ... 533 lines not shown
                                                           None, None))
        nvec = 7 ** self.dim
        perm = np.zeros((nperm.value, n), dtype=np.int32)
        inv = np.zeros((nperm.value, n), dtype=np.int32)
        pl = np.zeros(nvec, dtype=np.int32)
        rl = np.zeros(nvec, dtype=np.int32)
        self._raise(self._lib.bbfmm_get_permutation_tables(
            self._h, ctypes.byref(nperm), perm.ctypes.data, inv.ctypes.data, pl.ctypes.data,
            rl.ctypes.data))
        return perm, inv, pl, rl

    def points_to_leaves(self, x):
        x = self._targets(x)
        m = x.shape[0]
        cells = np.zeros(max(m, 1), dtype=np.int32)
        bad = ctypes.c_int64(-1)
        rc = self._lib.bbfmm_points_to_leaves(self._h, x.ctypes.data, m, max(m, 1),
                                              cells.ctypes.data, ctypes.byref(bad))
        self._raise(rc, bad)
        return cells[:m]

    def debug_dense_m2m(self, child_index: int):
        n = self.stats().n_nodes
        out = np.zeros((n, n), order="F")
        self._raise(self._lib.bbfmm_debug_dense_m2m(self._h, child_index, out.ctypes.data))
        return out

    def debug_m2l_variants(self):
        nv, nc = ctypes.c_int64(), ctypes.c_int64()
        self._raise(self._lib.bbfmm_debug_m2l_variants(self._h, ctypes.byref(nv), ctypes.byref(nc)))
        return nv.value, nc.value

    def debug_m2l_pairs(self, stage=1):
        fn = self._lib.bbfmm_debug_m2l_pairs if stage == 1 else self._lib.bbfmm_debug_m2l_pairs_stage2
        n, on = ctypes.c_int64(), ctypes.c_int32()
        self._raise(fn(self._h, None, 0, ctypes.byref(n), ctypes.byref(on)))
        buf = np.zeros(max(n.value, 1), dtype=np.int32)
        self._raise(fn(self._h, buf.ctypes.data, n.value, ctypes.byref(n), ctypes.byref(on)))
        d, ops, i = self.dim, [], 0
        while i < n.value:
            level, octant, kind, ne = (int(v) for v in buf[i:i + 4])
            ent = buf[i + 4:i + 4 + ne * (d + 1)].reshape(ne, d + 1)
            ops.append({"level": level, "octant": octant, "kind": kind,
                        "pairs": [tuple(int(x) for x in e[1:]) for e in ent if e[0] == 1],
                        "singles": [tuple(int(x) for x in e[1:]) for e in ent if e[0] == 0]})
            i += 4 + ne * (d + 1)
        return bool(on.value), ops

    def debug_m2l_pairs_axes(self, stage=1):
        if stage == 2:
            fn = self._lib.bbfmm_debug_m2l_pairs_axes_stage2
            n = ctypes.c_int64()
            self._raise(fn(self._h, None, 0, ctypes.byref(n)))
            buf = np.zeros(max(n.value, 1), dtype=np.int32)
            self._raise(fn(self._h, buf.ctypes.data, n.value, ctypes.byref(n)))
            info = {"axes": int(buf[0]), "work_x": int(buf[1]), "work_xy": int(buf[2])}
            d, ops, i = self.dim, [], 3
            while i < n.value:
                level, octant, kp, kpy, k_pad, pad, ne = (int(v) for v in buf[i:i + 7])
                ent = buf[i + 7:i + 7 + ne * (d + 4)].reshape(ne, d + 4)
                by_kind = [{tuple(int(x) for x in e[4:]): (int(e[1]), int(e[2]), int(e[3])) for e in ent if e[0] == k}
                           for k in range(3)]
                ops.append({"level": level, "octant": octant, "kp": kp, "kpy": kpy, "k_pad": k_pad, "pad": pad,
                            "singles": by_kind[0], "x_pairs": by_kind[1], "y_pairs": by_kind[2]})
                i += 7 + ne * (d + 4)
            return info, ops
        fn = self._lib.bbfmm_debug_m2l_pairs_axes
        n = ctypes.c_int64()
        self._raise(fn(self._h, None, 0, ctypes.byref(n)))
        buf = np.zeros(max(n.value, 1), dtype=np.int32)
        self._raise(fn(self._h, buf.ctypes.data, n.value, ctypes.byref(n)))
        info = {"axes": int(buf[0]), "work_x": int(buf[1]), "work_xy": int(buf[2])}
        d, ops, i = self.dim, [], 3
        while i < n.value:
            level, octant, kind, pad_cols, yb0, n_blk, ne = (int(v) for v in buf[i:i + 7])
            kinds = [int(v) for v in buf[i + 7:i + 7 + n_blk]]
            ent = buf[i + 7 + n_blk:i + 7 + n_blk + ne * (d + 3)].reshape(ne, d + 3)
            by_kind = [{tuple(int(x) for x in e[3:]): (int(e[1]), int(e[2])) for e in ent if e[0] == k} for k in range(3)]
            ops.append({"level": level, "octant": octant, "kind": kind, "pad_cols": pad_cols, "yb0": yb0, "block_kinds": kinds,
                        "singles": by_kind[0], "x_pairs": by_kind[1], "y_pairs": by_kind[2]})
            i += 7 + n_blk + ne * (d + 3)
        return info, ops

    M2L_DIGEST_FAMILIES = ("scalars", "partners_orbits", "class_lists", "class_rows", "class_cells", "tiles1", "tiles2", "batches")

    def debug_m2l_table_digests(self):
        n, nl = ctypes.c_int32(), ctypes.c_int32()
        self._raise(self._lib.bbfmm_debug_m2l_table_digests(self._h, None, 0, ctypes.byref(n), None, 0, ctypes.byref(nl)))
        assert n.value == len(self.M2L_DIGEST_FAMILIES)
        dig, fl = np.zeros(n.value, dtype=np.uint64), np.zeros(max(nl.value, 1))
        self._raise(self._lib.bbfmm_debug_m2l_table_digests(self._h, dig.ctypes.data, n.value, ctypes.byref(n), fl.ctypes.data,
                                                            nl.value, ctypes.byref(nl)))
        return {k: f"{int(v):016x}" for k, v in zip(self.M2L_DIGEST_FAMILIES, dig)}, [float(v) for v in fl[:nl.value]]

    def debug_m2l_s2_last_ksplit(self) -> int:
        ks = ctypes.c_int32()
        self._raise(self._lib.bbfmm_debug_m2l_s2_last_ksplit(self._h, ctypes.byref(ks)))
        return ks.value

    def debug_leaf_runs(self) -> dict:
        c = (ctypes.c_int32 * 4)()
        self._raise(self._lib.bbfmm_debug_leaf_runs(self._h, c))
        return {"mask": c[0], "runs": c[1], "rest": c[2], "jobs": c[3]}

    def debug_group_state(self) -> dict:
        parts = self.device_count()
        c = (ctypes.c_int64 * (9 + parts))()
        self._raise(self._lib.bbfmm_debug_group_state(self._h, c, len(c)))
        keys = ("parts", "own_copies", "live_mirrors", "mirror_pieces", "peer_copies", "plain_copies", "weight_waits", "weights_in",
                "self_peer_refused")
        st = {k: int(v) for k, v in zip(keys, c[:9])}
        st["own_copies"], st["self_peer_refused"] = bool(st["own_copies"]), bool(st["self_peer_refused"])
        st["owners"] = [int(v) for v in c[9:9 + parts]]
        return st

    def debug_get_coefficients(self, which: str, k: int) -> np.ndarray:
        s = self.stats()
        n = s.n_nodes
        if which in ("P", "p"):
            ln = ctypes.c_int32(0)
            self._raise(self._lib.bbfmm_debug_m2l_parity_len(self._h, ctypes.byref(ln)))
            n = ln.value
        out = np.zeros((k, s.n_cells, n))
        self._raise(self._lib.bbfmm_debug_get_coefficients(self._h, which.encode()[0:1], k,
                                                           out.ctypes.data))
        return out

    def debug_apply_m2l_tables_host(self, M: np.ndarray) -> np.ndarray:
        M = np.ascontiguousarray(M, dtype=np.float64)
        Lc = np.zeros_like(M)
        self._raise(self._lib.bbfmm_debug_apply_m2l_tables_host(self._h, M.ctypes.data,
                                                                Lc.ctypes.data))
        return Lc


def make_grid(origin, steps, shape) -> L.Grid:
    origin = np.asarray(origin, dtype=np.float64).reshape(-1)
    d = origin.size
    steps = np.asarray(steps, dtype=np.float64)
    shape = [int(n) for n in np.asarray(shape).reshape(-1)]
    if not 1 <= d <= 3 or steps.shape != (d, d) or len(shape) != d:
        raise ValueError("a d-D grid needs an origin of d coordinates, (d, d) steps and d counts, d = 1..3")
    g = L.Grid()
    g.size, g.d = ctypes.sizeof(L.Grid), d
    for a in range(3):
        g.shape[a] = shape[a] if a < d else 1
    for j in range(d):
        g.origin[j] = origin[j]
        for a in range(d):
            g.steps[3 * j + a] = steps[j, a]
    return g


def debug_grid_coords(where: int, origin, steps, shape, r0: int, n: int) -> np.ndarray:
    g = make_grid(origin, steps, shape)
    out = np.zeros((n, g.d), order="F")
    rc = L.load().bbfmm_debug_grid_coords(int(where), ctypes.byref(g), int(r0), int(n), out.ctypes.data, max(n, 1))
    if rc != L.OK:
        raise (RuntimeError if rc == L.DEVICE_ERROR else ValueError)(f"bbfmm_debug_grid_coords failed with status {rc}")
    return out


def debug_split_runs(where: int, tgt_begin, tgt_end, job_cell, cap: int):
    tb = np.ascontiguousarray(tgt_begin, dtype=np.int32)
    te = np.ascontiguousarray(tgt_end, dtype=np.int32)
    jc = np.ascontiguousarray(job_cell, dtype=np.int32)
# ... 58 lines not shown
```

### include/ferreus_bbfmm_hip.h

```cpp
#ifndef FERREUS_BBFMM_HIP_H
#define FERREUS_BBFMM_HIP_H

#include <stdint.h>

#ifdef __cplusplus
extern "C" {
#endif

typedef enum {
    BBFMM_OK = 0,
    BBFMM_POINT_OUTSIDE_TREE = 1,
    BBFMM_KERNEL_NO_GRADIENTS = 2,
    BBFMM_BAD_ARGUMENT = 3,
    BBFMM_DEVICE_ERROR = 4,
    BBFMM_UNSUPPORTED = 5,
    BBFMM_CALLBACK_FAILED = 6
} bbfmm_status;

typedef enum {
    BBFMM_KERNEL_LINEAR_RBF = 0,
    BBFMM_KERNEL_THIN_PLATE_SPLINE_RBF = 1,
    BBFMM_KERNEL_CUBIC_RBF = 2,
    BBFMM_KERNEL_SPHEROIDAL3_RBF = 3,
    BBFMM_KERNEL_SPHEROIDAL5_RBF = 4,
// ... 207 lines not shown
                                     int64_t basis_size, const int64_t *target_indices,
                                     int64_t n_target_indices, const double *poly, int64_t ldp,
                                     double nugget, double *result);

int bbfmm_prepare_target_subset(bbfmm_handle *h, const int64_t *target_indices, int64_t n_target_indices);

int bbfmm_matvec_device(bbfmm_handle *h, const double *d_w, int64_t ldw, int32_t k, double *d_out,
                        int64_t ldo, int32_t sync);

int bbfmm_target_subset_create(bbfmm_handle *h, const int64_t *target_indices, int64_t n_target_indices,
                               int32_t *subset_id);
int bbfmm_matvec_subset_device(bbfmm_handle *h, int32_t subset_id, const double *d_w, double *d_y, int32_t sync);

void *bbfmm_stream(bbfmm_handle *h);

int bbfmm_set_partition(bbfmm_handle *h, int32_t rank, int32_t world);
int64_t bbfmm_partition_row_count(const bbfmm_handle *h);
int bbfmm_partition_rows(const bbfmm_handle *h, int64_t *rows_out);

int64_t bbfmm_partition_coarse_count(const bbfmm_handle *h);
int bbfmm_matvec_partition_upward(bbfmm_handle *h, const double *d_w, int64_t ldw, int32_t k, double *d_coarse, void *comm_stream);
int bbfmm_matvec_partition_finish(bbfmm_handle *h, const double *d_coarse, double *d_out, int64_t ldo, int32_t sync, void *comm_stream);
int32_t bbfmm_partition_world(const bbfmm_handle *h);
int32_t bbfmm_partition_rank(const bbfmm_handle *h);
int bbfmm_partition_bounds(const bbfmm_handle *h, int32_t world, int64_t *bounds_out);
int bbfmm_matvec_partition_finish_sorted(bbfmm_handle *h, const double *d_coarse, double *d_seg, int64_t ld, void *comm_stream);
int bbfmm_partition_scatter(bbfmm_handle *h, const double *d_all, int32_t first_part, int32_t n_parts, int64_t m_max, int32_t k,
                            double *d_out, int64_t ldo);
int bbfmm_debug_partition_upward_counts(const bbfmm_handle *h, int64_t *counts_out, uint8_t *reads_out, int64_t *info_out);

int bbfmm_debug_host_copy_rates(int64_t n, double *out4);

typedef struct {
    int32_t d, order, n_nodes, depth;
    int64_t n_points, n_cells, n_leaves;
    int64_t n_u, n_v, n_w, n_x;
    int64_t p2p_pairs;
    int64_t p2p_tile_bytes_k1;
    double m2l_flops_k1;
    double center[3];
    double radius;
    int64_t wx_pairs;
    int64_t wx_tile_bytes_k1;
    int32_t m2l_basis_rank;
    int32_t m2l_basis_len;
    int32_t m2l_batches;
    int32_t m2l_rhs_per_pass;
    int64_t m2l_slots_bytes_per_rhs;
    int64_t m2l_intermediate_bytes;
} bbfmm_tree_stats;

int bbfmm_get_tree_stats(const bbfmm_handle *h, bbfmm_tree_stats *out);
int bbfmm_tree_built_on_device(const bbfmm_handle *h);

int bbfmm_get_cells(const bbfmm_handle *h, uint64_t *keys, uint8_t *is_leaf);
int bbfmm_get_leaf_sources(const bbfmm_handle *h, int64_t *ptr, int64_t *idx);
int bbfmm_get_list(const bbfmm_handle *h, char which, int64_t *ptr, int32_t *idx,
                   int64_t *n_entries);
int bbfmm_get_m2l_ranks(const bbfmm_handle *h, int32_t *ranks, int32_t *n_ref_out);
int bbfmm_get_m2l_operator(const bbfmm_handle *h, int32_t level, int32_t ref, double *out);
int bbfmm_get_m2l_factors(const bbfmm_handle *h, int32_t level, int32_t ref, double *u, double *vt);
int bbfmm_get_permutation_tables(const bbfmm_handle *h, int32_t *n_perm, int32_t *perm,
                                 int32_t *invperm, int32_t *perm_lookup, int32_t *ref_lookup);
int bbfmm_points_to_leaves(const bbfmm_handle *h, const double *x, int64_t m, int64_t ldx,
                           int32_t *cell_out, int64_t *bad_point_index);

#define BBFMM_N_PHASES 11
int bbfmm_set_profiling(bbfmm_handle *h, int32_t enable);
int bbfmm_get_phase_ms(bbfmm_handle *h, double *ms_out, int64_t *count_out);
int bbfmm_reset_phase_ms(bbfmm_handle *h);

int bbfmm_mfma_f64_selftest(double *tflops, int32_t *layout_errors, double *info6);
int bbfmm_fp64_valu_selftest(double *tflops, double *clock_mhz);

int bbfmm_debug_kernel_values(int32_t where, int32_t kernel_id, double base_range, double total_sill, const double *r2,
                              int64_t n, double *value_out, double *value_g_out, double *factor_out);
int bbfmm_debug_math(int32_t where, int32_t which, const double *x, int64_t n, double *out, double *out2);

int bbfmm_debug_dense_m2m(const bbfmm_handle *h, int32_t child_index, double *out);
int bbfmm_debug_apply_m2l_tables_host(const bbfmm_handle *h, const double *M, double *L);
int bbfmm_debug_m2l_variants(const bbfmm_handle *h, int64_t *n_variants, int64_t *n_cells);
int bbfmm_debug_m2l_pairs(const bbfmm_handle *h, int32_t *out, int64_t cap, int64_t *n_out, int32_t *pairs_on);
int bbfmm_debug_m2l_pairs_axes(const bbfmm_handle *h, int32_t *out, int64_t cap, int64_t *n_out);
int bbfmm_debug_m2l_pairs_stage2(const bbfmm_handle *h, int32_t *out, int64_t cap, int64_t *n_out, int32_t *pairs_on);
int bbfmm_debug_m2l_pairs_axes_stage2(const bbfmm_handle *h, int32_t *out, int64_t cap, int64_t *n_out);
int bbfmm_debug_m2l_table_digests(const bbfmm_handle *h, uint64_t *digests, int32_t cap, int32_t *n_out, double *flops_level,
                                  int32_t flops_cap, int32_t *n_levels_out);
int bbfmm_debug_m2l_s2_last_ksplit(const bbfmm_handle *h, int32_t *ksplit);
int bbfmm_debug_leaf_runs(const bbfmm_handle *h, int32_t *counts);
int bbfmm_debug_group_state(const bbfmm_handle *h, int64_t *out, int64_t cap);

uint64_t bbfmm_debug_morton_encode(int32_t d, const uint64_t *anchor, uint64_t level);
void bbfmm_debug_morton_decode(int32_t d, uint64_t key, uint64_t *anchor_out, uint64_t *level_out);
int32_t bbfmm_debug_morton_neighbours(int32_t d, uint64_t key, uint64_t *keys_out);
int32_t bbfmm_debug_direction_vectors(int32_t d, int32_t *out);
int bbfmm_debug_reference_vectors(const bbfmm_handle *h, int32_t *out, int32_t *n_ref_out);

int bbfmm_debug_get_coefficients(bbfmm_handle *h, char which, int32_t k, double *out);
int bbfmm_debug_m2l_parity_len(const bbfmm_handle *h, int32_t *len);


typedef int (*bbfmm_apply_fn)(void *user, const double *x, double *y, int64_t n);
typedef void (*bbfmm_iteration_fn)(void *user, int64_t iter, double residual, double progress);

enum { BBFMM_ACCURACY_ABSOLUTE = 0, BBFMM_ACCURACY_RELATIVE = 1 };

void bbfmm_givens_rotation(double f, double g, double *c, double *s, double *r);

int bbfmm_fgmres(int64_t n, bbfmm_apply_fn a, void *a_user, const double *b, bbfmm_apply_fn m, void *m_user,
                 const double *x0, int32_t max_outer_iterations, int32_t max_inner_iterations,
                 int32_t tolerance_type, double tolerance, bbfmm_iteration_fn callback, void *cb_user,
                 double *x, int64_t *iterations, double *final_residual);

int bbfmm_schwarz_ddm_solver(int64_t n, bbfmm_apply_fn matvec, void *a_user, const double *rhs,
                             bbfmm_apply_fn m, void *m_user, int32_t max_iterations, int32_t tolerance_type,
                             double tolerance, bbfmm_iteration_fn callback, void *cb_user, double *x,
                             int64_t *iterations, double *final_residual);

typedef struct bbfmm_rbf_system {
    bbfmm_handle *tree;
    int64_t basis_size;
    const double *monomial_matrix;
    int64_t ld_monomial;
    double nugget;
} bbfmm_rbf_system;
int bbfmm_rbf_system_apply(void *user, const double *x, double *y, int64_t n);


typedef int (*bbfmm_apply_device_fn)(void *user, const double *d_x, double *d_y, int64_t n, void *stream);

typedef struct bbfmm_rbf_system_device bbfmm_rbf_system_device;
int bbfmm_rbf_system_device_create(bbfmm_handle *tree, int64_t basis_size, const double *monomial_matrix, int64_t ld,
                                   double nugget, bbfmm_rbf_system_device **out);
void bbfmm_rbf_system_device_destroy(bbfmm_rbf_system_device *s);
int bbfmm_rbf_system_apply_device(void *user, const double *d_x, double *d_y, int64_t n, void *stream);

int bbfmm_fgmres_device(int64_t n, bbfmm_apply_device_fn a, void *a_user, const double *d_b, bbfmm_apply_device_fn m,
                        void *m_user, const double *d_x0, int32_t max_outer_iterations, int32_t max_inner_iterations,
                        int32_t tolerance_type, double tolerance, bbfmm_iteration_fn callback, void *cb_user,
                        double *d_x, int64_t *iterations, double *final_residual, void *stream);

int bbfmm_schwarz_ddm_solver_device(int64_t n, bbfmm_apply_device_fn matvec, void *a_user, const double *d_rhs,
                                    bbfmm_apply_device_fn m, void *m_user, int32_t max_iterations,
                                    int32_t tolerance_type, double tolerance, bbfmm_iteration_fn callback,
                                    void *cb_user, double *d_x, int64_t *iterations, double *final_residual,
                                    void *stream);

int bbfmm_debug_solver_vector_op(int32_t op, int32_t alpha_mode, int64_t n, const double *a, const double *b,
                                 const double *c, double alpha, int32_t count, const double *coeffs, int32_t offset,
                                 double *out, double *scalars_out);

typedef struct bbfmm_ddm bbfmm_ddm;
typedef struct bbfmm_ddm_params {
    int64_t leaf_threshold;
    double overlap_quota;
    double coarse_ratio;
    int64_t coarse_threshold;
} bbfmm_ddm_params;
void bbfmm_ddm_params_defaults(bbfmm_ddm_params *out);
void bbfmm_ddm_params_for_points(int64_t n, bbfmm_ddm_params *out);
int bbfmm_ddm_build(const double *points, int64_t n, int32_t d, int64_t ld, const bbfmm_ddm_params *params,
                    bbfmm_ddm **out);
void bbfmm_ddm_destroy(bbfmm_ddm *t);
int32_t bbfmm_ddm_num_levels(const bbfmm_ddm *t);
int64_t bbfmm_ddm_level_size(const bbfmm_ddm *t, int32_t level);
int bbfmm_ddm_level_points(const bbfmm_ddm *t, int32_t level, int64_t *out);
// ... 131 lines not shown
```

Measured before the change: 34.91 matvecs/s.

## Skip padded slices and dead row groups in M2L stage-1 parity GEMM

The parity-basis stage-1 M2L kernel now reads a per-block count of live 16-row groups and a per-part tail slice count, and skips MFMA work on zero-padded K slices at the end of each parity part and on row groups with no destination. The operand layout is reordered into 4-row slices so the inner loop can exit early, and the live counts are staged through LDS by DMA. A host-side reference and a debug query mirror the skipping. The cost is extra branching and a second unrolled MFMA path, which may add register pressure and code size.

```diff
diff --git a/ferreus_rbf_rs_amd/_lib.py b/ferreus_rbf_rs_amd/_lib.py
--- a/ferreus_rbf_rs_amd/_lib.py
+++ b/ferreus_rbf_rs_amd/_lib.py
@@ -142,6 +142,7 @@
     "bbfmm_debug_m2l_variants": (ctypes.c_int, [c_p, c_p, c_p]),
     "bbfmm_debug_m2l_pairs": (ctypes.c_int, [c_p, c_p, c_i64, c_p, c_p]),
     "bbfmm_debug_m2l_pairs_axes": (ctypes.c_int, [c_p, c_p, c_i64, c_p]),
+    "bbfmm_debug_m2l_s1_live_work": (ctypes.c_int, [c_p, c_p, c_i64, c_p]),
     "bbfmm_debug_m2l_pairs_stage2": (ctypes.c_int, [c_p, c_p, c_i64, c_p, c_p]),
     "bbfmm_debug_m2l_pairs_axes_stage2": (ctypes.c_int, [c_p, c_p, c_i64, c_p]),
     "bbfmm_debug_m2l_table_digests": (ctypes.c_int, [c_p, c_p, c_i32, c_p, c_p, c_i32, c_p]),
diff --git a/ferreus_rbf_rs_amd/csrc/capi_debug.cpp b/ferreus_rbf_rs_amd/csrc/capi_debug.cpp
--- a/ferreus_rbf_rs_amd/csrc/capi_debug.cpp
+++ b/ferreus_rbf_rs_amd/csrc/capi_debug.cpp
@@ -201,6 +201,15 @@
     return BBFMM_OK;
 }
 
+int bbfmm_debug_m2l_s1_live_work(const bbfmm_handle *h, int32_t *out, int64_t cap, int64_t *n_out) {
+    if (!h || !n_out) return BBFMM_BAD_ARGUMENT;
+    std::vector<int32_t> v;
+    h->tree.debug_m2l_s1_live_work(&v);
+    *n_out = static_cast<int64_t>(v.size());
+    if (out) std::copy(v.begin(), v.begin() + std::min<int64_t>(cap, *n_out), out);
+    return BBFMM_OK;
+}
+
 int bbfmm_debug_m2l_pairs_stage2(const bbfmm_handle *h, int32_t *out, int64_t cap, int64_t *n_out, int32_t *pairs_on) {
     if (!h || !n_out) return BBFMM_BAD_ARGUMENT;
     std::vector<int32_t> v;
diff --git a/ferreus_rbf_rs_amd/csrc/device.hpp b/ferreus_rbf_rs_amd/csrc/device.hpp
--- a/ferreus_rbf_rs_amd/csrc/device.hpp
+++ b/ferreus_rbf_rs_amd/csrc/device.hpp
@@ -13,6 +13,7 @@
 constexpr int kM2lS1BlockPairs = 160;
 constexpr int kM2lSlotWindow = 128;
 constexpr int kM2lBlkTwoDst = 1 << 30;
+constexpr int kM2lTailLiveAll = 4 | 4 << 3 | 4 << 6 | 4 << 9;
 
 struct DevCheb {
     int p, d, n, n_pad;
@@ -32,6 +33,7 @@
     const int32_t *row_dst;
     const int32_t *row_dst2;
     const int32_t *blk_t0;
+    const int32_t *blk_live;
     int32_t yb0;
     int32_t n_rows;
     int32_t r_pad16;
@@ -92,7 +94,7 @@
 void launch_m2l_stage1(const M2lClass *classes, const M2lTileDesc *tiles, const int32_t *tile_idx, int n_tiles,
                        int n_pad, int max_slot_t, int K, int64_t C, const double *M, double *cbuf,
                        int64_t cbuf_len, hipStream_t s, bool own_blocks = false, int max_blocks = 8, int ne16 = 0, int s_ee = 0,
-                       int s_eo = 0);
+                       int s_eo = 0, int tail_live = kM2lTailLiveAll);
 void launch_m2l_parity(const double *M, int n_pad, double *Mp, int n_par, int ne16, int n_e, int n_o, int p, int64_t rows,
                        hipStream_t s);
 struct M2lParityOffsets {
diff --git a/ferreus_rbf_rs_amd/csrc/device_m2l.hip b/ferreus_rbf_rs_amd/csrc/device_m2l.hip
--- a/ferreus_rbf_rs_amd/csrc/device_m2l.hip
+++ b/ferreus_rbf_rs_amd/csrc/device_m2l.hip
@@ -48,13 +48,19 @@
                  : "memory");
 }
 
+__device__ inline void dma4s(const int32_t *sbase, unsigned voff_bytes, unsigned lds_wave_byte_offset) {
+    asm volatile("s_mov_b32 m0, %2\n\ts_nop 0\n\tglobal_load_lds_dword %0, %1" ::"v"(voff_bytes),
+                 "s"(uniform_ptr(reinterpret_cast<const double *>(sbase))), "s"(uniform_u32(lds_wave_byte_offset))
+                 : "memory");
+}
+
 template <int NG16, int STAGE, int MINW, bool PAIRS = false>
 __global__ __launch_bounds__(512, MINW) void m2l_gemm_k4(const M2lClass *__restrict__ classes,
                                                   const M2lTileDesc *__restrict__ tiles, int n_pad, int g16_0,
                                                   int64_t C, const double *__restrict__ in, int64_t in_len,
                                                   double *__restrict__ out, int64_t out_len,
                                                   const uint16_t *__restrict__ qlist, int slot_t,
-                                                  const int32_t *__restrict__ tile_idx) {
+                                                  const int32_t *__restrict__ tile_idx, int tail_live) {
     extern __shared__ double lds[];
     const M2lTileDesc tile = tiles[blockIdx.x];
     const M2lClass cls = classes[tile.level_class];
@@ -84,16 +90,17 @@
     constexpr int BUF = OP_DOUBLES + 2048;
 
     constexpr int NP = NG16 / 2, NS = NG16 & 1;
+    constexpr bool ROWS4 = PAIRS;
     unsigned voff[NCH];
 #pragma unroll
     for (int i = 0; i < NCH; ++i) {
         const int c = wave + 8 * i;
         if (c < 4 * NP) {
             const int e = c / NP, pr = c - e * NP, k = lane >> 4, p = lane & 15;
-            voff[i] = (unsigned)(((4 * k + e) * ld + 32 * pr + 2 * p) * 8);
+            voff[i] = (unsigned)(((ROWS4 ? 4 * e + k : 4 * k + e) * ld + 32 * pr + 2 * p) * 8);
         } else {
             const int e = 2 * (c - 4 * NP) + (lane >> 5), r = lane & 31, k = r >> 3, pair = r & 7;
-            voff[i] = (unsigned)(((4 * k + e) * ld + 32 * NP + 2 * pair) * 8);
+            voff[i] = (unsigned)(((ROWS4 ? 4 * e + k : 4 * k + e) * ld + 32 * NP + 2 * pair) * 8);
         }
     }
     auto cell_p = [&](int pos) {
@@ -108,7 +115,7 @@
         const int p = cell_p(pos);
         const int64_t base = STAGE == 2 ? (int64_t)kr * in_len + cls.cbase[p]
                                         : ((int64_t)kr * C + cls.cells[p]) * (STAGE == 1 ? (int64_t)n_pad : in_len);
-        cptr[h] = in + base + 4 * k + 2 * eh;
+        cptr[h] = in + base + (ROWS4 ? 2 * ((lane >> 2) & 7) : 4 * k + 2 * eh);
     }
     const unsigned lds0 = lds_offset(lds);
     const int64_t qstride = (int64_t)16 * ld;
@@ -152,13 +159,17 @@
     if (STAGE == 1 && lane < 16) ptab[wave * 16 + lane] = cell_p(wave * 16 + lane);
     const unsigned aux0 = lds0 + (unsigned)(2 * BUF) * 8u;
     auto stage_cols = [&](int zb_, int par) {
-        if (STAGE == 1 && 64 * wave <= 16 * NG16) {
+        if constexpr (PAIRS) {
+            static_assert(!PAIRS || (16 * NG16 <= 192 && 192 + 16 * NG16 <= 7 * 64), "aux layout of the parity-basis stage 1");
+            const int e = 64 * wave + lane;
+            const unsigned dst = aux0 + (unsigned)(par * AUX + 64 * wave) * 4u;
+            if (e < 16 * NG16) dma4s(cls.row_dst + zb_ * BLK + 16 * g16, (unsigned)e * 4u, dst);
+            else if (e >= 192 && e < 192 + 16 * NG16) dma4s(cls.row_dst2 + zb_ * BLK + 16 * g16, (unsigned)(e - 192) * 4u, dst);
+            else if (wave == 7 && lane == 0) dma4s(cls.blk_t0 + zb_, 0u, aux0 + (unsigned)(par * AUX + 16 * NG16) * 4u);
+            else if (wave == 7 && lane == 1) dma4s(cls.blk_live + zb_, 0u, aux0 + (unsigned)(par * AUX + 16 * NG16) * 4u);
+        } else if (STAGE == 1 && 64 * wave <= 16 * NG16) {
             const int e = 64 * wave + lane;
             const int32_t *src = e < 16 * NG16 ? cls.row_dst + zb_ * BLK + 16 * g16 + e : cls.blk_t0 + zb_;
-            dma4(src, aux0 + (unsigned)(par * AUX + 64 * wave) * 4u);
-        } else if (PAIRS && 64 * wave < 192 + 16 * NG16) {
-            const int e = 64 * wave + lane - 192;
-            const int32_t *src = e < 16 * NG16 ? cls.row_dst2 + zb_ * BLK + 16 * g16 + e : cls.blk_t0 + zb_;
             dma4(src, aux0 + (unsigned)(par * AUX + 64 * wave) * 4u);
         }
     };
@@ -178,6 +189,9 @@
     }
     wait_dma_and_barrier();
     int qcnt = 0, zb = zb0;
+    const int q_end0 = s_ee > 0 ? s_ee - 1 : nq_e - 1, q_end1 = s_ee > 0 ? s_ee + s_eo - 1 : nq - 1;
+    const int q_end2 = s_ee > 0 ? s_ee + 2 * s_eo - 1 : -1, q_end3 = s_ee > 0 ? nq - 1 : -1;
+    int live_g = NG16;
     for (int sidx = 0; sidx < n_steps; ++sidx) {
         const double *op = lds + (sidx & 1) * BUF + lane;
         const double2 *op2 = reinterpret_cast<const double2 *>(lds + (sidx & 1) * BUF) + lane;
@@ -186,6 +200,8 @@
         if (STAGE == 1) {
             if (qcnt == 0 && zb + 1 < zb1) stage_cols(zb + 1, (zb + 1 - zb0) & 1);
             if (qcnt == nq - 2) stage_slots((zb - zb0) & 1);
+            if (ROWS4 && qcnt == 0)
+                live_g = min(max(__builtin_amdgcn_readfirstlane(aux[((zb - zb0) & 1) * AUX + 16 * NG16 + 1]), 0), NG16);
         }
         if (wave_live) {
             if constexpr (PAIRS) {
@@ -199,6 +215,49 @@
                         }
                 }
             }
+            if constexpr (ROWS4) {
+                const int nsl = qcnt == q_end0 ? tail_live & 7 : qcnt == q_end1 ? (tail_live >> 3) & 7
+                              : qcnt == q_end2 ? (tail_live >> 6) & 7 : qcnt == q_end3 ? (tail_live >> 9) & 7 : 4;
+                const double *cr = lds + (sidx & 1) * BUF + OP_DOUBLES + wave * 256 + 8 * (bk >> 1) + 2 * bj + (bk & 1);
+                static_assert(NS == 0, "the live-work walk takes the column groups in pairs");
+                int opaque_zero;
+                asm volatile("v_mov_b32 %0, 0" : "=v"(opaque_zero));
+                if ((nsl | opaque_zero) >= 4 && live_g == NG16) {
+#pragma unroll
+                    for (int e = 0; e < 4; ++e) {
+                        double bq[4];
+#pragma unroll
+                        for (int tg = 0; tg < 4; ++tg) bq[tg] = cr[tg * 64 + 16 * e];
+#pragma unroll
+                        for (int pr = 0; pr < NP; ++pr) {
+                            const double2 a = op2[(e * NP + pr) * 64];
+#pragma unroll
+                            for (int tg = 0; tg < 4; ++tg) {
+                                acc[tg][2 * pr] = __builtin_amdgcn_mfma_f64_4x4x4f64(a.x, bq[tg], acc[tg][2 * pr], 0, 0, 0);
+                                acc[tg][2 * pr + 1] = __builtin_amdgcn_mfma_f64_4x4x4f64(a.y, bq[tg], acc[tg][2 * pr + 1], 0, 0, 0);
+                            }
+                        }
+                    }
+                } else {
+#pragma unroll
+                    for (int e = 0; e < 4; ++e) {
+                        if (e >= nsl) break;
+                        double bq[4];
+#pragma unroll
+                        for (int tg = 0; tg < 4; ++tg) bq[tg] = cr[tg * 64 + 16 * e];
+#pragma unroll
+                        for (int pr = 0; pr < NP; ++pr) {
+                            if (2 * pr >= live_g) break;
+                            const double2 a = op2[(e * NP + pr) * 64];
+#pragma unroll
+                            for (int tg = 0; tg < 4; ++tg) {
+                                acc[tg][2 * pr] = __builtin_amdgcn_mfma_f64_4x4x4f64(a.x, bq[tg], acc[tg][2 * pr], 0, 0, 0);
+                                acc[tg][2 * pr + 1] = __builtin_amdgcn_mfma_f64_4x4x4f64(a.y, bq[tg], acc[tg][2 * pr + 1], 0, 0, 0);
+                            }
+                        }
+                    }
+                }
+            } else {
             constexpr int EH = PAIRS ? 1 : 2;
 #pragma unroll
             for (int eh0 = 0; eh0 < 2; eh0 += EH) {
@@ -231,6 +290,7 @@
                             acc[tg][NG16 - 1] = __builtin_amdgcn_mfma_f64_4x4x4f64(a, bq[tg][el], acc[tg][NG16 - 1], 0, 0, 0);
                     }
                 }
+            }
             }
         }
         if (++qcnt == nq) {
@@ -343,13 +403,14 @@
 template <int NG16, int STAGE, int MINW, bool PAIRS = false>
 static void m2l_gemm_launch(const M2lClass *classes, const M2lTileDesc *tiles, int n_tiles, int n_pad, int g16_0,
                             int n_colblocks, int K, int64_t C, const double *in, int64_t in_len, double *out,
-                            int64_t out_len, const uint16_t *qlist, int slot_t, const int32_t *tile_idx, hipStream_t s) {
+                            int64_t out_len, const uint16_t *qlist, int slot_t, const int32_t *tile_idx, hipStream_t s,
+                            int tail_live = 0) {
     const size_t lds = 2 * sizeof(double) * (size_t)(2 * NG16 * 128 + 2048) + (STAGE == 1 ? (size_t)(2 * (PAIRS ? 384 : 192) + 128 + 8 * 16 * (slot_t & 0xffff)) * 4 : 0);
     static std::atomic<uint64_t> attr_set[4] = {{0}, {0}, {0}, {0}};
     (void)allow_large_dynamic_lds(reinterpret_cast<const void *>(&m2l_gemm_k4<NG16, STAGE, MINW, PAIRS>), lds, attr_set);
     const int zdim = STAGE == 2 && slot_t > 1 ? n_colblocks * slot_t : n_colblocks;
     hipLaunchKernelGGL((m2l_gemm_k4<NG16, STAGE, MINW, PAIRS>), dim3(n_tiles, K, zdim), dim3(512), lds, s, classes,
-                       tiles, n_pad, g16_0, C, in, in_len, out, out_len, qlist, slot_t, tile_idx);
+                       tiles, n_pad, g16_0, C, in, in_len, out, out_len, qlist, slot_t, tile_idx, tail_live);
 }
 
 
@@ -411,7 +472,7 @@
 
 void launch_m2l_stage1(const M2lClass *classes, const M2lTileDesc *tiles, const int32_t *tile_idx, int n_tiles,
                        int n_pad, int max_slot_t, int K, int64_t C, const double *M, double *cbuf, int64_t cbuf_len,
-                       hipStream_t s, bool own_blocks, int max_blocks, int ne16, int s_ee, int s_eo) {
+                       hipStream_t s, bool own_blocks, int max_blocks, int ne16, int s_ee, int s_eo, int tail_live) {
     if (n_tiles == 0) return;
     int slot_t = 16;
     while (slot_t < max_slot_t) slot_t *= 2;
@@ -431,7 +492,7 @@
     if (ne16 > 0) {
         const int64_t packed = static_cast<int64_t>(ne16) | (static_cast<int64_t>(s_ee & 0xffff) << 32) | (static_cast<int64_t>(s_eo & 0x7fff) << 48);
         m2l_gemm_launch<kM2lS1BlockPairs / 16, 1, 1, true>(classes, tiles, n_tiles, n_pad, 0, n_colblocks, K, C, M, packed, cbuf, cbuf_len,
-                                                      nullptr, slot_t, tile_idx, s);
+                                                      nullptr, slot_t, tile_idx, s, tail_live);
         return;
     }
     m2l_dispatch_chunks<1>(kM2lS1Block / 16, classes, tiles, n_tiles, n_pad, n_colblocks, K, C, M, 0, cbuf, cbuf_len, nullptr,
diff --git a/ferreus_rbf_rs_amd/csrc/fmm_m2l_debug.cpp b/ferreus_rbf_rs_amd/csrc/fmm_m2l_debug.cpp
--- a/ferreus_rbf_rs_amd/csrc/fmm_m2l_debug.cpp
+++ b/ferreus_rbf_rs_amd/csrc/fmm_m2l_debug.cpp
@@ -146,15 +146,20 @@
                         const int32_t slot2 = hc.row_tpos2[row] >= 0 ? hc.cslot[pos * hc.n_t + hc.row_tpos2[row]] : -1;
                         if (slot < 0 && slot2 < 0) continue;
                         const double *mp = &Mp[static_cast<size_t>(hc.cells[pos]) * m2l_npar_];
+                        if ((row % m2l_s1_block_) / 16 >= hc.blk_live[static_cast<size_t>(row / m2l_s1_block_)]) continue;
+                        auto live = [&](int j) { return (j % 16) / 4 < m2l_live_slices_[static_cast<size_t>(j / 16)]; };
                         double a = 0.0, bsum = 0.0;
                         if (row / m2l_s1_block_ >= hc.yb0) {
                             for (int j = 0; j < m2l_npar_; ++j) {
+                                if (!live(j)) continue;
                                 const bool y_odd = (j >= m2l_s1_off_.v[1] && j < m2l_s1_off_.v[2]) || j >= m2l_s1_off_.v[3];
                                 (y_odd ? bsum : a) += hc.vt_all[static_cast<size_t>(j) * hc.r_pad16 + row] * mp[j];
                             }
                         } else {
-                            for (int j = 0; j < m2l_ne16_; ++j) a += hc.vt_all[static_cast<size_t>(j) * hc.r_pad16 + row] * mp[j];
-                            for (int j = m2l_ne16_; j < m2l_npar_; ++j) bsum += hc.vt_all[static_cast<size_t>(j) * hc.r_pad16 + row] * mp[j];
+                            for (int j = 0; j < m2l_ne16_; ++j)
+                                if (live(j)) a += hc.vt_all[static_cast<size_t>(j) * hc.r_pad16 + row] * mp[j];
+                            for (int j = m2l_ne16_; j < m2l_npar_; ++j)
+                                if (live(j)) bsum += hc.vt_all[static_cast<size_t>(j) * hc.r_pad16 + row] * mp[j];
                         }
                         if (slot >= 0) cbuf[static_cast<size_t>(slot) * 2 + hc.row_off[row]] = a + bsum;
                         if (slot2 >= 0) cbuf[static_cast<size_t>(slot2) * 2 + hc.row_off2[row]] = a - bsum;
@@ -284,6 +289,23 @@
     }
 }
 
+void FmmTree::debug_m2l_s1_live_work(std::vector<int32_t> *out) const {
+    out->clear();
+    out->push_back(m2l_s1_skip_);
+    out->push_back(m2l_s1_block_ / 16);
+    for (size_t i = 0; i < m2l_host_.size() + m2l_variants_.size(); ++i) {
+        const HostM2lClass &h = i < m2l_host_.size() ? m2l_host_[i] : m2l_variants_[i - m2l_host_.size()];
+        if (h.cells.empty()) continue;
+        out->push_back(h.level);
+        out->push_back(h.octant);
+        out->push_back(i < m2l_host_.size() ? 0 : 1);
+        out->push_back(static_cast<int32_t>(m2l_live_slices_.size()));
+        out->push_back(static_cast<int32_t>(h.blk_live.size()));
+        out->insert(out->end(), m2l_live_slices_.begin(), m2l_live_slices_.end());
+        out->insert(out->end(), h.blk_live.begin(), h.blk_live.end());
+    }
+}
+
 void FmmTree::debug_m2l_pairs_stage2(std::vector<int32_t> *out) const {
     out->clear();
     const int d = d_;
diff --git a/ferreus_rbf_rs_amd/csrc/fmm_m2l_tables.cpp b/ferreus_rbf_rs_amd/csrc/fmm_m2l_tables.cpp
--- a/ferreus_rbf_rs_amd/csrc/fmm_m2l_tables.cpp
+++ b/ferreus_rbf_rs_amd/csrc/fmm_m2l_tables.cpp
@@ -141,6 +141,7 @@
     double cbuf_mb = 0.0;
     bool s1_pairs = true, s2_pairs = true;
     int s1_axes = 0, s2_axes = 0;
+    int s1_skip = 3;
     int variant_min_tiles = 4;
     bool verbose = false;
     static M2lSwitches read() {
@@ -154,6 +155,7 @@
         sw.s2_pairs = number("BBFMM_M2L_S2_PAIRS", 1) != 0;
         sw.s1_axes = number("BBFMM_M2L_S1_AXES", 0);
         sw.s2_axes = number("BBFMM_M2L_S2_AXES", 0);
+        sw.s1_skip = number("BBFMM_M2L_S1_SKIP", 3) & 3;
         sw.variant_min_tiles = number("BBFMM_M2L_VARIANTS", 4);
         sw.verbose = std::getenv("BBFMM_VERBOSE") != nullptr;
         return sw;
@@ -457,6 +459,26 @@
     m2l_s_ee_ = off2.v[1] / 16;
     m2l_s_eo_ = (off2.v[2] - off2.v[1]) / 16;
     m2l_orbit_tables(q, npar2, [&](int part, int j) { return off2.v[part] + j; }, &m2l_par_node_, &m2l_par_sign_, nullptr);
+}
+
+void FmmTree::set_m2l_stage1_live_slices(const M2lSwitches &sw) {
+    m2l_s1_skip_ = sw.s1_skip;
+    m2l_tail_live_ = kM2lTailLiveAll;
+    m2l_live_slices_.assign(static_cast<size_t>(m2l_pairs_ ? m2l_npar_ : round_up(ops_.n, 32)) / 16, 4);
+    if (!m2l_pairs_ || !(m2l_s1_skip_ & 1)) return;
+    const M2lParts q(ops_);
+    const int n_parts = m2l_axes_ == 2 ? 4 : 2;
+    int tail = 0, step = 0;
+    for (int part = 0; part < 4; ++part) {
+        const int len = part >= n_parts ? 0 : m2l_axes_ == 2 ? q.len[part] : part == 0 ? m2l_ne_ : m2l_no_;
+        int last = 4;
+        for (int r = 0; r < len; r += 16, ++step) {
+            last = (std::min(16, len - r) + 3) / 4;
+            m2l_live_slices_[static_cast<size_t>(step)] = last;
+        }
+        tail |= last << (3 * part);
+    }
+    m2l_tail_live_ = tail;
 }
 
 FmmTree::M2lTargetOrder FmmTree::m2l_target_order(const std::vector<std::vector<int>> &tgt, int axes) const {
@@ -717,6 +739,14 @@
             hc.row_dst[r] = ((hc.row_tpos[r] - t0) << 24) | hc.row_off[r];
             if (hc.row_tpos2[r] >= 0) hc.row_dst2[r] = ((hc.row_tpos2[r] - t0) << 24) | hc.row_off2[r];
         }
+    }
+    const int n_g16 = m2l_s1_block_ / 16;
+    hc.blk_live.assign(n_blk, n_g16);
+    for (int b = 0; m2l_pairs_ && (m2l_s1_skip_ & 2) && b < n_blk; ++b) {
+        int live = 0;
+        for (int r = 0; r < m2l_s1_block_; ++r)
+            if (hc.row_dst[b * m2l_s1_block_ + r] >= 0 || hc.row_dst2[b * m2l_s1_block_ + r] >= 0) live = r / 16 + 1;
+        hc.blk_live[b] = live;
     }
     return true;
 }
@@ -1049,6 +1079,7 @@
         }
     std::vector<M2lSlotLayout> layouts;
     choose_m2l_stage1_axes(sw, &lists);
+    set_m2l_stage1_live_slices(sw);
     choose_m2l_stage2_axes(sw, &lists, &layouts);
     lists.index(ops_.n_vec);
     plan_m2l_batches(sw, layouts, &lists);
diff --git a/ferreus_rbf_rs_amd/csrc/fmm_tree.cpp b/ferreus_rbf_rs_amd/csrc/fmm_tree.cpp
--- a/ferreus_rbf_rs_amd/csrc/fmm_tree.cpp
+++ b/ferreus_rbf_rs_amd/csrc/fmm_tree.cpp
@@ -483,7 +483,7 @@
         c.n_cells = static_cast<int32_t>(h.cells.size());
         if (h.cells.empty()) continue;
         DevBuf<double> vt, ua;
-        DevBuf<int32_t> rt, rt2, ro, ce, cs;
+        DevBuf<int32_t> rt, rt2, ro, rl, ce, cs;
         DevBuf<int64_t> cb;
         {
             const size_t nvt = static_cast<size_t>(m2l_pairs_ ? m2l_npar_ : cheb_.n_pad) * h.r_pad16, nu = m2l_pairs2_ ? static_cast<size_t>(h.k_pad - h.kp) * m2l_s2_plan_.n_par() : static_cast<size_t>(h.k_pad) * cheb_.n_pad;
@@ -543,6 +543,7 @@
         CHK(dupload(&rt, h.row_dst));
         CHK(dupload(&rt2, h.row_dst2));
         CHK(dupload(&ro, h.blk_t0));
+        CHK(dupload(&rl, h.blk_live));
         CHK(dupload(&ce, h.cells));
         CHK(dalloc(&cs, h.cslot.size()));
         if (!h.cslot.empty()) HIPCHK(hipMemcpy(cs.p, h.cslot.data(), h.cslot.size() * sizeof(int32_t), hipMemcpyHostToDevice));
@@ -552,6 +553,7 @@
         c.row_dst = rt.p;
         c.row_dst2 = rt2.p;
         c.blk_t0 = ro.p;
+        c.blk_live = rl.p;
         c.cells = ce.p;
         c.cslot = cs.p;
         c.cbase = cb.p;
@@ -997,12 +999,12 @@
                                          cbuf_batch_len_, stream_);
             if (dp) {
                 launch_m2l_stage1(d_m2l_classes_.p, dp->d_tiles1.p + t1_first, dp->d_tile_idx.p, t1_count, s1_len, m2l_slot_t_, kb,
-                                  C, m_chunk, d_cbuf_.p, cbuf_batch_len_, stream_, false, m2l_max_blocks_, s1_ne16, m2l_s_ee_, m2l_s_eo_);
+                                  C, m_chunk, d_cbuf_.p, cbuf_batch_len_, stream_, false, m2l_max_blocks_, s1_ne16, m2l_s_ee_, m2l_s_eo_, m2l_tail_live_);
                 launch_m2l_stage1(d_m2l_classes_.p, dp->d_tiles1.p + dp->batch_t1[4 * b + 2], dp->d_tile_idx.p, dp->batch_t1[4 * b + 3],
-                                  s1_len, m2l_slot_t_, kb, C, m_chunk, d_cbuf_.p, cbuf_batch_len_, stream_, true, m2l_max_blocks_, s1_ne16, m2l_s_ee_, m2l_s_eo_);
+                                  s1_len, m2l_slot_t_, kb, C, m_chunk, d_cbuf_.p, cbuf_batch_len_, stream_, true, m2l_max_blocks_, s1_ne16, m2l_s_ee_, m2l_s_eo_, m2l_tail_live_);
             } else
                 launch_m2l_stage1(d_m2l_classes_.p, d_m2l_tiles1_.p + t1_first, d_tile_idx1_.p, t1_count, s1_len, m2l_slot_t_, kb, C,
-                                  m_chunk, d_cbuf_.p, cbuf_batch_len_, stream_, false, m2l_max_blocks_, s1_ne16, m2l_s_ee_, m2l_s_eo_);
+                                  m_chunk, d_cbuf_.p, cbuf_batch_len_, stream_, false, m2l_max_blocks_, s1_ne16, m2l_s_ee_, m2l_s_eo_, m2l_tail_live_);
             phase_end(kPhM2L1);
             phase_begin();
             if (s2_pairs) {
diff --git a/ferreus_rbf_rs_amd/csrc/fmm_tree.hpp b/ferreus_rbf_rs_amd/csrc/fmm_tree.hpp
--- a/ferreus_rbf_rs_amd/csrc/fmm_tree.hpp
+++ b/ferreus_rbf_rs_amd/csrc/fmm_tree.hpp
@@ -42,6 +42,7 @@
     std::vector<int8_t> src_kind;
     int yb0 = 0;
     int pad_cols = 0;
+    std::vector<int32_t> blk_live;
     int kp = 0;
     std::vector<int32_t> tgt_pair;
     std::vector<int8_t> tgt_kind;
@@ -217,6 +218,7 @@
     void debug_m2l_pairs(std::vector<int32_t> *out) const;
     bool m2l_pairs() const { return m2l_pairs_; }
     void debug_m2l_pairs_axes(std::vector<int32_t> *out) const;
+    void debug_m2l_s1_live_work(std::vector<int32_t> *out) const;
     void debug_m2l_pairs_stage2(std::vector<int32_t> *out) const;
     bool m2l_pairs_stage2() const { return m2l_pairs2_; }
     void debug_m2l_pairs_axes_stage2(std::vector<int32_t> *out) const;
@@ -258,6 +260,7 @@
     M2lSlotLayout m2l_slot_layout(int level, const M2lTargetOrder &order) const;
     std::vector<uint8_t> m2l_classes_present(int level) const;
     void choose_m2l_stage1_axes(const M2lSwitches &sw, M2lLists *lists);
+    void set_m2l_stage1_live_slices(const M2lSwitches &sw);
     void choose_m2l_stage2_axes(const M2lSwitches &sw, M2lLists *lists, std::vector<M2lSlotLayout> *layouts);
     void plan_m2l_batches(const M2lSwitches &sw, const std::vector<M2lSlotLayout> &layouts, M2lLists *lists);
     int build_m2l_level(const M2lLevel &lv, const M2lSwitches &sw, M2lBuildState *st);
@@ -354,6 +357,9 @@
     M2lParityOffsets m2l_s1_off_{{0, 0, 0, 0}};
     int m2l_s_ee_ = 0, m2l_s_eo_ = 0;
     int64_t m2l_work_[2] = {0, 0};
+    int m2l_s1_skip_ = 3;
+    std::vector<int32_t> m2l_live_slices_;
+    int m2l_tail_live_ = kM2lTailLiveAll;
     std::vector<int32_t> m2l_partner_y_;
     std::vector<int32_t> m2l_par_node_;
     std::vector<int8_t> m2l_par_sign_;
diff --git a/ferreus_rbf_rs_amd/fmm_tree.py b/ferreus_rbf_rs_amd/fmm_tree.py
--- a/ferreus_rbf_rs_amd/fmm_tree.py
+++ b/ferreus_rbf_rs_amd/fmm_tree.py
@@ -639,6 +639,22 @@
             i += 7 + n_blk + ne * (d + 3)
         return info, ops
 
+    def debug_m2l_s1_live_work(self):
+        fn = self._lib.bbfmm_debug_m2l_s1_live_work
+        n = ctypes.c_int64()
+        self._raise(fn(self._h, None, 0, ctypes.byref(n)))
+        buf = np.zeros(max(n.value, 2), dtype=np.int32)
+        self._raise(fn(self._h, buf.ctypes.data, n.value, ctypes.byref(n)))
+        info = {"skip": int(buf[0]), "groups": int(buf[1])}
+        ops, i = [], 2
+        while i < n.value:
+            level, octant, kind, ns, nb = (int(v) for v in buf[i:i + 5])
+            ops.append({"level": level, "octant": octant, "kind": kind,
+                        "slices": [int(v) for v in buf[i + 5:i + 5 + ns]],
+                        "groups": [int(v) for v in buf[i + 5 + ns:i + 5 + ns + nb]]})
+            i += 5 + ns + nb
+        return info, ops
+
     M2L_DIGEST_FAMILIES = ("scalars", "partners_orbits", "class_lists", "class_rows", "class_cells", "tiles1", "tiles2", "batches")
 
     def debug_m2l_table_digests(self):
diff --git a/include/ferreus_bbfmm_hip.h b/include/ferreus_bbfmm_hip.h
--- a/include/ferreus_bbfmm_hip.h
+++ b/include/ferreus_bbfmm_hip.h
@@ -313,6 +313,7 @@
 int bbfmm_debug_m2l_variants(const bbfmm_handle *h, int64_t *n_variants, int64_t *n_cells);
 int bbfmm_debug_m2l_pairs(const bbfmm_handle *h, int32_t *out, int64_t cap, int64_t *n_out, int32_t *pairs_on);
 int bbfmm_debug_m2l_pairs_axes(const bbfmm_handle *h, int32_t *out, int64_t cap, int64_t *n_out);
+int bbfmm_debug_m2l_s1_live_work(const bbfmm_handle *h, int32_t *out, int64_t cap, int64_t *n_out);
 int bbfmm_debug_m2l_pairs_stage2(const bbfmm_handle *h, int32_t *out, int64_t cap, int64_t *n_out, int32_t *pairs_on);
 int bbfmm_debug_m2l_pairs_axes_stage2(const bbfmm_handle *h, int32_t *out, int64_t cap, int64_t *n_out);
 int bbfmm_debug_m2l_table_digests(const bbfmm_handle *h, uint64_t *digests, int32_t cap, int32_t *n_out, double *flops_level,
```

New measurement: 34.87 matvecs/s. Within noise of the previous version (-0.1%).
